# XingqunQi-lab/EmotionGestures

Hardware: AMD Instinct MI355X
Metric: gesture clips/sec (34 frames, 43 joints) (higher is better)
Workload: dtype bf16x3; 1 GPU; TED clips: 4 s 16 kHz audio -> mel(128x124) -> CVAE sample -> generator -> 34x126 pose; global_batch=64, variant=Models_spatial_memory, parallelism=clip-sharded x1, no data-path collective, launch=hipGraph replay, 4 step(s) in flight, branch_streams=False, fold_affine=False

## Files before the change

emotiongestures_amd/_lib.py:

```python
from __future__ import annotations

import ctypes as C
import os

_HERE = os.path.dirname(os.path.abspath(__file__))
LIB_PATH = os.path.join(_HERE, "libemogest_hip.so")

EG_PREC_F32, EG_PREC_BF16X3, EG_PREC_BF16 = 0, 1, 2
PRECISIONS = {"f32": EG_PREC_F32, "fp32": EG_PREC_F32, "bf16x3": EG_PREC_BF16X3, "bf16": EG_PREC_BF16}

(PACK_RAW, PACK_LINEAR, PACK_VEC_PAD, PACK_CONV3X3, PACK_BN_SCALE, PACK_BN_SHIFT, PACK_CONV1X1, PACK_STEM,
 PACK_WN_TAP, PACK_CONV1D, PACK_POS_TABLE, PACK_LINEAR_T, PACK_LINEAR_FOLD, PACK_BIAS_FOLD) = range(14)


class EgError(RuntimeError):
    pass


class EgWeightEntry(C.Structure):
    _fields_ = [("key", C.c_char * 192), ("kind", C.c_int32), ("dims", C.c_int32 * 4),
                ("offset", C.c_int64), ("numel", C.c_int64)]


class EgGeneratorConfig(C.Structure):
    _fields_ = [(n, C.c_int32) for n in (
        "frames", "pose_dim", "prior_frames", "chunk", "d_model", "d_inner", "n_layers", "n_head", "d_k",
        "n_mels", "spec_len", "text_len", "n_words", "embed_dim", "tcn_hidden", "tcn_layers", "variant",
        "precision", "n_position")] + [("reserved", C.c_int32 * 5)]


class EgCvaeConfig(C.Structure):
    _fields_ = [("frames", C.c_int32), ("d_model", C.c_int32), ("latent", C.c_int32), ("n_classes", C.c_int32),
                ("reserved", C.c_int32 * 4)]


_P = C.c_void_p
_I = C.c_int32
_L = C.c_int64


class EgLinearArgs(C.Structure):
    _fields_ = [(n, _P) for n in ("x", "w", "bias", "res1", "res2", "y", "gate_src", "drop_epoch", "partial", "x_images", "y_images")] + \
               [("drop_offset", C.c_uint64)] + \
               [(n, _I) for n in ("lda", "ldw", "ldr", "ldc", "ldg", "m", "n", "k", "relu", "precision", "splits", "k_x", "y_k")] + \
               [("drop_seed", C.c_uint32), ("drop_p", C.c_float)]


SIGNATURES = {
    "eg_last_error": (C.c_char_p, []),
    "eg_launch_count": (_L, []),
    "eg_launch_histogram": (_L, [C.c_char_p, _L, C.c_int32]),
    "eg_version": (C.c_char_p, []),
    "eg_set_default_precision": (C.c_int, [C.c_int]),
    "eg_get_default_precision": (C.c_int, []),
    "eg_generator_default_config": (C.c_int, [C.POINTER(EgGeneratorConfig)]),
    "eg_generator_create": (C.c_int, [C.POINTER(EgGeneratorConfig), C.POINTER(_P)]),
    "eg_generator_destroy": (None, [_P]),
    "eg_generator_arena_floats": (_L, [_P]),
    "eg_generator_num_weights": (_I, [_P]),
    "eg_generator_weight_entry": (C.c_int, [_P, _I, C.POINTER(EgWeightEntry)]),
    "eg_generator_workspace_bytes": (_L, [_P, _I]),
    "eg_generator_forward": (C.c_int, [_P, _P, _I, _P, _P, _P, _P, _P, _P, _P, _P, _P, _P, _L, _P]),
    "eg_generator_forward_draws": (C.c_int, [_P, _P, _I, _I, _P, _P, _P, _P, _P, _L, _P]),
    "eg_generator_draws_workspace_bytes": (_L, [_P, _I, _I]),
    "eg_generator_forward_rollout": (C.c_int, [_P, _P, _I, _I, _P, _P, _P, _P, _P, _P, _P, _P, _P, _P, _P, _P, _L, _P]),
    "eg_generator_rollout_workspace_bytes": (_L, [_P, _I, _I]),
    "eg_generator_forward_rollout_draws": (C.c_int, [_P, _P, _I, _I, _I, _P, _P, _P, _P, _P, _P, _P, _P, _P, _P, _P, _P, _L, _P]),
    "eg_generator_rollout_draws_workspace_bytes": (_L, [_P, _I, _I, _I]),
    "eg_rows_by_table": (C.c_int, [_P, _P, _P, _I, _L, _I, _P]),
    "eg_rollout_ragged_plan_ints": (_L, [_I, _L]),
    "eg_rollout_ragged_plan": (C.c_int, [_P, _I, _P, _P, _P, _P]),
    "eg_generator_forward_rollout_ragged": (C.c_int, [_P, _P, _I, _P, _P, _P, _P, _P, _P, _P, _P, _P, _P, _P, _P, _P, _P, _L, _P]),
    "eg_generator_rollout_ragged_workspace_bytes": (_L, [_P, _I, _L]),
    "eg_stream_state_bytes": (_L, [_P, _I, _I, _I]),
    "eg_stream_reset": (C.c_int, [_P, _P, _I, _I, _I, _P, _P, _P]),
    "eg_stream_push": (C.c_int, [_P, _P, _I, _I, _I, _P, _P, _P, _P]),
    "eg_generator_stream_step": (C.c_int, [_P, _P, _P, _I, _I, _I, _P, _P, _P, _P, _P, _P, _P, _P, _P, _L, _P]),
    "eg_stream_tail": (C.c_int, [_P, _P, _I, _I, _I, _P, _P]),
    "eg_generator_tap": (C.c_int, [_P, _I, _P, C.c_char_p, C.POINTER(_P), C.POINTER(_L)]),
    "eg_cvae_default_config": (C.c_int, [C.POINTER(EgCvaeConfig)]),
    "eg_cvae_create": (C.c_int, [C.POINTER(EgCvaeConfig), C.POINTER(_P)]),
    "eg_cvae_destroy": (None, [_P]),
    "eg_cvae_arena_floats": (_L, [_P]),
    "eg_cvae_num_weights": (_I, [_P]),
    "eg_cvae_weight_entry": (C.c_int, [_P, _I, C.POINTER(EgWeightEntry)]),
    "eg_cvae_workspace_bytes": (_L, [_P, _I]),
    "eg_cvae_sample": (C.c_int, [_P, _P, _I, _P, _P, _P, _P, _L, _P]),
    "eg_cvae_forward": (C.c_int, [_P, _P, _I, _P, _P, _P, _P, _P, _P, _P, _L, _P]),
    "eg_mel_tables": (C.c_int, [_P, _P, _P, _P]),
    "eg_mel_workspace_bytes": (_L, [_I, _I]),
    "eg_melspectrogram": (C.c_int, [_P, _I, _I, _P, _P, _P, _P, _P, _I, _P, _L, _P]),
    "eg_window_gather": (C.c_int, [_P, _I, _L, _I, _L, _I, _P, _P]),
    "eg_window_gather_ragged": (C.c_int, [_P, _I, _L, _P, _P, _L, _I, _P, _P]),
    "eg_beat_tables": (C.c_int, [_P, _P, _P, _P]),
    "eg_beat_workspace_bytes": (_L, [_I, _I]),
    "eg_beat_align": (C.c_int, [_P, _I, _I, _P, _I, _I, _I, _I, _I, C.c_double, _I, _P, _P, _P, _P, _P, _L, _P, _P, _P, _P, _P, _P, _P]),
    "eg_beat_tracks_meta_ints": (_L, [_I]),
    "eg_beat_tracks_meta": (C.c_int, [_P, _P, _P, _I, _I, _P]),
    "eg_beat_tracks_workspace_bytes": (_L, [_P, _P, _I, _I, _I]),
    "eg_beat_align_tracks": (C.c_int, [_P, _I, _L, _P, _P, _P, _I, _I, _I, _P, _I, _I, _P, C.c_double, _I, _P, _P, _P, _P, _P, _L, _P, _P, _P,
                                       _P, _P, _P, _P]),
    "eg_beat_tracks_scan": (C.c_int, [_P, _P, _I, _P, _P, _L, _P, _P, _P]),
    "eg_take_meta_ints": (_L, [_I]),
    "eg_take_meta": (C.c_int, [_P, _I, _P]),
    "eg_track_rows_pack": (C.c_int, [_P, _I, _I, _I, _I, _P, _P, _P, _P]),
    "eg_take_distance_workspace_bytes": (_L, [_P, _I, _I]),
    "eg_take_distance": (C.c_int, [_P, _I, _I, _I, _P, _P, _I, _P, _L, _P, _P, _P]),
    "eg_conv3x3": (C.c_int, [_P, _P, _P, _P, _P, _P, _P, _I, _I, _I, _I, _I, _I, _I, _I, _I, _P]),
    "eg_conv3x3_se": (C.c_int, [_P, _P, _P, _P, _P, _P, _P, _P, _P, _I, _I, _I, _I, _I, _I, _I, _I, _I, _P]),
    "eg_se_gate_pre": (C.c_int, [_P, _P, _I, _P, _P, _P, _P, _P, _P, _P, _P, _I, _I, _I, _I, _P]),
    "eg_conv3x3_gap_tiles": (_I, [_I, _I, _I, _I, _I]),
    "eg_conv3x3_channel_split": (_I, [_I, _I, _I, _I, _I, _I, _I]),
    "eg_stem_conv": (C.c_int, [_P, _P, _P, _P, _P, _P, _I, _I, _I, _I, _P]),
    "eg_se_gate": (C.c_int, [_P, _I, _P, _P, _P, _P, _P, _I, _I, _I, _P]),
    "eg_se_residual_relu": (C.c_int, [_P, _P, _P, _P, _P, _P, _P, _I, _I, _I, _I, _I, _I, _I, _I, _P]),
    "eg_linear": (C.c_int, [_P, _I, _P, _I, _P, _P, _P, _I, _P, _I, _I, _I, _I, _I, _I, _I, _I, _P]),
    "eg_split_tiles": (C.c_int, [_P, _I, _I, _I, _P, _P]),
    "eg_linear_presplit": (C.c_int, [_P, _I, _P, _I, _P, _P, _P, _I, _P, _I, _I, _I, _I, _I, _I, _P]),
    "eg_linear_splitk": (C.c_int, [_P, _I, _P, _I, _P, _P, _I, _I, _I, _I, _I, _I, _P, _I, _P]),
    "eg_layernorm": (C.c_int, [_P, _P, _P, _P, _I, _I, C.c_float, _P]),
    "eg_attention": (C.c_int, [_P, _I, _P, _I, _P, _I, _P, _I, _P, _I, _I, _I, _I, _I, _I, _P]),
    "eg_attention_masked": (C.c_int, [_P, _I, _P, _I, _P, _I, _P, _L, _I, _P, _I, _P, _I, _I, _I, _I, _I, _I, _P]),
    "eg_mha_workspace_bytes": (_L, [_I, _I, _I, _I, _I]),
    "eg_multi_head_attention": (C.c_int, [_P, _P, _P, _P, _P, _P, _P, _P, _P, _P, _I, _I, _I, _I, _I, _I, _P, _L, _P]),
    "eg_ffn_workspace_bytes": (_L, [_I, _I, _I]),
    "eg_positionwise_ffn": (C.c_int, [_P, _P, _P, _P, _P, _P, _P, _P, _I, _I, _I, _I, _P, _L, _P]),
    "eg_tcn_forward": (C.c_int, [_P, _P, _P, _I, _I, _I, _I, _I, _P, _L, _P]),
    "eg_add_rows": (C.c_int, [_P, _P, _P, _L, _I, _I, _P]),
    "eg_conv3x3_packed_floats": (_L, [_I, _I]),
    "eg_profile_enable": (C.c_int, [_I]),
    "eg_profile_disable": (C.c_int, []),
    "eg_profile_read": (_I, [_P, _P, _P, _I]),
    "eg_profile_read_workgroups": (_I, [_P, _I]),
    "eg_reparameterize": (C.c_int, [_P, _P, _P, _P, _L, _P]),
    "eg_conv1d": (C.c_int, [_P, _P, _P, _P, _P, _P, _I, _I, _I, _I, _I, _I, _I, _I, _P]),
    "eg_contrastive_workspace_bytes": (C.c_int64, [_I]),
    "eg_contrastive_loss": (C.c_int, [_P, _P, _I, _I, _P, _P, _P, _P, _L, _P]),
    "eg_contrastive_backward_workspace_bytes": (_L, [_I]),
    "eg_contrastive_loss_backward": (C.c_int, [_P, _P, _I, _I, _P, _P, _P, _L, _P]),
    "eg_transpose": (C.c_int, [_P, _I, _I, _I, _P, _I, _P]),
    "eg_gemm_tn_workspace_floats": (_L, [_I, _I, _L]),
    "eg_gemm_tn": (C.c_int, [_P, _I, _P, _I, _P, _I, _I, _I, _L, _P, _L, _I, _P]),
    "eg_conv3x3_wgrad": (C.c_int, [_P, _P, _P, _I, _I, _I, _I, _I, _I, _P, _L, _P]),
    "eg_im2col3x3": (C.c_int, [_P, _P, _I, _I, _I, _I, _I, _I, _P]),
    "eg_subsample": (C.c_int, [_P, _P, _I, _I, _I, _I, _I, _I, _P]),
    "eg_im2col1d": (C.c_int, [_P, _P, _I, _I, _I, _I, _I, _I, _I, _I, _I, _P]),
    "eg_conv1d_cl_forward": (C.c_int, [_P, _P, _P, _P] + [_I] * 9 + [_P]),
    "eg_conv1d_cl_backward_input": (C.c_int, [_P, _P, _P, _P] + [_I] * 9 + [_P]),
    "eg_conv1d_cl_backward_weight_workspace_floats": (_L, [_I] * 7),
    "eg_conv1d_cl_backward_weight": (C.c_int, [_P, _P, _P, _P, _P] + [_I] * 9 + [_P, _L, _P]),
    "eg_pad_cols": (C.c_int, [_P, _P, _L, _I, _I, _P]),
    "eg_colreduce_workspace_floats": (_L, [_I]),
    "eg_bn_train_forward": (C.c_int, [_P, _P, _P, _P, _P, _P, _P, _P, _L, _I, C.c_float, C.c_float, _P, _P]),
    "eg_bn_train_backward": (C.c_int, [_P, _P, _P, _P, _P, _P, _P, _P, _L, _I, _I, _P, _P]),
    "eg_bn_train_forward_gap": (C.c_int, [_P, _P, _I, _I, _P, _P, _P, _P, _P, _P, _P, _P, _L, _I, C.c_float, C.c_float, _P, _P]),
    "eg_bn_train_forward_sq": (C.c_int, [_P, _P, _P, _I, _I, _P, _P, _P, _P, _P, _P, _P, _P, _L, _I, C.c_float, C.c_float, _P, _P]),
    "eg_conv3x3_sq": (C.c_int, [_P, _P, _P, _P, _P, _P] + [_I] * 8 + [_P]),
    "eg_se_gate_train_forward": (C.c_int, [_P] * 12 + [_I, _I, _I, _P]),
    "eg_se_tail_forward": (C.c_int, [_P] * 9 + [_I, _I, _I, _P]),
    "eg_se_tail_backward_reduce": (C.c_int, [_P] * 7 + [_I, _I, _I, _P, _P]),
    "eg_se_gate_train_backward": (C.c_int, [_P] * 16 + [_I, _I, _I, _P]),
    "eg_se_tail_backward_finish": (C.c_int, [_P] * 14 + [_I, _I, _I, _P]),
    "eg_se_tail_backward_apply": (C.c_int, [_P] * 13 + [_I, _I, _I, _P]),
# ... 82 lines not shown
```

emotiongestures_amd/csrc/common.h:

```cpp
#pragma once
#include <hip/hip_runtime.h>
#include <stdint.h>
#include <stdio.h>
#include <stdarg.h>
#include <atomic>
#include "emogest.h"


typedef float f4 __attribute__((ext_vector_type(4)));
typedef short bf8 __attribute__((ext_vector_type(8)));

#define EG_WAVE 64

void eg_set_error(const char* fmt, ...);

#define EG_REQUIRE(cond, code, ...)                      \
    do {                                                 \
        if (!(cond)) {                                   \
            eg_set_error(__VA_ARGS__);                   \
            return (code);                               \
        }                                                \
    } while (0)

extern std::atomic<long long> g_eg_launches;
extern bool g_eg_launch_hist;
void egi_count_launch(const char* what);
static inline int eg_check_launch(const char* what) {
    g_eg_launches.fetch_add(1, std::memory_order_relaxed);
    if (g_eg_launch_hist) egi_count_launch(what);
    hipError_t e = hipGetLastError();
    if (e != hipSuccess) {
        eg_set_error("%s: %s", what, hipGetErrorString(e));
        return EG_ERR_HIP;
    }
    return EG_OK;
}

int eg_ensure_dynamic_lds(const void* kernel, size_t bytes, const char* who);
#define EG_HIP_TRY(expr, what)                                                         \
    do {                                                                               \
        hipError_t _e = (expr);                                                        \
        if (_e != hipSuccess) {                                                        \
            eg_set_error("%s: %s", (what), hipGetErrorString(_e));                     \
            return EG_ERR_HIP;                                                         \
        }                                                                              \
    } while (0)

static inline bool eg_aligned16(const void* p) { return (reinterpret_cast<uintptr_t>(p) & 15u) == 0; }
static inline int64_t eg_round_up(int64_t x, int64_t m) { return (x + m - 1) / m * m; }
static inline int eg_cdiv(int a, int b) { return (a + b - 1) / b; }

__device__ __forceinline__ float handoff_blend(const float* __restrict__ alpha, int j, int P, float old, float fresh) {
#pragma clang fp contract(off)
    const float a = alpha ? alpha[j] : (float)(j + 1) / (float)(P + 1);
    const float keep = (1.f - a) * old, take = a * fresh;
    return keep + take;
}

__device__ __forceinline__ float wave_sum(float v) {
#pragma unroll
    for (int o = 32; o > 0; o >>= 1) v += __shfl_xor(v, o, 64);
    return v;
}
__device__ __forceinline__ float wave_max(float v) {
#pragma unroll
    for (int o = 32; o > 0; o >>= 1) v = fmaxf(v, __shfl_xor(v, o, 64));
    return v;
}

__device__ __forceinline__ unsigned short f32_to_bf16_rne(float x) {
    unsigned int u = __float_as_uint(x);
    u += 0x7FFFu + ((u >> 16) & 1u);
    return (unsigned short)(u >> 16);
}
__device__ __forceinline__ float bf16_to_f32(unsigned short h) { return __uint_as_float(((unsigned int)h) << 16); }

typedef __bf16 bf16x2_t __attribute__((ext_vector_type(2)));
typedef float f32x2_t __attribute__((ext_vector_type(2)));
typedef unsigned int u32x4_t __attribute__((ext_vector_type(4)));
template <bool WANT_LO>
__device__ __forceinline__ void split_octet(const f4& v0, const f4& v1, bf8& hi, bf8& lo) {
    u32x4_t h, l;
#pragma unroll
    for (int p = 0; p < 4; ++p) {
        const f32x2_t x = {p < 2 ? v0[2 * p] : v1[2 * p - 4], p < 2 ? v0[2 * p + 1] : v1[2 * p - 3]};
        const unsigned hu = __builtin_bit_cast(unsigned, __builtin_convertvector(x, bf16x2_t));
        h[p] = hu;
        if (WANT_LO) {
            const f32x2_t r = {x[0] - __uint_as_float(hu << 16), x[1] - __uint_as_float(hu & 0xffff0000u)};
            l[p] = __builtin_bit_cast(unsigned, __builtin_convertvector(r, bf16x2_t));
        }
    }
    hi = __builtin_bit_cast(bf8, h);
    if (WANT_LO) lo = __builtin_bit_cast(bf8, l);
}

__device__ __forceinline__ unsigned int mix32(unsigned int h) {
    h ^= h >> 16; h *= 0x85EBCA6Bu; h ^= h >> 13; h *= 0xC2B2AE35u; h ^= h >> 16;
    return h;
}
__device__ __forceinline__ unsigned int dropout_seed(unsigned int seed, const int* __restrict__ epoch) {
    return epoch ? seed ^ mix32((unsigned int)*epoch * 0x9E3779B9u + 0x7F4A7C15u) : seed;
}
__device__ __forceinline__ bool dropout_keep(unsigned int seed, unsigned long long ctr, unsigned int thr) {
    return mix32(mix32((unsigned int)ctr ^ seed) + (unsigned int)(ctr >> 32) * 0x9E3779B9u + 0x6A09E667u) >= thr;
}
struct EgDropout {
    unsigned int thr = 0, seed = 0;
    float inv_keep = 1.f;
    unsigned long long offset = 0;
    const int* epoch = nullptr;
};

__device__ __forceinline__ void xcd_tile(int& bx, int& by) {
    const int gx = gridDim.x, gy = gridDim.y, total = gx * gy;
// ... 38 lines not shown
```

emotiongestures_amd/csrc/conv.hip:

```cpp
#include <type_traits>
#include "common.h"


namespace {

struct ConvArgs {
    const float* x; const float* w; const float* bias; const float* scale; const float* shift;
    float* y; float* gap;
    float* gap2 = nullptr;
    int H, W, Ho, Wo, cout, relu, nchw, tiles_x, tiles;
    const float* gate = nullptr; const float* res = nullptr; int relu2 = 0;
    const float* in_scale = nullptr; const float* in_shift = nullptr;
    int wrow = 0;
    const unsigned* res_bits = nullptr;
    const float* res_q = nullptr;
    unsigned int* dbg = nullptr;
};
__device__ __forceinline__ f4 residual_quad(const float* __restrict__ res, const unsigned* __restrict__ bits, size_t e) {
    f4 r = *reinterpret_cast<const f4*>(res + e);
    if (bits) {
        const unsigned nb = bits[e >> 5] >> (unsigned)(e & 28);
        r[0] = (nb & 1u) ? r[0] : 0.f;
        r[1] = (nb & 2u) ? r[1] : 0.f;
        r[2] = (nb & 4u) ? r[2] : 0.f;
        r[3] = (nb & 8u) ? r[3] : 0.f;
    }
    return r;
}

template <int S, int TH> struct ConvGeom {
    static constexpr int IH = (TH - 1) * S + 3;
    static constexpr int IW = 31 * S + 3;
    static constexpr int NPIX = IH * IW;
    static constexpr int PL = (S == 1) ? ((NPIX + 15) / 16 * 16) : (NPIX | 1);
    static constexpr int MT = TH * 2 / 4;
};

template <int TH> struct ConvGeomDG2 {
    static constexpr int IH = TH + 1;
    static constexpr int IW = 33;
    static constexpr int NPIX = IH * IW;
    static constexpr int PL = (NPIX + 15) / 16 * 16;
};

template <int CIN, int NT, int S, int TH>
__global__ __launch_bounds__(256) void conv3x3_f32_kernel(ConvArgs a) {
    using G = ConvGeom<S, TH>;
    constexpr int COUTP = NT * 16, IW = G::IW, NPIX = G::NPIX, PL = G::PL, MT = G::MT;
    __shared__ f4 tile[8 * PL];

    const int tid = threadIdx.x, wave = tid >> 6, lane = tid & 63, li = lane & 15, kq = lane >> 4;
    int tile_id = blockIdx.x, b = blockIdx.y;
    {
        const int total = gridDim.x * gridDim.y;
        if ((total & 7) == 0) {
            const int lin = blockIdx.y * gridDim.x + blockIdx.x;
            const int log = (lin & 7) * (total >> 3) + (lin >> 3);
            b = log / (int)gridDim.x;
            tile_id = log - b * (int)gridDim.x;
        }
    }
    const int ty = tile_id / a.tiles_x, tx = tile_id - ty * a.tiles_x;
    const int oy0 = ty * TH, ox0 = tx * 32;
    const int iy0 = oy0 * S - 1, ix0 = ox0 * S - 1;

    int pbase[MT];
#pragma unroll
    for (int t = 0; t < MT; ++t) {
        const int id = wave * MT + t;
// ... 46 lines not shown
            }
        }
    }

    f4 gsum[NT];
#pragma unroll
    for (int n = 0; n < NT; ++n) gsum[n] = (f4){0.f, 0.f, 0.f, 0.f};
#pragma unroll
    for (int n = 0; n < NT; ++n) {
        const int co = n * 16 + kq * 4;
        const f4 bi = a.bias ? *reinterpret_cast<const f4*>(a.bias + co) : (f4){0.f, 0.f, 0.f, 0.f};
        const f4 sc = a.scale ? *reinterpret_cast<const f4*>(a.scale + co) : (f4){1.f, 1.f, 1.f, 1.f};
        const f4 sh = a.shift ? *reinterpret_cast<const f4*>(a.shift + co) : (f4){0.f, 0.f, 0.f, 0.f};
        const f4 gt = (a.gate && co < a.cout) ? *reinterpret_cast<const f4*>(a.gate + (size_t)b * a.cout + co) : (f4){1.f, 1.f, 1.f, 1.f};
#pragma unroll
        for (int t = 0; t < MT; ++t) {
            const int id = wave * MT + t;
            const int oy = oy0 + (id >> 1), ox = ox0 + (id & 1) * 16 + li;
            const bool valid = (oy < a.Ho) && (ox < a.Wo);
            f4 v = acc[t][n] + bi;
            if (a.relu) {
#pragma unroll
                for (int r = 0; r < 4; ++r) v[r] = fmaxf(v[r], 0.f);
            }
            v = v * sc + sh;
            if (a.gate) v = v * gt;
            if (a.res && valid && co < a.cout) v += residual_quad(a.res, a.res_bits, (((size_t)b * a.Ho + oy) * a.Wo + ox) * a.cout + co);
            if (a.relu2) {
#pragma unroll
                for (int r = 0; r < 4; ++r) v[r] = fmaxf(v[r], 0.f);
            }
            if (valid) {
                if (!a.nchw) {
                    if (co < a.cout)
                        *reinterpret_cast<f4*>(a.y + (((size_t)b * a.Ho + oy) * a.Wo + ox) * a.cout + co) = v;
                } else {
#pragma unroll
                    for (int r = 0; r < 4; ++r)
                        if (co + r < a.cout)
                            a.y[((size_t)b * a.cout + co + r) * a.Ho * a.Wo + (size_t)oy * a.Wo + ox] = v[r];
                }
                gsum[n] += v;
            }
        }
    }
    if (a.gap) {
        float* sred = reinterpret_cast<float*>(tile);
        __syncthreads();
#pragma unroll
        for (int n = 0; n < NT; ++n) {
#pragma unroll
            for (int r = 0; r < 4; ++r) {
                float s = gsum[n][r];
                s += __shfl_xor(s, 1, 64); s += __shfl_xor(s, 2, 64);
                s += __shfl_xor(s, 4, 64); s += __shfl_xor(s, 8, 64);
                if (li == 0) sred[wave * COUTP + n * 16 + kq * 4 + r] = s;
            }
        }
        __syncthreads();
        if (tid < a.cout) {
            const float s = (sred[tid] + sred[COUTP + tid]) + (sred[2 * COUTP + tid] + sred[3 * COUTP + tid]);
            a.gap[((size_t)b * a.tiles + tile_id) * a.cout + tid] = s;
        }
    }
}


template <int CIN, int NTT, int S, int TH, int WM, int WN, int TERMS, int RING, bool SPLIT = false, bool DG2 = false>
__global__ __launch_bounds__(256, 2) void conv3x3_bf16_kernel(ConvArgs a, const bf8* __restrict__ whi,
                                                           const bf8* __restrict__ wlo) {
    static_assert(!DG2 || (S == 1 && !SPLIT), "DG2 tiles the dy grid with unit stride");
    using G = typename std::conditional<DG2, ConvGeomDG2<TH>, ConvGeom<S, TH>>::type;
    constexpr int PH = DG2 ? 4 : 1;
    constexpr int COUTP = NTT * 16, IW = G::IW, NPIX = G::NPIX, PL = G::PL;
    constexpr int MT = TH * 2 / WM, NT = NTT / WN;
    constexpr int NIMG = (TERMS == 3) ? 2 : 1;
    constexpr int TILE = NIMG * 4 * PL;
    constexpr int WIMG = 4 * COUTP;
    constexpr int WBUF = NIMG * WIMG;
    constexpr int NSTEP = (CIN / 32) * 9;
    static_assert(WM * WN == 4 && MT * WM == TH * 2 && NT * WN == NTT, "wave tiling");
    extern __shared__ __attribute__((aligned(16))) bf8 lds[];
    bf8* tile = lds;
    bf8* wring = lds + TILE;

    const int tid = threadIdx.x, wave = tid >> 6, lane = tid & 63, li = lane & 15, kq = lane >> 4;
    const int wm = wave / WN, wn = wave % WN;
    int tile_id = blockIdx.x, b = blockIdx.y;
    const int c0 = SPLIT ? (int)blockIdx.z * COUTP : 0;
    if (!SPLIT) {
        const int total = gridDim.x * gridDim.y;
        if ((total & 7) == 0) {
            const int lin = blockIdx.y * gridDim.x + blockIdx.x;
            const int log = (lin & 7) * (total >> 3) + (lin >> 3);
            b = log / (int)gridDim.x;
            tile_id = log - b * (int)gridDim.x;
        }
    }
    const int ty = tile_id / a.tiles_x, tx = tile_id - ty * a.tiles_x;
    const int oy0 = ty * TH, ox0 = tx * 32;
    const int iy0 = DG2 ? oy0 : oy0 * S - 1, ix0 = DG2 ? ox0 : ox0 * S - 1;

    int pbase[MT];
#pragma unroll
    for (int t = 0; t < MT; ++t) {
        const int id = wm * MT + t;
        pbase[t] = ((id >> 1) * S) * IW + ((id & 1) * 16 + li) * S;
    }
    f4 acc[PH][MT][NT];
#pragma unroll
    for (int ph = 0; ph < PH; ++ph)
#pragma unroll
        for (int t = 0; t < MT; ++t)
#pragma unroll
            for (int n = 0; n < NT; ++n) acc[ph][t][n] = (f4){0.f, 0.f, 0.f, 0.f};
    const float* __restrict__ xb = a.x + (size_t)b * a.H * a.W * CIN;

    const int wave_u = __builtin_amdgcn_readfirstlane(wave);
    constexpr int PIECES = WIMG / 64;
    constexpr int GTOT = NIMG * PIECES;
    constexpr bool COUNTED = (GTOT % 4 == 0);
    constexpr int GW = GTOT / 4;
    auto issue_weights = [&](int step, int buf) {
        const int chunk = step / 9, tap = step - chunk * 9;
        if constexpr (SPLIT) {
            static_assert(COUNTED, "split instantiations deal whole pieces to the four waves");
            const size_t rbase = ((size_t)tap * (CIN / 8) + chunk * 4) * a.wrow + c0;
#pragma unroll
            for (int p = 0; p < GW; ++p) {
                const int flat = p * 4 + wave_u;
                const int img = flat / PIECES, piece = flat - img * PIECES;
                const int slot = piece * 64 + lane, oct = slot / COUTP, co = slot - oct * COUTP;
                const bf8* src = (img ? wlo : whi) + rbase + (size_t)oct * a.wrow + co;
                __builtin_amdgcn_global_load_lds((const __attribute__((address_space(1))) void*)src,
                                                 (__attribute__((address_space(3))) void*)(wring + buf * WBUF + img * WIMG + piece * 64), 16, 0, 0);
            }
            return;
        }
        const size_t gbase = ((size_t)tap * (CIN / 8) + chunk * 4) * COUTP;
        if constexpr (PIECES % 4 == 0) {
#pragma unroll
            for (int img = 0; img < NIMG; ++img) {
                const bf8* src = (img ? wlo : whi) + gbase;
#pragma unroll
                for (int p = 0; p < PIECES / 4; ++p) {
                    const int piece = p * 4 + wave_u;
                    __builtin_amdgcn_global_load_lds((const __attribute__((address_space(1))) void*)(src + piece * 64 + lane),
                                                     (__attribute__((address_space(3))) void*)(wring + buf * WBUF + img * WIMG + piece * 64),
                                                     16, 0, 0);
                }
            }
        } else {
#pragma unroll
            for (int p = 0; p < (GTOT + 3) / 4; ++p) {
                const int flat = p * 4 + wave_u;
                if (COUNTED || flat < GTOT) {
                    const int img = flat / PIECES, piece = flat - img * PIECES;
                    const bf8* src = (img ? wlo : whi) + gbase;
                    __builtin_amdgcn_global_load_lds((const __attribute__((address_space(1))) void*)(src + piece * 64 + lane),
                                                     (__attribute__((address_space(3))) void*)(wring + buf * WBUF + img * WIMG + piece * 64),
                                                     16, 0, 0);
                }
            }
        }
    };
    constexpr int NIT = (((NPIX + 7) / 8) * 32 + 255) / 256;
    f4 pv[NIT][2];
    int goff[NIT], lslot[NIT];
#pragma unroll
    for (int it = 0; it < NIT; ++it) {
        const int idx = tid + it * 256;
        const int p = (idx >> 5) * 8 + (idx & 7), oc = (idx >> 3) & 3;
        const int iy = p / IW, ix = p - iy * IW;
        const int gy = iy0 + iy, gx = ix0 + ix;
        const bool inside = p < NPIX && gy >= 0 && gy < a.H && gx >= 0 && gx < a.W;
        goff[it] = inside ? (gy * a.W + gx) * CIN + oc * 8 : -1;
        lslot[it] = p < NPIX ? oc * PL + p : -1;
    }
    auto load_tile = [&](int chunk) {
#pragma unroll
        for (int it = 0; it < NIT; ++it) {
            pv[it][0] = pv[it][1] = (f4){0.f, 0.f, 0.f, 0.f};
            if (goff[it] >= 0) {
                const float* src = xb + goff[it] + chunk * 32;
                pv[it][0] = *reinterpret_cast<const f4*>(src);
                pv[it][1] = *reinterpret_cast<const f4*>(src + 4);
            }
        }
    };
    const int oc8s = ((tid >> 3) & 3) * 8;
    auto store_tile = [&](int chunk) {
        f4 s0 = (f4){1.f, 1.f, 1.f, 1.f}, s1 = s0, h0 = (f4){0.f, 0.f, 0.f, 0.f}, h1 = h0;
        if (a.in_scale) {
            s0 = *reinterpret_cast<const f4*>(a.in_scale + chunk * 32 + oc8s); s1 = *reinterpret_cast<const f4*>(a.in_scale + chunk * 32 + oc8s + 4);
            h0 = *reinterpret_cast<const f4*>(a.in_shift + chunk * 32 + oc8s); h1 = *reinterpret_cast<const f4*>(a.in_shift + chunk * 32 + oc8s + 4);
        }
#pragma unroll
        for (int it = 0; it < NIT; ++it) {
            if (lslot[it] >= 0) {
                if (a.in_scale && goff[it] >= 0) {
                    pv[it][0] = pv[it][0] * s0 + h0;
                    pv[it][1] = pv[it][1] * s1 + h1;
                }
                bf8 hi, lo;
                split_octet<TERMS == 3>(pv[it][0], pv[it][1], hi, lo);
                tile[lslot[it]] = hi;
                if (TERMS == 3) tile[4 * PL + lslot[it]] = lo;
            }
        }
    };

    struct Frags { bf8 wh[NT], wl[NT], xh[MT], xl[MT]; };
    auto read_w = [&](Frags& f, int tap) {
        const bf8* Wh = wring + (tap % 3) * WBUF + kq * COUTP + wn * NT * 16 + li;
#pragma unroll
        for (int n = 0; n < NT; ++n) {
            f.wh[n] = Wh[n * 16];
            if (TERMS == 3) f.wl[n] = Wh[WIMG + n * 16];
        }
    };
    auto read_x = [&](Frags& f, int tap) {
        const int kh = tap / 3, kw = tap - kh * 3;
        const int toff = DG2 ? (kh == 2 ? IW : 0) + (kw == 2 ? 1 : 0) : kh * IW + kw;
#pragma unroll
        for (int t = 0; t < MT; ++t) {
            f.xh[t] = tile[kq * PL + pbase[t] + toff];
            if (TERMS == 3) f.xl[t] = tile[(4 + kq) * PL + pbase[t] + toff];
        }
    };
    static_assert(MT % 2 == 0, "a step's MFMAs are issued as two halves (pixel tiles)");
    auto mfma_half = [&](const Frags& f, int half, int tap) {
        const int ph = DG2 ? (tap / 3 != 1 ? 2 : 0) + (tap % 3 != 1 ? 1 : 0) : 0;
#pragma unroll
        for (int t = half * (MT / 2); t < (half + 1) * (MT / 2); ++t)
#pragma unroll
            for (int n = 0; n < NT; ++n) {
                if (TERMS == 3) {
                    acc[ph][t][n] = __builtin_amdgcn_mfma_f32_16x16x32_bf16(f.wl[n], f.xh[t], acc[ph][t][n], 0, 0, 0);
                    acc[ph][t][n] = __builtin_amdgcn_mfma_f32_16x16x32_bf16(f.wh[n], f.xl[t], acc[ph][t][n], 0, 0, 0);
                }
                acc[ph][t][n] = __builtin_amdgcn_mfma_f32_16x16x32_bf16(f.wh[n], f.xh[t], acc[ph][t][n], 0, 0, 0);
            }
    };
    static_assert(RING == 3, "schedule below assumes a 3-slot ring");
    auto mid_sync = [&](bool copy_in_flight) {
        if constexpr (COUNTED) {
            __builtin_amdgcn_sched_barrier(0);
            if (copy_in_flight) wait_vmcnt_imm<GW>(); else wait_vmcnt_imm<0>();
            wait_lgkmcnt0();
            wg_barrier();
        } else {
            __syncthreads();
        }
    };
    issue_weights(0, 0);
    if (NSTEP > 1) issue_weights(1, 1);
    load_tile(0);
    Frags fr[2];
#pragma unroll 1
    for (int chunk = 0; chunk < CIN / 32; ++chunk) {
        store_tile(chunk);
        if (COUNTED && chunk > 0) {
            wait_vmcnt_imm<GW>();
            wait_lgkmcnt0();
            wg_barrier();
        } else {
            __syncthreads();
        }
        if (chunk + 1 < CIN / 32) load_tile(chunk + 1);
        read_w(fr[0], 0);
        read_x(fr[0], 0);
#pragma unroll
        for (int tap = 0; tap < 9; ++tap) {
            const int step = chunk * 9 + tap;
            if (step + 2 < NSTEP) issue_weights(step + 2, (tap + 2) % 3);
            mfma_half(fr[tap & 1], 0, tap);
            mid_sync(step + 2 < NSTEP);
            if (tap < 8) { read_w(fr[(tap + 1) & 1], tap + 1); read_x(fr[(tap + 1) & 1], tap + 1); }
            mfma_half(fr[tap & 1], 1, tap);
        }
    }

    if constexpr (DG2) {
        const size_t ohw = (size_t)a.Ho * a.Wo;
        float* __restrict__ yb = a.y + (size_t)b * ohw * a.cout;
        const float* __restrict__ rq = a.res_q ? a.res_q + (size_t)b * a.H * a.W * a.cout : nullptr;
#pragma unroll
        for (int ph = 0; ph < 4; ++ph) {
            const int py = ph >> 1, px = ph & 1;
#pragma unroll
            for (int t = 0; t < MT; ++t) {
                const int id = wm * MT + t;
                const int by = oy0 + (id >> 1), bx = ox0 + (id & 1) * 16 + li;
                const int oy = 2 * by + py, ox = 2 * bx + px;
                if (by < a.H && bx < a.W && oy < a.Ho && ox < a.Wo) {
#pragma unroll
                    for (int n = 0; n < NT; ++n) {
                        const int co = (wn * NT + n) * 16 + kq * 4;
                        if (co < a.cout) {
                            f4 v = acc[ph][t][n];
                            if (ph == 0 && rq) v += *reinterpret_cast<const f4*>(rq + ((size_t)by * a.W + bx) * a.cout + co);
                            *reinterpret_cast<f4*>(yb + ((size_t)oy * a.Wo + ox) * a.cout + co) = v;
                        }
                    }
                }
            }
        }
        return;
    }

    f4 gsum[NT], gsq[NT];
    int pixo[MT];
#pragma unroll
    for (int t = 0; t < MT; ++t) {
        const int id = wm * MT + t;
        const int oy = oy0 + (id >> 1), ox = ox0 + (id & 1) * 16 + li;
        pixo[t] = (oy < a.Ho && ox < a.Wo) ? oy * a.Wo + ox : -1;
    }
    const int hw = a.Ho * a.Wo;
    float* __restrict__ yb = a.y + (size_t)b * hw * a.cout;
#pragma unroll
    for (int n = 0; n < NT; ++n) {
        gsum[n] = (f4){0.f, 0.f, 0.f, 0.f};
        gsq[n] = gsum[n];
        const int co = c0 + (wn * NT + n) * 16 + kq * 4;
        const f4 bi = a.bias ? *reinterpret_cast<const f4*>(a.bias + co) : (f4){0.f, 0.f, 0.f, 0.f};
        const f4 sc = a.scale ? *reinterpret_cast<const f4*>(a.scale + co) : (f4){1.f, 1.f, 1.f, 1.f};
        const f4 sh = a.shift ? *reinterpret_cast<const f4*>(a.shift + co) : (f4){0.f, 0.f, 0.f, 0.f};
        const f4 gt = (a.gate && co < a.cout) ? *reinterpret_cast<const f4*>(a.gate + (size_t)b * a.cout + co) : (f4){1.f, 1.f, 1.f, 1.f};
        const bool rb = a.res != nullptr;
        const size_t rbase = (size_t)b * hw * a.cout;
#pragma unroll
        for (int t = 0; t < MT; ++t) {
            f4 v = acc[0][t][n] + bi;
            if (a.relu) {
#pragma unroll
                for (int r = 0; r < 4; ++r) v[r] = fmaxf(v[r], 0.f);
            }
            v = v * sc + sh;
            if (a.gate) v = v * gt;
            if (rb && pixo[t] >= 0 && co < a.cout) v += residual_quad(a.res, a.res_bits, rbase + (size_t)pixo[t] * a.cout + co);
            if (a.relu2) {
#pragma unroll
                for (int r = 0; r < 4; ++r) v[r] = fmaxf(v[r], 0.f);
            }
            if (pixo[t] >= 0) {
                if (!a.nchw) {
                    if (co < a.cout) *reinterpret_cast<f4*>(yb + pixo[t] * a.cout + co) = v;
                } else {
#pragma unroll
                    for (int r = 0; r < 4; ++r)
                        if (co + r < a.cout) yb[(co + r) * hw + pixo[t]] = v[r];
                }
                gsum[n] += v;
                if (a.gap2) gsq[n] += v * v;
            }
        }
    }
    if (a.gap) {
        float* sred = reinterpret_cast<float*>(lds);
#pragma unroll
        for (int n = 0; n < NT; ++n) {
#pragma unroll
            for (int r = 0; r < 4; ++r) {
                float s = gsum[n][r];
                s += __shfl_xor(s, 1, 64); s += __shfl_xor(s, 2, 64);
                s += __shfl_xor(s, 4, 64); s += __shfl_xor(s, 8, 64);
                if (li == 0) sred[wm * COUTP + (wn * NT + n) * 16 + kq * 4 + r] = s;
                if (a.gap2) {
                    float q = gsq[n][r];
                    q += __shfl_xor(q, 1, 64); q += __shfl_xor(q, 2, 64);
                    q += __shfl_xor(q, 4, 64); q += __shfl_xor(q, 8, 64);
                    if (li == 0) sred[(WM + wm) * COUTP + (wn * NT + n) * 16 + kq * 4 + r] = q;
                }
            }
        }
        __syncthreads();
        if (tid < (SPLIT ? COUTP : a.cout)) {
            float s = 0.f;
#pragma unroll
            for (int m = 0; m < WM; ++m) s += sred[m * COUTP + tid];
            a.gap[((size_t)b * a.tiles + tile_id) * a.cout + c0 + tid] = s;
            if (a.gap2) {
                float q = 0.f;
#pragma unroll
                for (int m = 0; m < WM; ++m) q += sred[(WM + m) * COUTP + tid];
                a.gap2[((size_t)b * a.tiles + tile_id) * a.cout + c0 + tid] = q;
            }
        }
    }
}

template <int TERMS, int TH = 4, bool STAMP = false>
__global__ __launch_bounds__(256, 2) void conv3x3_c32_persistent_kernel(ConvArgs a, const bf8* __restrict__ whi, const bf8* __restrict__ wlo,
                                                                     int total_tiles, int tiles_per_wg) {
    using G = ConvGeom<1, TH>;
    constexpr int CIN = 32, IW = G::IW, NPIX = G::NPIX, PL = G::PL, MT = TH / 2, NT = 2;
    constexpr int NIMG = (TERMS == 3) ? 2 : 1;
    constexpr int TILE = NIMG * 4 * PL, WTAP = 4 * 32, WIMG = 9 * WTAP;
    static_assert(PL - NPIX >= 8 || TH == 4, "the gap scratch of the 8-row variant lives in the planes' padding slots");
    extern __shared__ __attribute__((aligned(16))) bf8 lds[];
    bf8* tile = lds;
    bf8* wl = lds + TILE;
    float* sred_base = reinterpret_cast<float*>(lds + TILE + NIMG * WIMG);
    const int sred_pitch = (TH == 4) ? 32 : PL * 4;
    float* sred = (TH == 4) ? sred_base : reinterpret_cast<float*>(tile + NPIX);

    const int tid = threadIdx.x, wave = tid >> 6, lane = tid & 63, li = lane & 15, kq = lane >> 4;
    const int wave_u = __builtin_amdgcn_readfirstlane(wave);
    int wg = blockIdx.x;
    if ((gridDim.x & 7) == 0) wg = (blockIdx.x & 7) * (gridDim.x >> 3) + (blockIdx.x >> 3);
    const int NWG = gridDim.x;
    const int t_begin = wg, t_end = total_tiles;
    (void)tiles_per_wg;
    if (t_begin >= t_end) return;

#pragma unroll
    for (int img = 0; img < NIMG; ++img) {
        const bf8* src = img ? wlo : whi;
#pragma unroll
        for (int p = 0; p < 5; ++p) {
            const int piece = p * 4 + wave_u;
            if (piece < WIMG / 64)
                __builtin_amdgcn_global_load_lds((const __attribute__((address_space(1))) void*)(src + piece * 64 + lane),
                                                 (__attribute__((address_space(3))) void*)(wl + img * WIMG + piece * 64), 16, 0, 0);
        }
    }

    constexpr int NIT = (((NPIX + 7) / 8) * 32 + 255) / 256;
    int piy[NIT], pix[NIT], lslot[NIT];
#pragma unroll
    for (int it = 0; it < NIT; ++it) {
        const int idx = tid + it * 256;
        const int p = (idx >> 5) * 8 + (idx & 7), oc = (idx >> 3) & 3;
        piy[it] = p / IW;
        pix[it] = p - piy[it] * IW;
        lslot[it] = p < NPIX ? oc * PL + p : -1;
    }
    const int oc8 = ((tid >> 3) & 3) * 8;
    f4 isc[2] = {(f4){1.f, 1.f, 1.f, 1.f}, (f4){1.f, 1.f, 1.f, 1.f}}, ish[2] = {(f4){0.f, 0.f, 0.f, 0.f}, (f4){0.f, 0.f, 0.f, 0.f}};
    if (a.in_scale) {
        isc[0] = *reinterpret_cast<const f4*>(a.in_scale + oc8); isc[1] = *reinterpret_cast<const f4*>(a.in_scale + oc8 + 4);
// ... 142 lines not shown
            for (int t = 0; t < MT; ++t)
#pragma unroll
                for (int n = 0; n < NT; ++n) {
                    if (TERMS == 3) {
                        acc[t][n] = __builtin_amdgcn_mfma_f32_16x16x32_bf16(f.wlf[n], f.xh[t], acc[t][n], 0, 0, 0);
                        acc[t][n] = __builtin_amdgcn_mfma_f32_16x16x32_bf16(f.wh[n], f.xl[t], acc[t][n], 0, 0, 0);
                    }
                    acc[t][n] = __builtin_amdgcn_mfma_f32_16x16x32_bf16(f.wh[n], f.xh[t], acc[t][n], 0, 0, 0);
                }
        }

        if constexpr (STAMP) {
#pragma unroll
            for (int t = 0; t < MT; ++t)
#pragma unroll
                for (int n = 0; n < NT; ++n) asm volatile("" : "+v"(acc[t][n]));
        }
        stamp(3);
        float* __restrict__ yb = a.y + (size_t)b * hw * 32;
        f4 gsum[NT], gsq[NT];
#pragma unroll
        for (int n = 0; n < NT; ++n) {
            gsum[n] = (f4){0.f, 0.f, 0.f, 0.f};
            gsq[n] = gsum[n];
            const int co = n * 16 + kq * 4;
            const f4 gt = a.gate ? *reinterpret_cast<const f4*>(a.gate + (size_t)b * 32 + co) : (f4){1.f, 1.f, 1.f, 1.f};
#pragma unroll
            for (int t = 0; t < MT; ++t) {
                f4 v = acc[t][n] + bi[n];
                if (a.relu) {
#pragma unroll
                    for (int r = 0; r < 4; ++r) v[r] = fmaxf(v[r], 0.f);
                }
                v = v * sc[n] + sh[n];
                if (a.gate) v = v * gt;
                if (has_res && pixo[t] >= 0) v += rs[t][n];
                if (a.relu2) {
#pragma unroll
                    for (int r = 0; r < 4; ++r) v[r] = fmaxf(v[r], 0.f);
                }
                if (pixo[t] >= 0) {
                    *reinterpret_cast<f4*>(yb + pixo[t] * 32 + co) = v;
                    gsum[n] += v;
                    if (a.gap2) gsq[n] += v * v;
                }
            }
        }
        if (a.gap) {
#pragma unroll
            for (int n = 0; n < NT; ++n)
#pragma unroll
                for (int r = 0; r < 4; ++r) {
                    float sm = gsum[n][r];
                    sm += __shfl_xor(sm, 1, 64); sm += __shfl_xor(sm, 2, 64);
                    sm += __shfl_xor(sm, 4, 64); sm += __shfl_xor(sm, 8, 64);
                    if (li == 0) sred[wave * sred_pitch + n * 16 + kq * 4 + r] = sm;
                    if (a.gap2) {
                        float q = gsq[n][r];
                        q += __shfl_xor(q, 1, 64); q += __shfl_xor(q, 2, 64);
                        q += __shfl_xor(q, 4, 64); q += __shfl_xor(q, 8, 64);
                        if (li == 0) sred[128 + wave * 32 + n * 16 + kq * 4 + r] = q;
                    }
                }
        }
        stamp(4);
        __syncthreads();
        stamp(5);
        if (a.gap && tid < 32) {
            float sm = 0.f;
#pragma unroll
            for (int m = 0; m < 4; ++m) sm += sred[m * sred_pitch + tid];
            a.gap[((size_t)b * a.tiles + tile_id) * 32 + tid] = sm;
            if (a.gap2) a.gap2[((size_t)b * a.tiles + tile_id) * 32 + tid] = (sred[128 + tid] + sred[160 + tid]) + (sred[192 + tid] + sred[224 + tid]);
        }
    }
    if constexpr (STAMP) {
        if (lane == 0 && a.dbg)
#pragma unroll
            for (int i = 0; i < 6; ++i) a.dbg[((size_t)blockIdx.x * 4 + wave) * 8 + i] = ph[i];
    }
}

__global__ __launch_bounds__(256) void stem_conv_kernel(const float* __restrict__ x, const float* __restrict__ w,
                                                        const float* __restrict__ bias, const float* __restrict__ scale,
                                                        const float* __restrict__ shift, float* __restrict__ y,
                                                        int B, int H, int W, int C) {
    extern __shared__ float rows[];
    const int cq_n = C >> 2, tid = threadIdx.x;
    const int b = blockIdx.x / H, oy = blockIdx.x - b * H, WP = W + 2;
    const float* xb = x + (size_t)b * H * W;
    for (int i = tid; i < 3 * WP; i += 256) {
        const int r = i / WP, c = i - r * WP, gy = oy + r - 1, gx = c - 1;
        rows[i] = (gy >= 0 && gy < H && gx >= 0 && gx < W) ? xb[gy * W + gx] : 0.f;
    }
    const int cq = tid % cq_n, px0 = tid / cq_n, pstep = 256 / cq_n;
    f4 wv[9];
#pragma unroll
    for (int t = 0; t < 9; ++t) wv[t] = *reinterpret_cast<const f4*>(w + t * C + cq * 4);
    const f4 bi = *reinterpret_cast<const f4*>(bias + cq * 4);
    const f4 sc = *reinterpret_cast<const f4*>(scale + cq * 4), sh = *reinterpret_cast<const f4*>(shift + cq * 4);
    __syncthreads();
    float* yrow = y + ((size_t)b * H + oy) * W * C + cq * 4;
    for (int ox = px0; ox < W; ox += pstep) {
        f4 acc = bi;
#pragma unroll
        for (int kh = 0; kh < 3; ++kh)
#pragma unroll
            for (int kw = 0; kw < 3; ++kw) acc += wv[kh * 3 + kw] * rows[kh * WP + ox + kw];
#pragma unroll
        for (int r = 0; r < 4; ++r) acc[r] = fmaxf(acc[r], 0.f);
        *reinterpret_cast<f4*>(yrow + (size_t)ox * C) = acc * sc + sh;
    }
}

__global__ __launch_bounds__(256) void se_gate_kernel(const float* __restrict__ gap, int tiles, const float* __restrict__ w1,
                                                      const float* __restrict__ b1, const float* __restrict__ w2,
                                                      const float* __restrict__ b2, float* __restrict__ gate, int C, float inv_hw) {
    __shared__ float m[256];
    __shared__ float h[32];
    const int b = blockIdx.x, t = threadIdx.x, R = C >> 3;
    {
        const int c = t % C, g = t / C, G = blockDim.x / C;
        float s = 0.f;
        for (int i = g; i < tiles; i += G) s += gap[((size_t)b * tiles + i) * C + c];
        m[t] = s;
        __syncthreads();
        float tot = 0.f;
        if (t < C)
            for (int j = 0; j < G; ++j) tot += m[j * C + t];
        __syncthreads();
        if (t < C) m[t] = tot * inv_hw;
    }
    __syncthreads();
    if (t < R) {
        float s = b1[t];
        for (int c = 0; c < C; ++c) s += w1[t * C + c] * m[c];
        h[t] = fmaxf(s, 0.f);
    }
    __syncthreads();
    if (t < C) {
        float s = b2[t];
        for (int j = 0; j < R; ++j) s += w2[t * R + j] * h[j];
        gate[(size_t)b * C + t] = 1.f / (1.f + expf(-s));
    }
}

constexpr int GP_T = 1024;
__global__ __launch_bounds__(GP_T) void se_gate_pre_kernel(const float* __restrict__ t1, const float* __restrict__ gap, int tiles,
                                                           const float* __restrict__ w2img, const float* __restrict__ scale2,
                                                           const float* __restrict__ shift2, const float* __restrict__ w1, const float* __restrict__ b1,
                                                           const float* __restrict__ wf2, const float* __restrict__ bf2, float* __restrict__ gate,
                                                           int H, int W, int C) {
    extern __shared__ __attribute__((aligned(16))) float sm[];
    const int b = blockIdx.x, t = threadIdx.x, G = GP_T / C, c = t % C, g = t / C, R = C >> 3;
    float* part = sm;
    float* S = sm + 5 * GP_T;
    float* zp = S + 9 * C;
    float* m = zp + GP_T;
    float* hbuf = m + C;
    const float* tb = t1 + (size_t)b * H * W * C;
    float s0 = 0.f, s1 = 0.f, s2 = 0.f, s3 = 0.f, s4 = 0.f;
#pragma unroll 4
    for (int i = g; i < tiles; i += G) s0 += gap[((size_t)b * tiles + i) * C + c];
#pragma unroll 4
    for (int x = g; x < W; x += G) {
        s1 += tb[(size_t)x * C + c];
        s2 += tb[((size_t)(H - 1) * W + x) * C + c];
    }
#pragma unroll 4
    for (int y = g; y < H; y += G) {
        s3 += tb[((size_t)y * W) * C + c];
        s4 += tb[((size_t)y * W + W - 1) * C + c];
    }
    part[t] = s0; part[GP_T + t] = s1; part[2 * GP_T + t] = s2; part[3 * GP_T + t] = s3; part[4 * GP_T + t] = s4;
    __syncthreads();
    if (t < C) {
        float T = 0.f, R0 = 0.f, RL = 0.f, C0 = 0.f, CL = 0.f;
        for (int j = 0; j < G; ++j) {
            T += part[j * C + t]; R0 += part[GP_T + j * C + t]; RL += part[2 * GP_T + j * C + t]; C0 += part[3 * GP_T + j * C + t];
            CL += part[4 * GP_T + j * C + t];
        }
        const float c00 = tb[t], c0L = tb[(size_t)(W - 1) * C + t], cL0 = tb[((size_t)(H - 1) * W) * C + t], cLL = tb[((size_t)(H - 1) * W + W - 1) * C + t];
#pragma unroll
        for (int kh = 0; kh < 3; ++kh)
#pragma unroll
            for (int kw = 0; kw < 3; ++kw) {
                const float rex = kh == 0 ? RL : (kh == 2 ? R0 : 0.f);
                const float cex = kw == 0 ? CL : (kw == 2 ? C0 : 0.f);
                float corner = 0.f;
                if (kh == 0 && kw == 0) corner = cLL;
                if (kh == 0 && kw == 2) corner = cL0;
                if (kh == 2 && kw == 0) corner = c0L;
                if (kh == 2 && kw == 2) corner = c00;
                S[(kh * 3 + kw) * C + t] = T - rex - cex + corner;
            }
    }
    __syncthreads();
    {
        const f4* w4 = reinterpret_cast<const f4*>(w2img);
        const int nq = 9 * (C >> 2);
        float z = 0.f;
#pragma unroll 4
        for (int q = g; q < nq; q += G) {
            const int tap = q / (C >> 2), cq = q - tap * (C >> 2);
            const f4 wv = w4[(size_t)q * C + c];
            const float* sp = S + tap * C + cq * 4;
            z += (wv[0] * sp[0] + wv[1] * sp[1]) + (wv[2] * sp[2] + wv[3] * sp[3]);
        }
        zp[g * C + c] = z;
    }
    __syncthreads();
    if (t < C) {
        float z = 0.f;
        for (int j = 0; j < G; ++j) z += zp[j * C + t];
        m[t] = z / (float)(H * W) * scale2[t] + shift2[t];
    }
    __syncthreads();
    {
        const int wv = t >> 6, lane = t & 63;
        for (int j = wv; j < R; j += GP_T / 64) {
            float s = 0.f;
            for (int cc = lane; cc < C; cc += 64) s += w1[j * C + cc] * m[cc];
#pragma unroll
            for (int o = 32; o > 0; o >>= 1) s += __shfl_xor(s, o, 64);
            if (lane == 0) hbuf[j] = fmaxf(s + b1[j], 0.f);
        }
    }
    __syncthreads();
    if (t < C) {
        float s = bf2[t];
        for (int j = 0; j < R; ++j) s += wf2[t * R + j] * hbuf[j];
        gate[(size_t)b * C + t] = 1.f / (1.f + expf(-s));
    }
}

__global__ __launch_bounds__(256) void se_tail_identity_kernel(const f4* __restrict__ y, const float* __restrict__ gate,
                                                               const f4* __restrict__ res, f4* __restrict__ out,
                                                               size_t n4, int hw_cq, int cq_n) {
    for (size_t i = (size_t)blockIdx.x * blockDim.x + threadIdx.x; i < n4; i += (size_t)gridDim.x * blockDim.x) {
        const int cq = (int)(i % cq_n);
        const size_t b = i / hw_cq;
        const f4 g = *reinterpret_cast<const f4*>(gate + b * cq_n * 4 + cq * 4);
        f4 v = y[i] * g + res[i];
#pragma unroll
        for (int r = 0; r < 4; ++r) v[r] = fmaxf(v[r], 0.f);
        out[i] = v;
    }
}

template <int CIN, int COUT>
__global__ __launch_bounds__(256) void se_tail_downsample_kernel(const float* __restrict__ y, const float* __restrict__ gate,
                                                                 const float* __restrict__ xin, const float* __restrict__ dsw,
                                                                 const float* __restrict__ dss, const float* __restrict__ dsh,
                                                                 float* __restrict__ out, int B, int Ho, int Wo, int Hin, int Win, int S) {
    extern __shared__ __attribute__((aligned(16))) f4 wl[];
    for (int i = threadIdx.x; i < CIN * COUT / 4; i += 256) wl[i] = reinterpret_cast<const f4*>(dsw)[i];
    __syncthreads();
    constexpr int CQ = COUT / 4;
    for (int row = blockIdx.x; row < B * Ho; row += gridDim.x) {
      const int b = row / Ho, oy = row - b * Ho;
      for (int t = threadIdx.x; t < Wo * CQ; t += 256) {
        const int cq = t % CQ, ox = t / CQ;
        const size_t p = (size_t)row * Wo + ox;
        const float* xp = xin + (((size_t)b * Hin + (size_t)oy * S) * Win + (size_t)ox * S) * CIN;
        f4 acc = (f4){0.f, 0.f, 0.f, 0.f};
#pragma unroll 8
        for (int ci = 0; ci < CIN; ci += 4) {
            const f4 xv = *reinterpret_cast<const f4*>(xp + ci);
#pragma unroll
            for (int j = 0; j < 4; ++j) acc += wl[(ci + j) * CQ + cq] * xv[j];
        }
        const f4 res = acc * *reinterpret_cast<const f4*>(dss + cq * 4) + *reinterpret_cast<const f4*>(dsh + cq * 4);
        const f4 g = *reinterpret_cast<const f4*>(gate + (size_t)b * COUT + cq * 4);
        f4 v = *reinterpret_cast<const f4*>(y + p * COUT + cq * 4) * g + res;
#pragma unroll
        for (int r = 0; r < 4; ++r) v[r] = fmaxf(v[r], 0.f);
        *reinterpret_cast<f4*>(out + p * COUT + cq * 4) = v;
      }
    }
}

template <int CIN, int NT, int S, int TH, int WM, int WN, int TERMS>
int launch_conv_bf16(const ConvArgs& a, const bf8* whi, const bf8* wlo, dim3 grid, hipStream_t st) {
    constexpr int RING = 3;
    using G = ConvGeom<S, TH>;
    constexpr int NIMG = (TERMS == 3) ? 2 : 1;
    constexpr size_t LDS_BYTES = sizeof(bf8) * (size_t)(NIMG * 4 * G::PL + RING * NIMG * 4 * NT * 16);
    auto kern = conv3x3_bf16_kernel<CIN, NT, S, TH, WM, WN, TERMS, RING>;
    if (int rc = eg_ensure_dynamic_lds(reinterpret_cast<const void*>(kern), LDS_BYTES, "conv3x3")) return rc;
    hipLaunchKernelGGL(kern, grid, dim3(256), LDS_BYTES, st, a, whi, wlo);
    return eg_check_launch("conv3x3");
}

template <int CIN, int NTS, int TH, int WM, int WN, int TERMS>
int launch_conv_split_t(ConvArgs a, int batch, const bf8* whi, const bf8* wlo, hipStream_t st) {
    constexpr int RING = 3;
    using G = ConvGeom<1, TH>;
    constexpr int NIMG = (TERMS == 3) ? 2 : 1;
    constexpr size_t LDS_BYTES = sizeof(bf8) * (size_t)(NIMG * 4 * G::PL + RING * NIMG * 4 * NTS * 16);
    auto kern = conv3x3_bf16_kernel<CIN, NTS, 1, TH, WM, WN, TERMS, RING, true>;
    if (int rc = eg_ensure_dynamic_lds(reinterpret_cast<const void*>(kern), LDS_BYTES, "conv3x3 (channel split)")) return rc;
    a.wrow = a.cout;
    hipLaunchKernelGGL(kern, dim3(a.tiles, batch, a.cout / (NTS * 16)), dim3(256), LDS_BYTES, st, a, whi, wlo);
    return eg_check_launch("conv3x3 (channel split)");
}
template <int KCH, int NTN, int TH, int WM, int WN>
int launch_dgrad_s2_t(const ConvArgs& a, int batch, const bf8* whi, const bf8* wlo, hipStream_t st) {
    constexpr int RING = 3;
    using G = ConvGeomDG2<TH>;
    constexpr size_t LDS_BYTES = sizeof(bf8) * (size_t)(2 * 4 * G::PL + RING * 2 * 4 * NTN * 16);
    auto kern = conv3x3_bf16_kernel<KCH, NTN, 1, TH, WM, WN, 3, RING, false, true>;
    if (int rc = eg_ensure_dynamic_lds(reinterpret_cast<const void*>(kern), LDS_BYTES, "conv3x3 (stride-2 input gradient)")) return rc;
    dim3 grid(eg_cdiv(a.W, 32) * eg_cdiv(a.H, TH), batch);
    hipLaunchKernelGGL(kern, grid, dim3(256), LDS_BYTES, st, a, whi, wlo);
    return eg_check_launch("conv3x3 (stride-2 input gradient)");
}
int conv_channel_split(int wgs, int max_split) {
    const char* e = getenv("EG_CONV_SPLIT");
    const int forced = (e && e[0]) ? atoi(e) : -1;
    if (forced >= 0) return (forced == 2 || forced == 4) && forced <= max_split ? forced : 1;
    int split = 1;
    while (split < max_split && wgs * split * 2 <= 512) split *= 2;
    return split;
}

int body_channel_split(int batch, int tiles, int cin, int cout, int stride, int precision, int nchw_out) {
    if (!((cin == 64 || cin == 128) && cout == cin && stride == 1 && precision == EG_PREC_BF16X3 && !nchw_out)) return 1;
    return conv_channel_split(tiles * batch, cin == 128 ? 4 : 2);
}

template <int CIN, int NT, int S, int TH, int WM, int WN>
int launch_conv(const ConvArgs& a, int batch, int precision, hipStream_t st) {
    dim3 grid(a.tiles, batch), block(256);
    if (precision == EG_PREC_F32) {
        hipLaunchKernelGGL((conv3x3_f32_kernel<CIN, NT, S, TH>), grid, block, 0, st, a);
        return eg_check_launch("conv3x3");
    }
    const size_t f32_floats = (size_t)9 * CIN * NT * 16;
    const bf8* whi = reinterpret_cast<const bf8*>(a.w + f32_floats);
    const bf8* wlo = whi + (size_t)9 * (CIN / 8) * NT * 16;
    if (precision == EG_PREC_BF16X3) return launch_conv_bf16<CIN, NT, S, TH, WM, WN, 3>(a, whi, wlo, grid, st);
    return launch_conv_bf16<CIN, NT, S, TH, WM, WN, 1>(a, whi, wlo, grid, st);
}

bool conv32_persistent_enabled() {
    static const bool on = [] { const char* e = getenv("EG_CONV32_PERSISTENT"); return !(e && e[0] == '0'); }();
    return on;
}

template <int TERMS, int TH>
int launch_conv32_persistent_t(const ConvArgs& a, int batch, const bf8* whi, const bf8* wlo, hipStream_t st) {
    using G = ConvGeom<1, TH>;
    constexpr int NIMG = (TERMS == 3) ? 2 : 1;
    constexpr size_t LDS_BYTES = sizeof(bf8) * (size_t)(NIMG * 4 * G::PL + NIMG * 9 * 128) + (TH == 4 ? 2 * 4 * 32 * sizeof(float) : 0);
    auto kern = conv3x3_c32_persistent_kernel<TERMS, TH>;
    if (int rc = eg_ensure_dynamic_lds(reinterpret_cast<const void*>(kern), LDS_BYTES, "conv3x3 (32 -> 32, persistent)")) return rc;
    const int total = a.tiles * batch;
    const int cap = 512;
    int grid = total < cap ? total : cap;
    int tpw = eg_cdiv(total, grid);
    grid = eg_cdiv(total, tpw);
    if (grid >= 8) grid = (int)eg_round_up(grid, 8);
    hipLaunchKernelGGL(kern, dim3(grid), dim3(256), LDS_BYTES, st, a, whi, wlo, total, tpw);
    return eg_check_launch("conv3x3 (32 -> 32, persistent)");
}
int launch_conv32_persistent(const ConvArgs& a, int batch, int precision, int th, hipStream_t st) {
    const size_t f32_floats = (size_t)9 * 32 * 32;
    const bf8* whi = reinterpret_cast<const bf8*>(a.w + f32_floats);
    const bf8* wlo = whi + (size_t)9 * 4 * 32;
    static const bool stamp = [] { const char* e = getenv("EG_CONV32_STAMP"); return e && e[0] == '1'; }();
    if (stamp && precision == EG_PREC_BF16X3 && th == 4) {
        static unsigned int* dbg = nullptr;
        const int nwords = 512 * 4 * 8;
        if (!dbg && hipMalloc(&dbg, nwords * sizeof(unsigned int)) != hipSuccess) return EG_ERR_HIP;
        (void)hipMemsetAsync(dbg, 0, nwords * sizeof(unsigned int), st);
        ConvArgs b = a;
        b.dbg = dbg;
        constexpr size_t LDS_BYTES = sizeof(bf8) * (size_t)(2 * 4 * ConvGeom<1, 4>::PL + 2 * 9 * 128) + 2 * 4 * 32 * sizeof(float);
        auto kern = conv3x3_c32_persistent_kernel<3, 4, true>;
        if (int rc = eg_ensure_dynamic_lds(reinterpret_cast<const void*>(kern), LDS_BYTES, "conv3x3 (stamps)")) return rc;
        const int total = a.tiles * batch;
        int grid = total < 512 ? total : 512;
        grid = eg_cdiv(total, eg_cdiv(total, grid));
        if (grid >= 8) grid = (int)eg_round_up(grid, 8);
        hipLaunchKernelGGL(kern, dim3(grid), dim3(256), LDS_BYTES, st, b, whi, wlo, total, 0);
        static unsigned int host[512 * 4 * 8];
        if (hipMemcpyAsync(host, dbg, sizeof(host), hipMemcpyDeviceToHost, st) != hipSuccess || hipStreamSynchronize(st) != hipSuccess) return EG_ERR_HIP;
        double sum[6] = {0, 0, 0, 0, 0, 0};
        int nw = 0;
        for (int w = 0; w < grid * 4; ++w) {
            if (host[w * 8 + 3] == 0) continue;
            ++nw;
            for (int i = 0; i < 6; ++i) sum[i] += host[w * 8 + i];
        }
        const double tiles_per_wave = (double)total / grid;
        fprintf(stderr, "conv32 stamps (cycles per tile and wave, %d waves, %s residual): store_tile %.0f  barrier1 %.0f  issue_loads %.0f  taps %.0f  epilogue %.0f  barrier2 %.0f\n",
                nw, a.res ? "with" : "no", sum[0] / nw / tiles_per_wave, sum[1] / nw / tiles_per_wave, sum[2] / nw / tiles_per_wave, sum[3] / nw / tiles_per_wave,
                sum[4] / nw / tiles_per_wave, sum[5] / nw / tiles_per_wave);
        return eg_check_launch("conv3x3 (32 -> 32, stamps)");
    }
    if (th == 8) {
        if (precision == EG_PREC_BF16X3) return launch_conv32_persistent_t<3, 8>(a, batch, whi, wlo, st);
        return launch_conv32_persistent_t<1, 8>(a, batch, whi, wlo, st);
    }
    if (precision == EG_PREC_BF16X3) return launch_conv32_persistent_t<3, 4>(a, batch, whi, wlo, st);
    return launch_conv32_persistent_t<1, 4>(a, batch, whi, wlo, st);
}

int conv_tile_rows(int cin, int cout, int stride) {
    if (stride == 2 || cout >= 256) return 2;
    if (cin == 32 && cout == 32) {
        static const int th = [] { const char* e = getenv("EG_CONV32_TH"); return (e && atoi(e) == 8) ? 8 : 4; }();
        return th;
    }
    return (cout >= 128 || cin >= 128) ? 4 : 8;
}

}

extern "C" int32_t eg_conv3x3_gap_tiles(int32_t h, int32_t wdt, int32_t cin, int32_t cout, int32_t stride) {
    const int ho = (h + 2 - 3) / stride + 1, wo = (wdt + 2 - 3) / stride + 1;
    const int th = conv_tile_rows(cin, cout, stride);
    return eg_cdiv(ho, th) * eg_cdiv(wo, 32);
}

extern "C" int32_t eg_conv3x3_channel_split(int32_t batch, int32_t h, int32_t wdt, int32_t cin, int32_t cout, int32_t stride, int32_t precision) {
    return body_channel_split(batch, eg_conv3x3_gap_tiles(h, wdt, cin, cout, stride), cin, cout, stride, precision, 0);
}

extern "C" int64_t eg_conv3x3_packed_floats(int32_t cin, int32_t cout_pad) {
    return (int64_t)9 * cin * cout_pad * 2;
}

extern "C" int eg_conv3x3(const float* x, const float* w, const float* bias, const float* scale, const float* shift,
                          float* y, float* gap_partial, int32_t batch, int32_t h, int32_t wdt, int32_t cin, int32_t cout,
                          int32_t stride, int32_t relu, int32_t nchw_out, int32_t precision, void* stream) {
    return eg_conv3x3_se(x, w, bias, scale, shift, nullptr, nullptr, y, gap_partial, batch, h, wdt, cin, cout, stride, relu, nchw_out, precision, stream);
}

namespace {
int conv3x3_dispatch(const float* x, const float* w, const float* bias, const float* scale, const float* shift, const float* gate, const float* residual,
                     float* y, float* gap_partial, float* gap_sq, int32_t batch, int32_t h, int32_t wdt, int32_t cin, int32_t cout, int32_t stride,
                     int32_t relu, int32_t nchw_out, int32_t precision, void* stream, const float* in_scale = nullptr, const float* in_shift = nullptr,
                     const uint32_t* res_bits = nullptr);
}
extern "C" int eg_conv3x3_se(const float* x, const float* w, const float* bias, const float* scale, const float* shift, const float* gate,
                             const float* residual, float* y, float* gap_partial, int32_t batch, int32_t h, int32_t wdt, int32_t cin,
                             int32_t cout, int32_t stride, int32_t relu, int32_t nchw_out, int32_t precision, void* stream) {
    return conv3x3_dispatch(x, w, bias, scale, shift, gate, residual, y, gap_partial, nullptr, batch, h, wdt, cin, cout, stride, relu, nchw_out, precision, stream);
}
extern "C" int eg_conv3x3_res_masked(const float* x, const float* w, const float* residual, const uint32_t* res_bits, float* y, int32_t batch, int32_t h,
                                     int32_t wdt, int32_t cin, int32_t cout, int32_t precision, void* stream) {
    EG_REQUIRE(residual && res_bits, EG_ERR_BAD_ARG, "eg_conv3x3_res_masked: the residual and its bit mask are required");
    return conv3x3_dispatch(x, w, nullptr, nullptr, nullptr, nullptr, residual, y, nullptr, nullptr, batch, h, wdt, cin, cout, 1, 0, 0, precision, stream, nullptr,
                            nullptr, res_bits);
}
extern "C" int eg_conv3x3_sq(const float* x, const float* w, const float* bias, float* y, float* gap_partial, float* gap_sq_partial, int32_t batch, int32_t h,
                             int32_t wdt, int32_t cin, int32_t cout, int32_t stride, int32_t relu, int32_t precision, void* stream) {
    EG_REQUIRE(gap_partial && gap_sq_partial, EG_ERR_BAD_ARG, "eg_conv3x3_sq: both partial buffers are required");
    EG_REQUIRE(precision != EG_PREC_F32, EG_ERR_UNSUPPORTED, "eg_conv3x3_sq: split-bf16 modes only (the fp32 kernel emits sums only)");
    EG_REQUIRE(!(cin == 32 && cout == 32 && stride == 1) || conv_tile_rows(cin, cout, stride) == 4, EG_ERR_UNSUPPORTED,
               "eg_conv3x3_sq: the 8-row experiment tiles of the 32 -> 32 kernel have no room for the squares scratch");
    return conv3x3_dispatch(x, w, bias, nullptr, nullptr, nullptr, nullptr, y, gap_partial, gap_sq_partial, batch, h, wdt, cin, cout, stride, relu, 0, precision,
                            stream);
}
extern "C" int eg_conv3x3_sq_in_affine(const float* x, const float* in_scale, const float* in_shift, const float* w, const float* bias, float* y,
                                       float* gap_partial, float* gap_sq_partial, int32_t batch, int32_t h, int32_t wdt, int32_t cin, int32_t cout,
                                       int32_t stride, int32_t relu, int32_t precision, void* stream) {
    EG_REQUIRE(in_scale && in_shift, EG_ERR_BAD_ARG, "eg_conv3x3_sq_in_affine: both affine vectors are required");
    EG_REQUIRE(!gap_partial == !gap_sq_partial, EG_ERR_BAD_ARG, "eg_conv3x3_sq_in_affine: both partial buffers or none");
    return conv3x3_dispatch(x, w, bias, nullptr, nullptr, nullptr, nullptr, y, gap_partial, gap_sq_partial, batch, h, wdt, cin, cout, stride, relu, 0, precision,
                            stream, in_scale, in_shift);
}
namespace {
int conv3x3_dispatch(const float* x, const float* w, const float* bias, const float* scale, const float* shift, const float* gate, const float* residual,
                     float* y, float* gap_partial, float* gap_sq, int32_t batch, int32_t h, int32_t wdt, int32_t cin, int32_t cout, int32_t stride,
                     int32_t relu, int32_t nchw_out, int32_t precision, void* stream, const float* in_scale, const float* in_shift, const uint32_t* res_bits) {
    EG_REQUIRE(x && w && y && batch > 0 && h > 0 && wdt > 0, EG_ERR_BAD_ARG, "eg_conv3x3: null pointer or empty shape");
    EG_REQUIRE(!res_bits || (residual && !gate && ((size_t)batch * h * wdt * cout) % 32 == 0), EG_ERR_BAD_ARG,
               "eg_conv3x3_res_masked: the bit mask needs a residual, no gate and a map of a multiple of 32 elements");
    EG_REQUIRE((in_scale == nullptr) == (in_shift == nullptr) && (!in_scale || (precision != EG_PREC_F32 && cin % 32 == 0 && eg_aligned16(in_scale) &&
               eg_aligned16(in_shift))), EG_ERR_BAD_ARG, "eg_conv3x3: the input affine needs both vectors, a split-bf16 mode and cin %% 32 == 0");
    EG_REQUIRE(!gate || residual, EG_ERR_BAD_ARG, "eg_conv3x3_se: a gate needs a residual");
    EG_REQUIRE(!residual || (!nchw_out && stride == 1 && cout % 4 == 0 && (!gate || eg_aligned16(gate)) && eg_aligned16(residual) && residual != y),
               EG_ERR_BAD_ARG, "eg_conv3x3_se: the fused residual needs NHWC output, stride 1, cout %% 4 == 0 and a residual buffer distinct from y");
    EG_REQUIRE(eg_aligned16(x) && eg_aligned16(w) && eg_aligned16(y), EG_ERR_ALIGN, "eg_conv3x3: pointers must be 16-byte aligned");
    EG_REQUIRE(stride == 1 || stride == 2, EG_ERR_UNSUPPORTED, "eg_conv3x3: stride %d", stride);
    EG_REQUIRE(precision >= 0 && precision <= 2, EG_ERR_BAD_ARG, "eg_conv3x3: precision %d", precision);
    EG_REQUIRE(nchw_out || (cout % 4 == 0), EG_ERR_UNSUPPORTED, "eg_conv3x3: NHWC output needs cout %% 4 == 0");
    ConvArgs a;
    a.x = x; a.w = w; a.bias = bias; a.scale = scale; a.shift = shift; a.y = y; a.gap = gap_partial; a.gap2 = gap_sq;
    a.gate = gate; a.res = residual; a.relu2 = gate ? 1 : 0;
    a.res_bits = res_bits;
    a.in_scale = in_scale; a.in_shift = in_shift;
    a.H = h; a.W = wdt; a.Ho = (h + 2 - 3) / stride + 1; a.Wo = (wdt + 2 - 3) / stride + 1;
    a.cout = cout; a.relu = relu; a.nchw = nchw_out;
    const int th = conv_tile_rows(cin, cout, stride);
    a.tiles_x = eg_cdiv(a.Wo, 32);
    a.tiles = a.tiles_x * eg_cdiv(a.Ho, th);
    hipStream_t st = (hipStream_t)stream;
    const int coutp = (int)eg_round_up(cout, 16);
    EgProfScope prof((int64_t)cin * 1000000 + (int64_t)cout * 1000 + stride * 100 + 1,
                     2.0 * 9 * cin * cout * (double)a.Ho * a.Wo * batch, st);
    if (cin == 32 && coutp == 32 && cout == 32 && stride == 1 && precision != EG_PREC_F32 && !nchw_out && conv32_persistent_enabled())
        return launch_conv32_persistent(a, batch, precision, th, st);
    if (cin == 32 && coutp == 32 && stride == 1 && th == 4) return launch_conv<32, 2, 1, 4, 4, 1>(a, batch, precision, st);
    if (cin == 32 && coutp == 32 && stride == 1) return launch_conv<32, 2, 1, 8, 4, 1>(a, batch, precision, st);
    if (cin == 32 && coutp == 64 && stride == 2) return launch_conv<32, 4, 2, 2, 2, 2>(a, batch, precision, st);
    if (const int split = body_channel_split(batch, a.tiles, cin, cout, stride, precision, nchw_out); split > 1) {
        const size_t f32_floats = (size_t)9 * cin * cout;
        const bf8* whi = reinterpret_cast<const bf8*>(a.w + f32_floats);
        const bf8* wlo = whi + (size_t)9 * (cin / 8) * cout;
        if (cin == 64 && split == 2) return launch_conv_split_t<64, 2, 8, 4, 1, 3>(a, batch, whi, wlo, st);
        if (cin == 128 && split == 2) return launch_conv_split_t<128, 4, 4, 2, 2, 3>(a, batch, whi, wlo, st);
        if (cin == 128 && split == 4) return launch_conv_split_t<128, 2, 4, 2, 2, 3>(a, batch, whi, wlo, st);
    }
    if (cin == 64 && coutp == 64 && stride == 1) return launch_conv<64, 4, 1, 8, 4, 1>(a, batch, precision, st);
    if (cin == 64 && coutp == 128 && stride == 2) return launch_conv<64, 8, 2, 2, 2, 2>(a, batch, precision, st);
    if (cin == 64 && coutp == 128 && stride == 1) return launch_conv<64, 8, 1, 4, 2, 2>(a, batch, precision, st);
    if (cin == 128 && coutp == 128 && stride == 1) return launch_conv<128, 8, 1, 4, 2, 2>(a, batch, precision, st);
    if (cin == 128 && coutp == 256 && stride == 2) return launch_conv<128, 16, 2, 2, 1, 4>(a, batch, precision, st);
    if (cin == 256 && coutp == 256 && stride == 1) return launch_conv<256, 16, 1, 2, 1, 4>(a, batch, precision, st);
    if (cin == 128 && coutp <= 64 && stride == 1) {
        if (coutp <= 48) return launch_conv<128, 3, 1, 4, 4, 1>(a, batch, precision, st);
        return launch_conv<128, 4, 1, 4, 4, 1>(a, batch, precision, st);
    }
    if (cin == 128 && coutp <= 128 && stride == 1) return launch_conv<128, 8, 1, 4, 2, 2>(a, batch, precision, st);
    eg_set_error("eg_conv3x3: unsupported channels cin=%d cout=%d stride=%d", cin, cout, stride);
    return EG_ERR_UNSUPPORTED;
}
}

extern "C" int eg_conv3x3_dgrad_s2(const float* dy, const float* w_flip, const float* res_q, float* dx, int32_t batch, int32_t h, int32_t wdt, int32_t cin,
                                   int32_t cout, int32_t precision, void* stream) {
    EG_REQUIRE(dy && w_flip && dx && batch > 0 && h > 0 && wdt > 0, EG_ERR_BAD_ARG, "eg_conv3x3_dgrad_s2: null pointer or empty shape");
    EG_REQUIRE(precision == EG_PREC_BF16X3, EG_ERR_UNSUPPORTED, "eg_conv3x3_dgrad_s2: split-bf16 arithmetic only (precision %d)", precision);
    EG_REQUIRE(eg_aligned16(dy) && eg_aligned16(w_flip) && eg_aligned16(dx) && (!res_q || eg_aligned16(res_q)), EG_ERR_ALIGN,
               "eg_conv3x3_dgrad_s2: pointers must be 16-byte aligned");
    ConvArgs a;
    a.x = dy; a.w = w_flip; a.bias = nullptr; a.scale = nullptr; a.shift = nullptr; a.y = dx; a.gap = nullptr;
    a.H = (h - 1) / 2 + 1; a.W = (wdt - 1) / 2 + 1; a.Ho = h; a.Wo = wdt;
    a.cout = cin; a.relu = 0; a.nchw = 0; a.tiles_x = eg_cdiv(a.W, 32); a.tiles = 0;
    a.res_q = res_q;
    hipStream_t st = (hipStream_t)stream;
    const size_t f32_floats = (size_t)9 * cout * cin;
    const bf8* whi = reinterpret_cast<const bf8*>(w_flip + f32_floats);
    const bf8* wlo = whi + (size_t)9 * (cout / 8) * cin;
    EgProfScope prof((int64_t)cin * 1000000 + (int64_t)cout * 1000 + 200 + 8, 2.0 * 9 * cin * cout * (double)a.H * a.W * batch, st);
    if (cin == 32 && cout == 64) return launch_dgrad_s2_t<64, 2, 4, 4, 1>(a, batch, whi, wlo, st);
    if (cin == 64 && cout == 128) return launch_dgrad_s2_t<128, 4, 2, 2, 2>(a, batch, whi, wlo, st);
    if (cin == 128 && cout == 256) return launch_dgrad_s2_t<256, 8, 1, 1, 4>(a, batch, whi, wlo, st);
    eg_set_error("eg_conv3x3_dgrad_s2: unsupported channels %d -> %d", cin, cout);
    return EG_ERR_UNSUPPORTED;
}

extern "C" int eg_stem_conv(const float* x, const float* w9xc, const float* bias, const float* scale, const float* shift,
                            float* y, int32_t batch, int32_t h, int32_t wdt, int32_t c, void* stream) {
    EG_REQUIRE(x && w9xc && bias && scale && shift && y && batch > 0, EG_ERR_BAD_ARG, "eg_stem_conv: null pointer");
    EG_REQUIRE(c % 4 == 0 && c <= 128 && 256 % (c / 4) == 0, EG_ERR_UNSUPPORTED, "eg_stem_conv: C=%d", c);
    hipLaunchKernelGGL(stem_conv_kernel, dim3(batch * h), dim3(256), 3 * (wdt + 2) * sizeof(float), (hipStream_t)stream, x, w9xc, bias, scale, shift, y,
                       batch, h, wdt, c);
    return eg_check_launch("stem_conv");
}

extern "C" int eg_se_gate(const float* gap_partial, int32_t tiles, const float* w1, const float* b1, const float* w2,
                          const float* b2, float* gate, int32_t batch, int32_t c, int32_t hw, void* stream) {
    EG_REQUIRE(gap_partial && w1 && b1 && w2 && b2 && gate && batch > 0, EG_ERR_BAD_ARG, "eg_se_gate: null pointer");
    EG_REQUIRE(c % 8 == 0 && c <= 256 && (c <= 128 ? 128 % c : 256 % c) == 0, EG_ERR_UNSUPPORTED, "eg_se_gate: C=%d", c);
    hipLaunchKernelGGL(se_gate_kernel, dim3(batch), dim3(c <= 128 ? 128 : 256), 0, (hipStream_t)stream, gap_partial, tiles, w1, b1, w2, b2,
                       gate, c, 1.0f / (float)hw);
    return eg_check_launch("se_gate");
}

extern "C" int eg_se_gate_pre(const float* t1, const float* gap_partial, int32_t tiles, const float* conv2_w, const float* scale2,
                              const float* shift2, const float* w1, const float* b1, const float* w2, const float* b2, float* gate,
                              int32_t batch, int32_t h, int32_t wdt, int32_t c, void* stream) {
    EG_REQUIRE(t1 && gap_partial && conv2_w && scale2 && shift2 && w1 && b1 && w2 && b2 && gate && batch > 0 && h > 1 && wdt > 1, EG_ERR_BAD_ARG,
               "eg_se_gate_pre: null pointer or empty shape");
    EG_REQUIRE(c % 8 == 0 && c <= 256 && 256 % c == 0 && eg_aligned16(conv2_w), EG_ERR_UNSUPPORTED, "eg_se_gate_pre: C=%d", c);
    const size_t smem = sizeof(float) * (5 * GP_T + 9 * (size_t)c + GP_T + c + (c >> 3) + 4);
    hipLaunchKernelGGL(se_gate_pre_kernel, dim3(batch), dim3(GP_T), smem, (hipStream_t)stream, t1, gap_partial, tiles, conv2_w, scale2, shift2, w1,
                       b1, w2, b2, gate, h, wdt, c);
    return eg_check_launch("se_gate_pre");
}

extern "C" int eg_se_residual_relu(const float* y, const float* gate, const float* x_in, const float* ds_w,
                                   const float* ds_scale, const float* ds_shift, float* out, int32_t batch, int32_t ho,
                                   int32_t wo, int32_t c, int32_t h_in, int32_t w_in, int32_t cin, int32_t stride, void* stream) {
    EG_REQUIRE(y && gate && x_in && out && batch > 0, EG_ERR_BAD_ARG, "eg_se_residual_relu: null pointer");
    hipStream_t st = (hipStream_t)stream;
    if (!ds_w) {
        EG_REQUIRE(cin == c && h_in == ho && w_in == wo, EG_ERR_BAD_ARG, "eg_se_residual_relu: identity shortcut shape mismatch");
        const size_t n4 = (size_t)batch * ho * wo * c / 4;
        const int blocks = (int)((n4 + 255) / 256 < 8192 ? (n4 + 255) / 256 : 8192);
        hipLaunchKernelGGL(se_tail_identity_kernel, dim3(blocks), dim3(256), 0, st, reinterpret_cast<const f4*>(y), gate,
                           reinterpret_cast<const f4*>(x_in), reinterpret_cast<f4*>(out), n4, ho * wo * (c / 4), c / 4);
        return eg_check_launch("se_tail");
    }
    EG_REQUIRE(ds_scale && ds_shift, EG_ERR_BAD_ARG, "eg_se_residual_relu: downsample BN missing");
    const size_t total = (size_t)batch * ho * wo * (c / 4);
    const int blocks = (int)((total + 255) / 256 < 4096 ? (total + 255) / 256 : 4096);
    if (cin == 32 && c == 64)
        hipLaunchKernelGGL((se_tail_downsample_kernel<32, 64>), dim3(blocks), dim3(256), 32 * 64 * 4, st, y, gate, x_in, ds_w, ds_scale,
                           ds_shift, out, batch, ho, wo, h_in, w_in, stride);
    else if (cin == 64 && c == 128)
        hipLaunchKernelGGL((se_tail_downsample_kernel<64, 128>), dim3(blocks), dim3(256), 64 * 128 * 4, st, y, gate, x_in, ds_w, ds_scale,
                           ds_shift, out, batch, ho, wo, h_in, w_in, stride);
    else if (cin == 128 && c == 256) {
        if (int rc = eg_ensure_dynamic_lds(reinterpret_cast<const void*>(se_tail_downsample_kernel<128, 256>), 128 * 256 * 4, "eg_se_residual_relu")) return rc;
        hipLaunchKernelGGL((se_tail_downsample_kernel<128, 256>), dim3(blocks < 1024 ? blocks : 1024), dim3(256), 128 * 256 * 4, st, y, gate,
                           x_in, ds_w, ds_scale, ds_shift, out, batch, ho, wo, h_in, w_in, stride);
    } else {
        eg_set_error("eg_se_residual_relu: unsupported downsample %d->%d", cin, c);
        return EG_ERR_UNSUPPORTED;
    }
    return eg_check_launch("se_tail_downsample");
}
```

emotiongestures_amd/csrc/generator.hip:

```cpp
#include "common.h"
#include <string>
#include <vector>
#include <algorithm>
#include <string.h>
#include <map>
#include <mutex>

static thread_local char g_err[512] = "";
void eg_set_error(const char* fmt, ...) {
    va_list ap;
    va_start(ap, fmt);
    vsnprintf(g_err, sizeof(g_err), fmt, ap);
    va_end(ap);
}
extern "C" const char* eg_last_error(void) { return g_err; }
std::atomic<long long> g_eg_launches{0};
extern "C" int64_t eg_launch_count(void) { return (int64_t)g_eg_launches.load(std::memory_order_relaxed); }
bool g_eg_launch_hist = [] { const char* e = getenv("EG_LAUNCH_HIST"); return e && e[0] == '1'; }();
namespace {
std::mutex g_hist_mu;
std::map<std::string, long long> g_hist;
}
void egi_count_launch(const char* what) {
    std::lock_guard<std::mutex> lk(g_hist_mu);
// ... 103 lines not shown
int egi_linear(const EgiLinear& p, hipStream_t st);
int egi_layernorm(const float* x, const float* gamma, const float* beta, float* y, void* img, int rows, int d, float eps, hipStream_t st);
int egi_attention(const float* q, int ldq, const float* k, int ldk, const float* v, int ldv, float* out, int ldo, float* attn,
                  void* oimg, int batch, int heads, int lq, int lk, int dk, int precision, hipStream_t st);
int egi_add_bcast(const float* a, const float* b, float* out, size_t rows, int row_len, int period, int rep, hipStream_t st);
int egi_prior_encoder(const float* prior, const EgiPriorW& w, float* cat, float* tm_mem, float* tm_pe, float* tm_gram, int batch,
                      int P, int F, int D, int Dpad, int chunk, int variant, hipStream_t st);
int egi_conv1d(const float* x, const float* w, const float* bias, const float* scale, const float* shift, float* y, int n, int cin,
               int cout, int lin, int k, int stride, int pad, int act, hipStream_t st);
int egi_convt1d(const float* x, const float* w, const float* bias, const float* scale, const float* shift, float* y, int n, int cin,
                int cout, int lin, hipStream_t st);
int egi_swap01(const void* in, void* out, int A, int B, size_t inner_words, hipStream_t st);
int egi_rows_by_table(const void* in, void* out, const int32_t* table, int rows, size_t inner_words, bool scatter, hipStream_t st);
int egi_rollout_handoff_ragged(const float* pose, const float* prior_in, const float* alpha, float* track, float* windows, float* prior_out,
                               const int32_t* table, int N, int U, int active, int Wmax, int s, int F, int P, int D, hipStream_t st);
int egi_rollout_handoff(const float* pose, const float* prior_in, const float* alpha, float* track, float* windows, float* prior_out, int U,
                        int W, int w, int F, int P, int D, hipStream_t st);
int egi_small_linear(const float* x, int ldx, const float* w, const float* bias, float* y, int ldy, int n, int in, int out,
                     hipStream_t st);

#define EG_TRY(expr)              \
    do {                          \
        int _rc = (expr);         \
        if (_rc) return _rc;      \
    } while (0)

namespace {

struct Layout {
    std::vector<EgWeightEntry> entries;
    int64_t total = 0;
    int64_t add(const std::string& key, int kind, int d0, int d1, int d2, int d3, int64_t numel) {
        total = eg_round_up(total, 16);
        EgWeightEntry e;
        memset(&e, 0, sizeof(e));
        snprintf(e.key, sizeof(e.key), "%s", key.c_str());
        e.kind = kind; e.dims[0] = d0; e.dims[1] = d1; e.dims[2] = d2; e.dims[3] = d3;
        e.offset = total; e.numel = numel;
        entries.push_back(e);
        total += numel;
        return e.offset;
    }
    int64_t raw(const std::string& key, int64_t numel) { return add(key, EG_PACK_RAW, (int)numel, 0, 0, 0, numel); }
    int64_t vec(const std::string& key, int n, int npad) { return add(key, EG_PACK_VEC_PAD, n, npad, 0, 0, npad); }
};

struct LinW { int64_t w = -1, b = -1; int n = 0, k = 0, npad = 0, kpad = 0; };
struct ConvW { int64_t w = -1, bias = -1, scale = -1, shift = -1; int cin = 0, cout = 0, coutp = 0, stride = 1; };
struct BlockW {
    ConvW c1, c2;
    int64_t se_w1, se_b1, se_w2, se_b2;
    bool ds = false;
    int64_t ds_w = -1, ds_scale = -1, ds_shift = -1;
    int cin, cout, stride;
};
struct MhaW { LinW q, kv, qkv, o; int64_t ln_g, ln_b; };
struct FfnW { LinW w1, w2; int64_t ln_g, ln_b; };

LinW add_linear(Layout& L, const std::string& prefix, int n, int k, bool bias, int kpad_force = 0, int npad_force = 0) {
    LinW w;
    w.n = n; w.k = k;
    w.npad = npad_force ? npad_force : (int)eg_round_up(n, 64);
    w.kpad = kpad_force ? kpad_force : (int)eg_round_up(k, 64);
    w.w = L.add(prefix + ".weight", EG_PACK_LINEAR, n, k, w.npad, w.kpad, (int64_t)w.npad * w.kpad * 2);
    if (bias) w.b = L.vec(prefix + ".bias", n, w.npad);
    return w;
}
ConvW add_conv3(Layout& L, const std::string& key, int cin, int cout, int stride) {
    ConvW c;
    c.cin = cin; c.cout = cout; c.coutp = (int)eg_round_up(cout, 16); c.stride = stride;
    c.w = L.add(key + ".weight", EG_PACK_CONV3X3, cout, cin, c.coutp, 0, (int64_t)9 * cin * c.coutp * 2);
    return c;
}
void add_bn(Layout& L, const std::string& prefix, int n, int npad, int64_t& scale, int64_t& shift) {
    scale = L.add(prefix, EG_PACK_BN_SCALE, n, npad, 0, 0, npad);
    shift = L.add(prefix, EG_PACK_BN_SHIFT, n, npad, 0, 0, npad);
}
LinW add_linear_cat(Layout& L, const std::vector<std::string>& prefixes, int n_each, int k, bool bias) {
    LinW w;
    const int n = n_each * (int)prefixes.size();
    w.n = n; w.k = k; w.npad = (int)eg_round_up(n, 64); w.kpad = (int)eg_round_up(k, 64);
    std::string wk, bk;
    for (size_t i = 0; i < prefixes.size(); ++i) {
        wk += (i ? "|" : "") + prefixes[i] + ".weight";
        bk += (i ? "|" : "") + prefixes[i] + ".bias";
    }
    w.w = L.add(wk, EG_PACK_LINEAR, n, k, w.npad, w.kpad, (int64_t)w.npad * w.kpad * 2);
    if (bias) w.b = L.vec(bk, n, w.npad);
    return w;
}
LinW add_linear_fold(Layout& L, const std::string& chains, int n, int k, int kpad_force = 0, int npad_force = 0) {
    LinW w;
    w.n = n; w.k = k;
    w.npad = npad_force ? npad_force : (int)eg_round_up(n, 64);
    w.kpad = kpad_force ? kpad_force : (int)eg_round_up(k, 64);
    w.w = L.add(chains, EG_PACK_LINEAR_FOLD, n, k, w.npad, w.kpad, (int64_t)w.npad * w.kpad * 2);
    w.b = L.add(chains, EG_PACK_BIAS_FOLD, n, w.npad, 0, 0, w.npad);
    return w;
}
MhaW add_mha(Layout& L, const std::string& p, int d, bool self_attn) {
    MhaW m;
    if (self_attn) {
        m.qkv = add_linear_cat(L, {p + ".w_qs", p + ".w_ks", p + ".w_vs"}, d, d, false);
    } else {
        m.q = add_linear(L, p + ".w_qs", d, d, false);
        m.kv = add_linear_cat(L, {p + ".w_ks", p + ".w_vs"}, d, d, false);
// ... 23 lines not shown

}

struct EgGenerator {
    EgGeneratorConfig cfg;
    Layout L;
    int H1, W1, H2, W2, H3, W3, HW3, Dpad, stages[3] = {3, 4, 6}, filters[3] = {32, 64, 128};
    int64_t stem_w, stem_b, stem_scale, stem_shift;
    std::vector<BlockW> blocks;
    ConvW final_conv;
    LinW a_fc1, a_fc2, emosem0, emo2, sem2, fus0, fus2, cls[4], post[4], prior_h0, prior_h2, txt_dec;
    bool fuse_se = true;
    bool fold = false;
    bool shared_chip = false;
    LinW f_audio, f_emo, f_sem, f_post, f_prior;
    int64_t pos_table;
    std::vector<MhaW> enc_attn, dec_attn;
    std::vector<FfnW> enc_ffn, dec_ffn;
    int64_t pc_w1, pc_b1, pc_s1, pc_t1, pc_w2, pc_b2, pc_s2, pc_t2;
    int64_t sp_w0, sp_b0, sp_w1, sp_b1, tc_w0, tc_b0, tc_w1, tc_b1, tm_w0, tm_b0, tm_w1, tm_b1;
    int64_t emb;
    struct TcnConv { LinW tap0, tap1; int64_t bias; };
    std::vector<TcnConv> tcn;
    int64_t txt_fc1_w, txt_fc1_b;
    int Cpad;
    bool keep_taps = false;
    bool concurrent = false;
    mutable hipStream_t side[2] = {nullptr, nullptr};
    mutable hipEvent_t ev_fork = nullptr, ev_join[2] = {nullptr, nullptr};
    int ensure_streams() const {
        if (side[0]) return EG_OK;
        for (int i = 0; i < 2; ++i) {
            if (hipStreamCreateWithFlags(&side[i], hipStreamNonBlocking) != hipSuccess ||
                hipEventCreateWithFlags(&ev_join[i], hipEventDisableTiming) != hipSuccess) {
                eg_set_error("cannot create side stream/event");
                return EG_ERR_HIP;
            }
        }
        if (hipEventCreateWithFlags(&ev_fork, hipEventDisableTiming) != hipSuccess) { eg_set_error("cannot create event"); return EG_ERR_HIP; }
        return EG_OK;
    }
    ~EgGenerator() {
        for (int i = 0; i < 2; ++i) {
            if (side[i]) (void)hipStreamDestroy(side[i]);
            if (ev_join[i]) (void)hipEventDestroy(ev_join[i]);
        }
        if (ev_fork) (void)hipEventDestroy(ev_fork);
    }
};

namespace {

struct GenWs {
    int64_t act[3], gap, gate, amap, afc1, afeat, emo_t, emo, sem_t, sem, cls_part, cls_h[3], cls_out;
    int64_t fus_in, fus_h, fusion, xa, xb, q, qkv, ao, proj, ffn_h, im_x[2], im_enc, im_h, im_a[3], im_p[2];
    int64_t prior_cat, prior_h, prior_enc, prior_rep, tm_mem, tm_pe, tm_gram, post_a, post_b, post_c, pose;
    int64_t t_emb, t_a, t_b, t_c, t_out;
    int64_t tap_stem, tap_l[3];
    int64_t total;
};

GenWs carve(const EgGenerator* g, int B, int NB = 0) {
    if (NB <= 0) NB = B;
    const EgGeneratorConfig& c = g->cfg;
    GenWs w;
    Carver cv;
    const int64_t BF = (int64_t)B * c.frames, D = c.d_model, NF = (int64_t)NB * c.frames;
    const int64_t act = (int64_t)B * g->H1 * g->W1 * 32;
    for (int i = 0; i < 3; ++i) w.act[i] = cv.take(act);
    {
        int64_t gap_per_clip = 0;
        int h = g->H1, wd = g->W1;
        for (const BlockW& b : g->blocks) {
            const int ho = (h + 2 - 3) / b.stride + 1, wo = (wd + 2 - 3) / b.stride + 1;
            const int64_t need = (int64_t)eg_conv3x3_gap_tiles(ho, wo, b.cout, b.cout, 1) * b.cout;
            gap_per_clip = need > gap_per_clip ? need : gap_per_clip;
            h = ho; wd = wo;
        }
        w.gap = cv.take((int64_t)B * gap_per_clip);
    }
    w.gate = cv.take((int64_t)B * 128);
    w.amap = cv.take(BF * g->HW3);
    w.afc1 = cv.take(BF * D); w.afeat = cv.take(BF * D);
    w.emo_t = cv.take(BF * D * 2); w.emo = cv.take(BF * D); w.sem_t = cv.take(16); w.sem = cv.take(BF * D);
    w.cls_part = cv.take((int64_t)(c.frames > 64 ? c.frames : 64) * B * D);
    w.cls_h[0] = cv.take((int64_t)B * D); w.cls_h[1] = cv.take((int64_t)B * 256); w.cls_h[2] = cv.take((int64_t)B * 64);
    w.cls_out = cv.take((int64_t)B * 16);
    w.fus_in = cv.take(NF * D); w.fus_h = cv.take(NF * D); w.fusion = cv.take(NF * D);
    w.xa = cv.take(NF * D); w.xb = cv.take(NF * D);
    w.q = cv.take(NF * D); w.qkv = cv.take(NF * D * 3); w.ao = cv.take(NF * D); w.proj = cv.take(NF * D);
    w.ffn_h = cv.take(NF * c.d_inner);
    {
        const int64_t N64 = eg_round_up(NF, 64), B64 = eg_round_up(BF, 64), KX = D > g->Dpad ? D : g->Dpad;
        w.im_x[0] = cv.take(N64 * KX); w.im_x[1] = cv.take(N64 * KX); w.im_enc = cv.take(N64 * D); w.im_h = cv.take(N64 * c.d_inner);
        w.im_a[0] = cv.take(B64 * D); w.im_a[1] = cv.take(B64 * D); w.im_a[2] = cv.take(B64 * D * 2);
        w.im_p[0] = cv.take(B64 * D); w.im_p[1] = cv.take(B64 * D);
    }
    w.prior_cat = cv.take(BF * g->Dpad); w.prior_h = cv.take(BF * D); w.prior_enc = cv.take(BF * D);
    w.prior_rep = cv.take(NB > B ? NF * D : 16);
    w.tm_mem = cv.take((int64_t)B * c.pose_dim); w.tm_pe = cv.take((int64_t)B * c.chunk + 16); w.tm_gram = cv.take((int64_t)c.pose_dim * c.chunk);
    w.post_a = cv.take(NF * D * 4); w.post_b = cv.take(NF * D); w.post_c = cv.take(NF * g->Dpad); w.pose = cv.take(NF * c.pose_dim);
    const int64_t BT = (int64_t)B * c.text_len;
    w.t_emb = cv.take(BT * g->Cpad); w.t_a = cv.take(BT * g->Cpad); w.t_b = cv.take(BT * g->Cpad); w.t_c = cv.take(BT * g->Cpad);
    w.t_out = cv.take(BT * 512);
    w.tap_stem = w.tap_l[0] = w.tap_l[1] = w.tap_l[2] = -1;
    if (g->keep_taps) {
        w.tap_stem = cv.take(act);
        w.tap_l[0] = cv.take(act);
        w.tap_l[1] = cv.take((int64_t)B * g->H2 * g->W2 * 64);
        w.tap_l[2] = cv.take((int64_t)B * g->H3 * g->W3 * 128);
    }
    w.total = cv.off;
    return w;
}

inline float* P(void* ws, int64_t off) { return reinterpret_cast<float*>(reinterpret_cast<char*>(ws) + off); }

int run_linear(const float* arena, const LinW& w, const float* x, int lda, float* y, int ldc, int m, int relu, const float* res1,
               int ldr, int prec, hipStream_t st, int n_override = 0) {
    return eg_linear(x, lda, arena + w.w, w.kpad, w.b >= 0 ? arena + w.b : nullptr, res1, nullptr, ldr, y, ldc, m,
                     n_override ? n_override : w.n, w.kpad <= lda ? w.kpad : w.k, relu, 0, 0, prec, st);
}

int run_conv(const float* arena, const ConvW& c, const float* x, float* y, float* gap, int B, int h, int w, int relu, int nchw,
             int prec, hipStream_t st) {
    return eg_conv3x3(x, arena + c.w, c.bias >= 0 ? arena + c.bias : nullptr, c.scale >= 0 ? arena + c.scale : nullptr,
                      c.shift >= 0 ? arena + c.shift : nullptr, y, gap, B, h, w, c.cin, c.cout, c.stride, relu, nchw, prec, st);
}

struct Act { float* f = nullptr; int ld = 0; void* img = nullptr; int kimg = 0; };
inline Act act(float* f, int ld, void* img = nullptr, int kimg = 0) { Act a; a.f = f; a.ld = ld; a.img = img; a.kimg = kimg; return a; }

int lin(const EgGenerator* g, const float* arena, const LinW& w, const Act& x, int xk0, const Act& y, bool want_f32, int m, int relu,
        const float* res1, int ldr, hipStream_t st, int n_override = 0, int splits = 0, float* partial = nullptr) {
// ... 19 lines not shown
    const int D = g->cfg.d_model;
    float *qkv = P(ws, w.qkv), *ao = P(ws, w.ao), *pr = P(ws, w.proj);
    void* aimg = g->cfg.precision != EG_PREC_F32 ? P(ws, w.im_h) : nullptr;
    if (!xkv.f) {
        EG_TRY(lin(g, arena, m.qkv, xq, 0, act(qkv, 3 * D), true, B * Lq, 0, nullptr, 0, st));
        EG_TRY(egi_attention(qkv, 3 * D, qkv + D, 3 * D, qkv + 2 * D, 3 * D, ao, D, nullptr, aimg, B, g->cfg.n_head, Lq, Lk, g->cfg.d_k, g->cfg.precision, st));
    } else {
        float* q = P(ws, w.q);
        EG_TRY(lin(g, arena, m.q, xq, 0, act(q, D), true, B * Lq, 0, nullptr, 0, st));
        EG_TRY(lin(g, arena, m.kv, xkv, 0, act(qkv, 2 * D), true, B * Lk, 0, nullptr, 0, st));
        EG_TRY(egi_attention(q, D, qkv, 2 * D, qkv + D, 2 * D, ao, D, nullptr, aimg, B, g->cfg.n_head, Lq, Lk, g->cfg.d_k, g->cfg.precision, st));
    }
    EG_TRY(lin(g, arena, m.o, act(ao, D, aimg, D), 0, act(pr, D), true, B * Lq, 0, xq.f, D, st));
    return egi_layernorm(pr, arena + m.ln_g, arena + m.ln_b, out.f, g->cfg.precision != EG_PREC_F32 ? out.img : nullptr, B * Lq, D, 1e-6f, st);
}

int run_mha_kv(const EgGenerator* g, const float* arena, const MhaW& m, const Act& xq, const float* kv, const Act& out, const GenWs& w,
               void* ws, int B, int Lq, int Lk, hipStream_t st) {
    const int D = g->cfg.d_model;
    float *q = P(ws, w.q), *ao = P(ws, w.ao), *pr = P(ws, w.proj);
    void* aimg = g->cfg.precision != EG_PREC_F32 ? P(ws, w.im_h) : nullptr;
    EG_TRY(lin(g, arena, m.q, xq, 0, act(q, D), true, B * Lq, 0, nullptr, 0, st));
    EG_TRY(egi_attention(q, D, kv, 2 * D, kv + D, 2 * D, ao, D, nullptr, aimg, B, g->cfg.n_head, Lq, Lk, g->cfg.d_k, g->cfg.precision, st));
    EG_TRY(lin(g, arena, m.o, act(ao, D, aimg, D), 0, act(pr, D), true, B * Lq, 0, xq.f, D, st));
    return egi_layernorm(pr, arena + m.ln_g, arena + m.ln_b, out.f, g->cfg.precision != EG_PREC_F32 ? out.img : nullptr, B * Lq, D, 1e-6f, st);
}

int run_ffn(const EgGenerator* g, const float* arena, const FfnW& f, const Act& x, const Act& out, const GenWs& w, void* ws, int rows,
            hipStream_t st) {
    const int D = g->cfg.d_model, DI = g->cfg.d_inner;
    float *h = P(ws, w.ffn_h), *pr = P(ws, w.proj);
    const Act hid = act(h, DI, P(ws, w.im_h), DI);
    EG_TRY(lin(g, arena, f.w1, x, 0, hid, false, rows, 1, nullptr, 0, st));
    const int sp = (g->cfg.precision != EG_PREC_F32 && rows <= 64 && DI >= 2048 && 4 * D <= DI) ? 4 : 0;
    EG_TRY(lin(g, arena, f.w2, hid, 0, act(pr, D), true, rows, 0, x.f, D, st, 0, sp, h));
    return egi_layernorm(pr, arena + f.ln_g, arena + f.ln_b, out.f, g->cfg.precision != EG_PREC_F32 ? out.img : nullptr, rows, D, 1e-6f, st);
}


int run_audio_tower(const EgGenerator* g, const float* arena, const float* spec, const GenWs& w, void* ws, int B, hipStream_t st) {
    const int prec = g->cfg.precision, F = g->cfg.frames, D = g->cfg.d_model;
    float* bufs[3] = {P(ws, w.act[0]), P(ws, w.act[1]), P(ws, w.act[2])};
    float *gap = P(ws, w.gap), *gate = P(ws, w.gate);
    int xi = 0, h = g->H1, wd = g->W1, bi = 0;
    EG_TRY(eg_stem_conv(spec, arena + g->stem_w, arena + g->stem_b, arena + g->stem_scale, arena + g->stem_shift, bufs[0], B, g->H1,
                        g->W1, 32, st));
    if (g->keep_taps)
        EG_HIP_TRY(hipMemcpyAsync(P(ws, w.tap_stem), bufs[0], sizeof(float) * (size_t)B * g->H1 * g->W1 * 32, hipMemcpyDeviceToDevice, st), "tap copy");
    for (int s = 0; s < 3; ++s) {
        for (int j = 0; j < g->stages[s]; ++j, ++bi) {
            const BlockW& bw = g->blocks[bi];
            const int t1 = (xi + 1) % 3, t2 = (xi + 2) % 3;
            const int ho = (h + 2 - 3) / bw.stride + 1, wo = (wd + 2 - 3) / bw.stride + 1;
            if (!bw.ds && g->fuse_se) {
                EG_TRY(run_conv(arena, bw.c1, bufs[xi], bufs[t1], gap, B, h, wd, 1, 0, prec, st));
                const int tiles1 = eg_conv3x3_gap_tiles(h, wd, bw.cin, bw.cout, 1);
                EG_TRY(eg_se_gate_pre(bufs[t1], gap, tiles1, arena + bw.c2.w, arena + bw.c2.scale, arena + bw.c2.shift, arena + bw.se_w1,
                                      arena + bw.se_b1, arena + bw.se_w2, arena + bw.se_b2, gate, B, ho, wo, bw.cout, st));
                EG_TRY(eg_conv3x3_se(bufs[t1], arena + bw.c2.w, nullptr, arena + bw.c2.scale, arena + bw.c2.shift, gate, bufs[xi], bufs[t2], nullptr, B,
                                     ho, wo, bw.cout, bw.cout, 1, 0, 0, prec, st));
                xi = t2; h = ho; wd = wo;
                continue;
            }
            EG_TRY(run_conv(arena, bw.c1, bufs[xi], bufs[t1], nullptr, B, h, wd, 1, 0, prec, st));
            EG_TRY(run_conv(arena, bw.c2, bufs[t1], bufs[t2], gap, B, ho, wo, 0, 0, prec, st));
            const int tiles = eg_conv3x3_gap_tiles(ho, wo, bw.cout, bw.cout, 1);
            EG_TRY(eg_se_gate(gap, tiles, arena + bw.se_w1, arena + bw.se_b1, arena + bw.se_w2, arena + bw.se_b2, gate, B, bw.cout,
                              ho * wo, st));
            EG_TRY(eg_se_residual_relu(bufs[t2], gate, bufs[xi], bw.ds ? arena + bw.ds_w : nullptr, bw.ds ? arena + bw.ds_scale : nullptr,
                                       bw.ds ? arena + bw.ds_shift : nullptr, bufs[t1], B, ho, wo, bw.cout, h, wd, bw.cin, bw.stride, st));
            xi = t1; h = ho; wd = wo;
        }
        if (g->keep_taps)
            EG_HIP_TRY(hipMemcpyAsync(P(ws, w.tap_l[s]), bufs[xi], sizeof(float) * (size_t)B * h * wd * g->filters[s], hipMemcpyDeviceToDevice, st), "tap copy");
    }
    float* amap = P(ws, w.amap);
    EG_TRY(run_conv(arena, g->final_conv, bufs[xi], amap, nullptr, B, h, wd, 0, 1, prec, st));
    if (g->fold) return lin(g, arena, g->f_audio, act(amap, g->HW3), 0, act(P(ws, w.afeat), D, P(ws, w.im_a[1]), D), true, B * F, 0, nullptr, 0, st);
    const Act h1 = act(P(ws, w.afc1), D, P(ws, w.im_a[0]), D);
    EG_TRY(lin(g, arena, g->a_fc1, act(amap, g->HW3), 0, h1, false, B * F, 0, nullptr, 0, st));
    return lin(g, arena, g->a_fc2, h1, 0, act(P(ws, w.afeat), D, P(ws, w.im_a[1]), D), true, B * F, 0, nullptr, 0, st);
}

int run_text(const EgGenerator* g, const float* arena, const int64_t* text, float* out, const GenWs& w, void* ws, int B, hipStream_t st) {
    const EgGeneratorConfig& c = g->cfg;
    const int L = c.text_len, C = c.tcn_hidden, ld = g->Cpad, rows = B * L, prec = c.precision;
    float *x = P(ws, w.t_emb), *h1 = P(ws, w.t_a), *h2 = P(ws, w.t_b), *y = P(ws, w.t_c);
    EG_TRY(egi_embedding(text, arena + g->emb, x, rows, c.embed_dim, ld, c.n_words, st));
    for (int i = 0; i < c.tcn_layers; ++i) {
        const int d = 1 << i;
        const EgGenerator::TcnConv& c1 = g->tcn[2 * i];
        const EgGenerator::TcnConv& c2 = g->tcn[2 * i + 1];
        EG_TRY(eg_linear(x, ld, arena + c1.tap0.w, c1.tap0.kpad, arena + c1.bias, nullptr, nullptr, 0, h1, ld, rows, C, C, 0, d, L, prec, st));
        EG_TRY(eg_linear(x, ld, arena + c1.tap1.w, c1.tap1.kpad, nullptr, h1, nullptr, ld, h1, ld, rows, C, C, 1, 0, 0, prec, st));
        EG_TRY(eg_linear(h1, ld, arena + c2.tap0.w, c2.tap0.kpad, arena + c2.bias, nullptr, nullptr, 0, h2, ld, rows, C, C, 0, d, L, prec, st));
        EG_TRY(eg_linear(h1, ld, arena + c2.tap1.w, c2.tap1.kpad, nullptr, h2, x, ld, y, ld, rows, C, C, 1, 0, 0, prec, st));
        float* t = x; x = y; y = t;
    }
    EG_TRY(egi_time_linear(x, arena + g->txt_fc1_w, arena + g->txt_fc1_b, h1, B, L, C, ld, st));
    return eg_linear(h1, ld, arena + g->txt_dec.w, g->txt_dec.kpad, arena + g->txt_dec.b, nullptr, nullptr, 0, out, 512, rows, 512, C, 0,
                     0, 0, prec, st);
}

int run_prior(const EgGenerator* g, const float* arena, const float* prior, const GenWs& w, void* ws, int B, hipStream_t st) {
    const EgGeneratorConfig& c = g->cfg;
    EgiPriorW pw;
    memset(&pw, 0, sizeof(pw));
    pw.w1 = arena + g->pc_w1; pw.b1 = arena + g->pc_b1; pw.s1 = arena + g->pc_s1; pw.t1 = arena + g->pc_t1;
    pw.w2 = arena + g->pc_w2; pw.b2 = arena + g->pc_b2; pw.s2 = arena + g->pc_s2; pw.t2 = arena + g->pc_t2;
    if (c.variant == 1) {
        pw.sp_w0 = arena + g->sp_w0; pw.sp_b0 = arena + g->sp_b0; pw.sp_w1 = arena + g->sp_w1; pw.sp_b1 = arena + g->sp_b1;
        pw.tc_w0 = arena + g->tc_w0; pw.tc_b0 = arena + g->tc_b0; pw.tc_w1 = arena + g->tc_w1; pw.tc_b1 = arena + g->tc_b1;
        pw.tm_w0 = arena + g->tm_w0; pw.tm_b0 = arena + g->tm_b0; pw.tm_w1 = arena + g->tm_w1; pw.tm_b1 = arena + g->tm_b1;
// ... 106 lines not shown

extern "C" int eg_generator_default_config(EgGeneratorConfig* c) {
    EG_REQUIRE(c, EG_ERR_BAD_ARG, "null config");
    memset(c, 0, sizeof(*c));
    c->frames = 34; c->pose_dim = 126; c->prior_frames = 4; c->chunk = 4; c->d_model = 512; c->d_inner = 2048; c->n_layers = 3;
    c->n_head = 8; c->d_k = 64; c->n_mels = 128; c->spec_len = 124; c->text_len = 60; c->n_words = 200; c->embed_dim = 300;
    c->tcn_hidden = 300; c->tcn_layers = 3; c->variant = 0; c->precision = g_default_precision; c->n_position = 60;
    return EG_OK;
}

extern "C" int eg_generator_create(const EgGeneratorConfig* cfg, EgGenerator** out) {
    EG_REQUIRE(cfg && out, EG_ERR_BAD_ARG, "eg_generator_create: null pointer");
    EG_TRY(validate_cfg(*cfg));
    EgGenerator* g = new EgGenerator();
    g->cfg = *cfg;
    g->keep_taps = cfg->reserved[0] != 0;
    g->concurrent = cfg->reserved[1] != 0;
    g->fold = cfg->reserved[2] != 0;
    g->fuse_se = cfg->reserved[3] == 0;
    g->shared_chip = cfg->reserved[4] != 0;
    const EgGeneratorConfig& c = g->cfg;
    g->H1 = c.n_mels; g->W1 = c.spec_len;
    g->H2 = (g->H1 - 1) / 2 + 1; g->W2 = (g->W1 - 1) / 2 + 1;
    g->H3 = (g->H2 - 1) / 2 + 1; g->W3 = (g->W2 - 1) / 2 + 1;
    g->HW3 = g->H3 * g->W3;
    if (g->HW3 % 8 != 0) { delete g; eg_set_error("config: final map %dx%d not a multiple of 8", g->H3, g->W3); return EG_ERR_UNSUPPORTED; }
    g->Dpad = (int)eg_round_up(c.pose_dim, 64);
    g->Cpad = (int)eg_round_up(c.tcn_hidden, 64);
    Layout& L = g->L;
    const int D = c.d_model, F = c.frames, P_ = c.prior_frames, PL = F - P_, PD = c.pose_dim;
    const std::string fe = "audio_encoder.feat_extractor";
    g->stem_w = L.add(fe + ".conv1.weight", EG_PACK_STEM, 32, 0, 0, 0, 9 * 32);
    g->stem_b = L.raw(fe + ".conv1.bias", 32);
    add_bn(L, fe + ".bn1", 32, 32, g->stem_scale, g->stem_shift);
    int inpl = 32;
    for (int s = 0; s < 3; ++s) {
        const int planes = g->filters[s];
        for (int j = 0; j < g->stages[s]; ++j) {
            BlockW b;
            const std::string p = fe + ".layer" + std::to_string(s + 1) + "." + std::to_string(j);
            b.stride = (s > 0 && j == 0) ? 2 : 1;
            b.cin = inpl; b.cout = planes;
            b.c1 = add_conv3(L, p + ".conv1", inpl, planes, b.stride);
            add_bn(L, p + ".bn1", planes, planes, b.c1.scale, b.c1.shift);
            b.c2 = add_conv3(L, p + ".conv2", planes, planes, 1);
            add_bn(L, p + ".bn2", planes, planes, b.c2.scale, b.c2.shift);
            b.se_w1 = L.raw(p + ".se.fc.0.weight", planes / 8 * planes);
            b.se_b1 = L.raw(p + ".se.fc.0.bias", planes / 8);
            b.se_w2 = L.raw(p + ".se.fc.2.weight", planes * (planes / 8));
            b.se_b2 = L.raw(p + ".se.fc.2.bias", planes);
            b.ds = (b.stride != 1 || inpl != planes);
            if (b.ds) {
                b.ds_w = L.add(p + ".downsample.0.weight", EG_PACK_CONV1X1, planes, inpl, 0, 0, (int64_t)inpl * planes);
                add_bn(L, p + ".downsample.1", planes, planes, b.ds_scale, b.ds_shift);
            }
            g->blocks.push_back(b);
            inpl = planes;
        }
    }
    g->final_conv = add_conv3(L, "audio_encoder.final_conv1", 128, F, 1);
    if (g->final_conv.coutp > 64) {
        g->final_conv.coutp = 128;
        L.entries.back().dims[2] = 128;
        L.total -= L.entries.back().numel;
        L.entries.back().numel = (int64_t)9 * 128 * 128 * 2;
        L.total += L.entries.back().numel;
    }
    g->final_conv.bias = L.vec("audio_encoder.final_conv1.bias", F, g->final_conv.coutp);
    add_bn(L, "audio_encoder.bn1", F, g->final_conv.coutp, g->final_conv.scale, g->final_conv.shift);
    if (g->fold) {
        g->f_audio = add_linear_fold(L, "audio_encoder.fc2@audio_encoder.fc1", D, g->HW3);
        g->f_emo = add_linear_fold(L, "emotion_proj.2@emotion_proj.0", D, D);
        g->f_sem = add_linear_fold(L, "semantic_proj.2@semantic_proj.0", D, D);
    } else {
        g->a_fc1 = add_linear(L, "audio_encoder.fc1", D, g->HW3, true);
        g->a_fc2 = add_linear(L, "audio_encoder.fc2", D, D, true);
        g->emosem0 = add_linear_cat(L, {"emotion_proj.0", "semantic_proj.0"}, D, D, true);
        g->emo2 = add_linear(L, "emotion_proj.2", D, D, true);
        g->sem2 = add_linear(L, "semantic_proj.2", D, D, true);
    }
    g->fus0 = add_linear(L, "fusion_proj.0", D, D, true); g->fus2 = add_linear(L, "fusion_proj.2", D, D, true);
    g->cls[0] = add_linear(L, "emotion_classifer_header.0", D, F * D, true);
    g->cls[1] = add_linear(L, "emotion_classifer_header.2", 256, D, true);
    g->cls[2] = add_linear(L, "emotion_classifer_header.4", 64, 256, true);
    g->cls[3] = add_linear(L, "emotion_classifer_header.6", 8, 64, true);
    const std::string pp = "prior_seq_encoder";
    if (g->fold) {
        g->f_post = add_linear_fold(L, "post_projector.6@post_projector.4@post_projector.2@post_projector.0", PD, D);
        g->f_prior = add_linear_fold(L, pp + ".post_header.2@" + pp + ".post_header.0", D, PD, g->Dpad, 0);
    } else {
        g->post[0] = add_linear(L, "post_projector.0", D * 4, D, true);
        g->post[1] = add_linear(L, "post_projector.2", D, D * 4, true);
        g->post[2] = add_linear(L, "post_projector.4", PD, D, true, 0, g->Dpad);
        g->post[3] = add_linear(L, "post_projector.6", PD, PD, true, g->Dpad, 0);
        g->prior_h0 = add_linear(L, pp + ".post_header.0", D, PD, true, g->Dpad, 0);
        g->prior_h2 = add_linear(L, pp + ".post_header.2", D, D, true);
    }
    g->pc_w1 = L.raw(pp + ".pred_conv.0.weight", (int64_t)PL * P_ * 3); g->pc_b1 = L.raw(pp + ".pred_conv.0.bias", PL);
    add_bn(L, pp + ".pred_conv.2", PL, PL, g->pc_s1, g->pc_t1);
    g->pc_w2 = L.raw(pp + ".pred_conv.3.weight", (int64_t)PL * PL * 3); g->pc_b2 = L.raw(pp + ".pred_conv.3.bias", PL);
    add_bn(L, pp + ".pred_conv.5", PL, PL, g->pc_s2, g->pc_t2);
    if (c.variant == 1) {
        const int CD = c.chunk * PD;
        const std::string sp = pp + ".spatial_memory.spatial_chunk_encoder", tm = pp + ".temporal_memory";
        g->sp_w0 = L.raw(sp + ".0.weight", (int64_t)PD * CD); g->sp_b0 = L.raw(sp + ".0.bias", PD);
        g->sp_w1 = L.raw(sp + ".2.weight", (int64_t)PD * PD); g->sp_b1 = L.raw(sp + ".2.bias", PD);
// ... 664 lines not shown
```

emotiongestures_amd/csrc/misc.hip:

```cpp
#include "common.h"

namespace {

struct LnSum { int nparts = 0; const float* bias2 = nullptr; const float* resid = nullptr; int ldr = 0; };
template <int NV, bool SUMP = false>
__global__ __launch_bounds__(256) void layernorm_kernel(const float* __restrict__ x, const float* __restrict__ g,
                                                        const float* __restrict__ b, float* __restrict__ y, int rows, int D,
                                                        float eps, unsigned short* __restrict__ img, LnSum ps = LnSum()) {
    const int row = blockIdx.x * 4 + (threadIdx.x >> 6), lane = threadIdx.x & 63;
    if (row >= rows) return;
    const f4* xr = reinterpret_cast<const f4*>(x + (size_t)row * D);
    const int nq = D >> 2;
    f4 v[NV];
    float s = 0.f;
#pragma unroll
    for (int i = 0; i < NV; ++i) {
        const int q = lane + i * 64;
        v[i] = q < nq ? xr[q] : (f4){0.f, 0.f, 0.f, 0.f};
        if (SUMP && q < nq) {
            for (int p = 1; p < ps.nparts; ++p) v[i] += reinterpret_cast<const f4*>(x + ((size_t)p * rows + row) * D)[q];
            v[i] = v[i] + reinterpret_cast<const f4*>(ps.bias2)[q] + reinterpret_cast<const f4*>(ps.resid + (size_t)row * ps.ldr)[q];
        }
        s += (v[i][0] + v[i][1]) + (v[i][2] + v[i][3]);
    }
    const float mean = wave_sum(s) / (float)D;
    float ss = 0.f;
#pragma unroll
    for (int i = 0; i < NV; ++i) {
        const int q = lane + i * 64;
        if (q < nq) {
            const f4 d = v[i] - mean;
            ss += (d[0] * d[0] + d[1] * d[1]) + (d[2] * d[2] + d[3] * d[3]);
        }
    }
    const float rstd = 1.0f / sqrtf(wave_sum(ss) / (float)D + eps);
    f4* yr = reinterpret_cast<f4*>(y + (size_t)row * D);
#pragma unroll
    for (int i = 0; i < NV; ++i) {
        const int q = lane + i * 64;
        if (q < nq) {
            const f4 o = (v[i] - mean) * rstd * reinterpret_cast<const f4*>(g)[q] + reinterpret_cast<const f4*>(b)[q];
            yr[q] = o;
            if (img) {
                const f4 z = (f4){0.f, 0.f, 0.f, 0.f};
                bf8 h8, l8;
                split_octet<true>(o, z, h8, l8);
                const int KO = D >> 3;
                const size_t slot = (((size_t)(row >> 6) * KO + (q >> 1)) * 64 + (row & 63)) * 8 + (q & 1) * 4;
                const size_t lo_off = (size_t)((rows + 63) >> 6) * KO * 512;
                typedef unsigned int u32x2 __attribute__((ext_vector_type(2)));
                const u32x4_t hh = __builtin_bit_cast(u32x4_t, h8), ll = __builtin_bit_cast(u32x4_t, l8);
                *reinterpret_cast<u32x2*>(img + slot) = (u32x2){hh[0], hh[1]};
                *reinterpret_cast<u32x2*>(img + lo_off + slot) = (u32x2){ll[0], ll[1]};
            }
        }
    }
}

__global__ __launch_bounds__(256) void layernorm_any_kernel(const float* __restrict__ x, const float* __restrict__ g, const float* __restrict__ b,
                                                            float* __restrict__ y, int rows, int D, float eps) {
    const int row = blockIdx.x * 4 + (threadIdx.x >> 6), lane = threadIdx.x & 63;
    if (row >= rows) return;
    const float* xr = x + (size_t)row * D;
    float s = 0.f;
    for (int i = lane; i < D; i += 64) s += xr[i];
    const float mean = wave_sum(s) / (float)D;
    float ss = 0.f;
    for (int i = lane; i < D; i += 64) { const float d = xr[i] - mean; ss += d * d; }
    const float rstd = 1.0f / sqrtf(wave_sum(ss) / (float)D + eps);
    for (int i = lane; i < D; i += 64) y[(size_t)row * D + i] = (xr[i] - mean) * rstd * g[i] + b[i];
}

__global__ __launch_bounds__(256) void add_rows_any_kernel(const float* __restrict__ a, const float* __restrict__ table, float* __restrict__ out,
                                                           size_t n, int d, int period) {
    for (size_t i = (size_t)blockIdx.x * 256 + threadIdx.x; i < n; i += (size_t)gridDim.x * 256) {
// ... 763 lines not shown
```

emotiongestures_amd/modules.py:

```python
from __future__ import annotations

import copy
import functools
import math
import threading
from typing import Optional

import numpy as np
import torch
import torch.nn as nn

from . import _lib as L
from . import ops
from .engine import CvaeEngine, GeneratorEngine

__all__ = [
    "Linear", "Conv1d", "Conv2d", "ConvTranspose1d", "BatchNorm", "LayerNormParams", "WeightNormConv1d",
    "SELayer", "SEBasicBlock", "ResNetSE", "ScaledDotProductAttention", "MultiHeadAttention",
    "PositionwiseFeedForward", "EncoderLayer", "DecoderLayer", "TemporalBlock", "TemporalConvNet",
    "PositionalEncoding", "Audio_ResNetEncoder", "TextEncoderTCN", "SP_Memory_Net_v1", "SP_Memory_Net_v2",
    "TM_Memory_Net", "Prior_MemoryEncoder", "Encoder", "Decoder", "Transformer", "MLP_Reconstruct_v3",
]

_DEFAULT_PRECISION = "f32"
# ... 187 lines not shown
    def forward(self, x):
        raise RuntimeError("placeholder slot; computed by the fused HIP path of the parent module")


def _seq(*mods):
    return nn.Sequential(*[m if m is not None else _Placeholder() for m in mods])


class SELayer(nn.Module):

    def __init__(self, channel, reduction=8):
        super().__init__()
        self.fc = _seq(Linear(channel, channel // reduction), None, Linear(channel // reduction, channel), None)


class SEBasicBlock(nn.Module):
    expansion = 1

    def __init__(self, inplanes, planes, stride=1, downsample=None, reduction=8):
        super().__init__()
        self.conv1 = Conv2d(inplanes, planes, 3, stride, 1, bias=False)
        self.bn1 = BatchNorm(planes)
        self.conv2 = Conv2d(planes, planes, 3, 1, 1, bias=False)
        self.bn2 = BatchNorm(planes)
        self.se = SELayer(planes, reduction)
        self.downsample = downsample
        self.stride = stride if isinstance(stride, int) else stride[0]
        self.precision = _DEFAULT_PRECISION

    def _packed(self, device):
        ver = (str(device),) + tuple(t._version for t in list(self.parameters()) + list(self.buffers()))
        if getattr(self, "_pack", None) is None or self._pack[0] != ver:
            s1, t1 = self.bn1.affine()
            s2, t2 = self.bn2.affine()
            c1 = ops.conv3x3_pack(self.conv1.weight, None, s1, t1, device)
            c2 = ops.conv3x3_pack(self.conv2.weight, None, s2, t2, device)
            ds = None
            if self.downsample is not None:
                a, b = self.downsample[1].affine()
                ds = (a.detach().to(device).contiguous(), b.detach().to(device).contiguous())
            self._pack = (ver, c1, c2, ds)
        return self._pack[1:]

    def forward_nhwc(self, x):
        _eval_only(self)
        c1, c2, ds = self._packed(x.device)
        h = ops.conv3x3(x, self.conv1.weight, stride=self.stride, relu=True, precision=self.precision, packed=c1)
        y, gap = ops.conv3x3(h, self.conv2.weight, want_gap=True, precision=self.precision, packed=c2)
        gate = ops.se_gate(gap, self.se.fc[0].weight, self.se.fc[0].bias, self.se.fc[2].weight, self.se.fc[2].bias,
                           y.shape[1] * y.shape[2])
        if self.downsample is not None:
            return ops.se_residual_relu(y, gate, x, self.downsample[0].weight, ds[0], ds[1], stride=self.stride)
        return ops.se_residual_relu(y, gate, x)

    def forward(self, x):
        return self.forward_nhwc(x.permute(0, 2, 3, 1).contiguous()).permute(0, 3, 1, 2).contiguous()


class ResNetSE(nn.Module):

    def __init__(self, block, layers, num_filters):
        super().__init__()
        self.inplanes = num_filters[0]
        self.conv1 = Conv2d(1, num_filters[0], 3, 1, 1)
        self.bn1 = BatchNorm(num_filters[0])
        self.layer1 = self._make_layer(block, num_filters[0], layers[0])
        self.layer2 = self._make_layer(block, num_filters[1], layers[1], stride=(2, 2))
        self.layer3 = self._make_layer(block, num_filters[2], layers[2], stride=(2, 2))
        if len(num_filters) > 3:
            self.layer4 = self._make_layer(block, num_filters[3], layers[3], stride=(2, 2))
        for m in self.modules():
            if isinstance(m, Conv2d):
                nn.init.kaiming_normal_(m.weight, mode="fan_out", nonlinearity="relu")

    def _make_layer(self, block, planes, blocks, stride=1):
        downsample = None
        s = stride if isinstance(stride, int) else stride[0]
        if s != 1 or self.inplanes != planes * block.expansion:
            downsample = _seq(Conv2d(self.inplanes, planes * block.expansion, 1, s, 0, bias=False),
                              BatchNorm(planes * block.expansion))
        layers = [block(self.inplanes, planes, s, downsample)]
        self.inplanes = planes * block.expansion
        layers += [block(self.inplanes, planes) for _ in range(1, blocks)]
        return nn.Sequential(*layers)

    def forward_nhwc(self, spec):
        _eval_only(self)
        s, t = self.bn1.affine()
        x = ops.stem_conv(spec, self.conv1.weight, self.conv1.bias, s, t)
        for layer in (self.layer1, self.layer2, self.layer3, getattr(self, "layer4", ())):
            for blk in layer:
                x = blk.forward_nhwc(x)
        return x

    def forward(self, x):
        return self.forward_nhwc(x[:, 0]).permute(0, 3, 1, 2).contiguous()


class ScaledDotProductAttention(nn.Module):

    def __init__(self, temperature, attn_dropout=0.1):
        super().__init__()
        self.temperature = temperature
        self.dropout_p = float(attn_dropout)

    def forward(self, q, k, v, mask=None):
# ... 438 lines not shown
```

emotiongestures_amd/ops.py:

```python
from __future__ import annotations

import ctypes as C
from typing import Optional

import numpy as np
import torch

from . import _lib as L
from . import packing
from .engine import _need_cuda, _ptr, _stream


def _dev(t):
    return t.device


def pack_linear_weight(w: torch.Tensor, device) -> torch.Tensor:
    n, k = w.shape
    npad, kpad = (n + 63) // 64 * 64, (k + 63) // 64 * 64
    if w.is_cuda and w.device == torch.device(device) and w.dtype == torch.float32:
        lib = L.load()
        wd = w.detach().contiguous()
        img = torch.empty(int(lib.eg_linear_packed_floats(n, k)), dtype=torch.float32, device=wd.device)
        L.check(lib.eg_pack_linear_device(_ptr(wd), k, n, k, 0, _ptr(img), _stream(wd.device)), "eg_pack_linear_device")
# ... 37 lines not shown
    tiles = lib.eg_conv3x3_gap_tiles(H, W, Cin, Cout, stride)
    if want_gap:
        gap = torch.empty(B, tiles, Cout, device=dev)
    L.check(lib.eg_conv3x3(_ptr(x), _ptr(wp), _ptr(bias_p), _ptr(scale_p), _ptr(shift_p), _ptr(y), _ptr(gap), B, H, W, Cin, Cout,
                           stride, int(relu), int(nchw_out), L.precision_code(precision), _stream(dev)), "eg_conv3x3")
    return (y, gap) if want_gap else y


def conv3x3_pack(weight_oihw, bias, scale, shift, device):
    wp, opad = pack_conv3x3_weight(weight_oihw, device)
    return wp, _padvec(bias, opad, device), _padvec(scale, opad, device), _padvec(shift, opad, device)


def stem_conv(x, weight, bias, scale, shift):
    lib = L.load()
    x = _need_cuda(x, "x")
    dev = x.device
    B, H, W = x.shape
    Cc = weight.shape[0]
    w9 = weight.detach().reshape(Cc, 9).t().contiguous().to(dev, torch.float32)
    y = torch.empty(B, H, W, Cc, device=dev)
    L.check(lib.eg_stem_conv(_ptr(x), _ptr(w9), _ptr(_need_cuda(bias, "bias")), _ptr(_need_cuda(scale, "scale")),
                             _ptr(_need_cuda(shift, "shift")), _ptr(y), B, H, W, Cc, _stream(dev)), "eg_stem_conv")
    return y


def se_gate(gap_partial, w1, b1, w2, b2, hw: int):
    lib = L.load()
    g = _need_cuda(gap_partial, "gap")
    dev = g.device
    B, tiles, Cc = g.shape
    gate = torch.empty(B, Cc, device=dev)
    L.check(lib.eg_se_gate(_ptr(g), tiles, _ptr(_need_cuda(w1, "w1")), _ptr(_need_cuda(b1, "b1")), _ptr(_need_cuda(w2, "w2")),
                           _ptr(_need_cuda(b2, "b2")), _ptr(gate), B, Cc, hw, _stream(dev)), "eg_se_gate")
    return gate


def se_residual_relu(y, gate, x_in, ds_weight=None, ds_scale=None, ds_shift=None, stride=1):
    lib = L.load()
    y, gate, x_in = _need_cuda(y, "y"), _need_cuda(gate, "gate"), _need_cuda(x_in, "x_in")
    dev = y.device
    B, Ho, Wo, Cc = y.shape
    _, Hi, Wi, Cin = x_in.shape
    dsw = None
    if ds_weight is not None:
        dsw = ds_weight.detach().reshape(Cc, Cin).t().contiguous().to(dev, torch.float32)
        ds_scale, ds_shift = _need_cuda(ds_scale, "ds_scale"), _need_cuda(ds_shift, "ds_shift")
    out = torch.empty_like(y)
    L.check(lib.eg_se_residual_relu(_ptr(y), _ptr(gate), _ptr(x_in), _ptr(dsw), _ptr(ds_scale), _ptr(ds_shift), _ptr(out), B, Ho, Wo,
                                    Cc, Hi, Wi, Cin, stride, _stream(dev)), "eg_se_residual_relu")
    return out


def linear(x, weight, bias=None, res1=None, res2=None, relu=False, a_shift=0, a_seq=0, precision="f32", packed=None):
    lib = L.load()
    x = _need_cuda(x, "x")
    dev = x.device
    M, K = x.shape
    N = weight.shape[0]
    wp, npad, kpad = packed if packed is not None else pack_linear_weight(weight, dev)
    bias_p = _padvec(bias, npad, dev)
    y = torch.empty(M, N, device=dev)
    r1 = _need_cuda(res1, "res1") if res1 is not None else None
    r2 = _need_cuda(res2, "res2") if res2 is not None else None
    L.check(lib.eg_linear(_ptr(x), K, _ptr(wp), kpad, _ptr(bias_p), _ptr(r1), _ptr(r2), N, _ptr(y), N, M, N, K, int(relu), a_shift,
                          a_seq, L.precision_code(precision), _stream(dev)), "eg_linear")
    return y


def linear_splitk(x, weight, bias=None, relu=False, splits=8, precision="f32", packed=None):
    lib = L.load()
    x = _need_cuda(x, "x")
    dev = x.device
    M, K = x.shape
    N = weight.shape[0]
    wp, npad, kpad = packed if packed is not None else pack_linear_weight(weight, dev)
    bias_p = _padvec(bias, npad, dev)
    y = torch.empty(M, N, device=dev)
    part = torch.empty(splits + 1, M, N, device=dev)
    L.check(lib.eg_linear_splitk(_ptr(x), K, _ptr(wp), kpad, _ptr(bias_p), _ptr(y), N, M, N, K, int(relu), splits, _ptr(part),
                                 L.precision_code(precision), _stream(dev)), "eg_linear_splitk")
    return y


def layernorm(x, gamma, beta, eps=1e-6):
    lib = L.load()
    x = _need_cuda(x, "x")
    dev = x.device
    rows, d = x.reshape(-1, x.shape[-1]).shape
    y = torch.empty_like(x)
    L.check(lib.eg_layernorm(_ptr(x), _ptr(_need_cuda(gamma, "gamma")), _ptr(_need_cuda(beta, "beta")), _ptr(y), rows, d, eps,
                             _stream(dev)), "eg_layernorm")
    return y


def _attention_mask_bytes(mask, B, Lq, Lk, dev):
    m = mask
    if m.dim() == 4:
        if m.shape[1] != 1:
            raise NotImplementedError("attention mask: per-head masks are not used by the reference (the head axis is broadcast)")
        m = m[:, 0]
    if m.dim() == 2:
        m = m[:, None, :]
    rows = Lq if m.shape[1] != 1 else 1
    m = (m != 0).expand(B, rows, Lk).to(device=dev, dtype=torch.uint8).contiguous()
    return m, rows * Lk, (Lk if rows > 1 else 0)
# ... 126 lines not shown
```

emotiongestures_amd/packing.py:

```python
from __future__ import annotations

import ctypes as C
from typing import Mapping

import numpy as np
import torch

from . import _lib as L

BN_EPS = 1e-5


def _t(sd: Mapping[str, torch.Tensor], key: str) -> torch.Tensor:
    if "|" in key:
        return torch.cat([_t(sd, k) for k in key.split("|")], 0)
    if key not in sd:
        raise KeyError(f"state_dict is missing '{key}' required by the HIP weight manifest")
    return sd[key].detach().to("cpu", torch.float32)


def _bf16_split_bits(w: torch.Tensor):
    hi = w.to(torch.bfloat16)
    lo = (w - hi.to(torch.float32)).to(torch.bfloat16)
    return hi.view(torch.int16).numpy(), lo.view(torch.int16).numpy()


def _with_bf16_images(f32_img: np.ndarray, hi_bits: np.ndarray, lo_bits: np.ndarray) -> np.ndarray:
    out = np.concatenate([f32_img.reshape(-1).view(np.int16), hi_bits.reshape(-1), lo_bits.reshape(-1)])
    return out.view(np.float32)


def _pack_linear(w: torch.Tensor, npad: int, kpad: int) -> np.ndarray:
    n, k = w.shape
    assert npad % 64 == 0 and kpad % 64 == 0
    p = torch.zeros(npad, kpad, dtype=torch.float32)
    p[:n, :k] = w
    t = p.reshape(npad // 64, 64, kpad // 8, 8).permute(0, 2, 1, 3).contiguous()
    hi, lo = _bf16_split_bits(t)
    return _with_bf16_images(p.numpy(), hi, lo)


def _pack_conv3x3(w: torch.Tensor, opad: int) -> np.ndarray:
    o, i = w.shape[:2]
    p = torch.zeros(opad, i, 3, 3, dtype=torch.float32)
    p[:o] = w
    t = p.permute(2, 3, 1, 0).reshape(9, i, opad)
    f32 = t.reshape(9, i // 4, 4, opad).permute(0, 1, 3, 2).contiguous()
    oct_ = t.reshape(9, i // 8, 8, opad).permute(0, 1, 3, 2).contiguous()
    hi, lo = _bf16_split_bits(oct_)
    return _with_bf16_images(f32.numpy(), hi, lo)


def _bn_affine(sd, prefix: str):
    scale = _t(sd, prefix + ".weight") / torch.sqrt(_t(sd, prefix + ".running_var") + BN_EPS)
    shift = _t(sd, prefix + ".bias") - _t(sd, prefix + ".running_mean") * scale
    return scale, shift


def _pad1(v: torch.Tensor, npad: int) -> np.ndarray:
    out = np.zeros(npad, dtype=np.float32)
    out[: v.numel()] = v.reshape(-1).numpy()
    return out


def _fold_chain(sd, chain: str):
    names = chain.split("@")[::-1]
    w = _t(sd, names[0] + ".weight").double()
    b = _t(sd, names[0] + ".bias").double()
    for nme in names[1:]:
        wi, bi = _t(sd, nme + ".weight").double(), _t(sd, nme + ".bias").double()
        w, b = wi @ w, wi @ b + bi
    return w, b


def _fold(sd, key: str):
    parts = [_fold_chain(sd, c) for c in key.split("|")]
    return torch.cat([p[0] for p in parts], 0).float(), torch.cat([p[1] for p in parts], 0).float()


def pack_entry(sd: Mapping[str, torch.Tensor], e: L.EgWeightEntry) -> np.ndarray:
    key, kind, d = e.key.decode(), e.kind, list(e.dims)
    if kind in (L.PACK_RAW, L.PACK_CONV1D):
        out = _t(sd, key).reshape(-1).numpy()
    elif kind == L.PACK_LINEAR:
        out = _pack_linear(_t(sd, key), d[2], d[3])
    elif kind == L.PACK_VEC_PAD:
        out = _pad1(_t(sd, key), d[1])
    elif kind == L.PACK_CONV3X3:
        out = _pack_conv3x3(_t(sd, key), d[2])
    elif kind == L.PACK_BN_SCALE:
        out = _pad1(_bn_affine(sd, key)[0], d[1])
    elif kind == L.PACK_BN_SHIFT:
        out = _pad1(_bn_affine(sd, key)[1], d[1])
    elif kind == L.PACK_CONV1X1:
        w = _t(sd, key)
        out = w.reshape(w.shape[0], w.shape[1]).t().contiguous().reshape(-1).numpy()
    elif kind == L.PACK_STEM:
        w = _t(sd, key)
        out = w.reshape(w.shape[0], 9).t().contiguous().reshape(-1).numpy()
    elif kind == L.PACK_WN_TAP:
        g, v = _t(sd, key + ".weight_g"), _t(sd, key + ".weight_v")
        w = v * (g / v.flatten(1).norm(dim=1).view(-1, 1, 1))
        npad = (d[0] + 63) // 64 * 64
        out = _pack_linear(w[:, :, d[2]].contiguous(), npad, d[3])
    elif kind == L.PACK_POS_TABLE:
        out = _t(sd, key)[0, : d[0], :].contiguous().reshape(-1).numpy()
    elif kind == L.PACK_LINEAR_T:
        out = _t(sd, key).t().contiguous().reshape(-1).numpy()
    elif kind == L.PACK_LINEAR_FOLD:
        out = _pack_linear(_fold(sd, key)[0], d[2], d[3])
    elif kind == L.PACK_BIAS_FOLD:
        out = _pad1(_fold(sd, key)[1], d[1])
    else:
        raise L.EgError(f"unknown pack kind {kind} for '{key}'")
    out = np.ascontiguousarray(out, dtype=np.float32)
    if out.size != e.numel:
        raise L.EgError(f"packing '{key}' (kind {kind}) produced {out.size} floats, manifest says {e.numel}")
    return out


def manifest(handle, num_fn, entry_fn):
    lib = L.load()
    n = getattr(lib, num_fn)(handle)
    out = []
    for i in range(n):
        e = L.EgWeightEntry()
        L.check(getattr(lib, entry_fn)(handle, i, C.byref(e)), entry_fn)
        out.append(e)
    return out


def build_arena(sd: Mapping[str, torch.Tensor], entries, total_floats: int) -> torch.Tensor:
    arena = np.zeros(int(total_floats), dtype=np.float32)
    for e in entries:
        arena[e.offset: e.offset + e.numel] = pack_entry(sd, e)
    return torch.from_numpy(arena)


def strip_module_prefix(sd: Mapping[str, torch.Tensor]):
    return {(k[7:] if k.startswith("module.") else k): v for k, v in sd.items()}
```

include/emogest.h:

```cpp
#ifndef EMOGEST_H
#define EMOGEST_H

#include <stddef.h>
#include <stdint.h>

#ifdef __cplusplus
extern "C" {
#endif

typedef enum EgStatus {
    EG_OK = 0,
    EG_ERR_BAD_ARG = -1,
    EG_ERR_UNSUPPORTED = -2,
    EG_ERR_WORKSPACE = -3,
    EG_ERR_HIP = -4,
    EG_ERR_ALIGN = -5
} EgStatus;

typedef enum EgPrecision {
    EG_PREC_F32 = 0,
    EG_PREC_BF16X3 = 1,
    EG_PREC_BF16 = 2
} EgPrecision;

const char* eg_last_error(void);
const char* eg_version(void);
int eg_set_default_precision(int precision);
int eg_get_default_precision(void);

int64_t eg_launch_count(void);
int64_t eg_launch_histogram(char* buf, int64_t cap, int32_t reset);
int eg_profile_enable(int32_t max_records);
int eg_profile_disable(void);
int32_t eg_profile_read(int64_t* tags, double* flops, float* ms, int32_t capacity);
int32_t eg_profile_read_workgroups(int32_t* workgroups, int32_t capacity);

typedef enum EgPackKind {
    EG_PACK_RAW = 0,
    EG_PACK_LINEAR = 1,
    EG_PACK_VEC_PAD = 2,
    EG_PACK_CONV3X3 = 3,
    EG_PACK_BN_SCALE = 4,
    EG_PACK_BN_SHIFT = 5,
    EG_PACK_CONV1X1 = 6,
    EG_PACK_STEM = 7,
    EG_PACK_WN_TAP = 8,
    EG_PACK_CONV1D = 9,
    EG_PACK_POS_TABLE = 10,
    EG_PACK_LINEAR_T = 11,
    EG_PACK_LINEAR_FOLD = 12,
    EG_PACK_BIAS_FOLD = 13
} EgPackKind;

typedef struct EgWeightEntry {
    char key[192];
    int32_t kind;
    int32_t dims[4];
    int64_t offset;
    int64_t numel;
} EgWeightEntry;

typedef struct EgGeneratorConfig {
    int32_t frames;
    int32_t pose_dim;
    int32_t prior_frames;
    int32_t chunk;
    int32_t d_model;
    int32_t d_inner;
    int32_t n_layers;
    int32_t n_head;
    int32_t d_k;
    int32_t n_mels;
    int32_t spec_len;
    int32_t text_len;
    int32_t n_words;
    int32_t embed_dim;
    int32_t tcn_hidden;
    int32_t tcn_layers;
    int32_t variant;
    int32_t precision;
    int32_t n_position;
    int32_t reserved[5];
} EgGeneratorConfig;

typedef struct EgGenerator EgGenerator;

int eg_generator_default_config(EgGeneratorConfig* cfg);
int eg_generator_create(const EgGeneratorConfig* cfg, EgGenerator** out);
void eg_generator_destroy(EgGenerator* g);
int64_t eg_generator_arena_floats(const EgGenerator* g);
int32_t eg_generator_num_weights(const EgGenerator* g);
int eg_generator_weight_entry(const EgGenerator* g, int32_t index, EgWeightEntry* out);
int64_t eg_generator_workspace_bytes(const EgGenerator* g, int32_t batch);

int eg_generator_forward(const EgGenerator* g, const float* arena, int32_t batch,
                         const float* spec, const int64_t* text, const float* prior, const float* sampled,
                         float* pose, float* emotion_feature, float* semantic_feature,
                         float* emotion_prediction, float* text_embedding,
                         void* workspace, int64_t workspace_bytes, void* stream);

int eg_generator_forward_draws(const EgGenerator* g, const float* arena, int32_t batch, int32_t draws,
                               const float* spec, const float* prior, const float* sampled, float* pose,
                               void* workspace, int64_t workspace_bytes, void* stream);
int64_t eg_generator_draws_workspace_bytes(const EgGenerator* g, int32_t batch, int32_t draws);
// ... 75 lines not shown
#define EG_BEAT_MAX_FRAMES 1024
int eg_beat_tables(float* h_melfb_t , float* h_window , float* h_twiddle ,
                   int32_t* h_band );
int64_t eg_beat_workspace_bytes(int32_t batch, int32_t n_samples);
int eg_beat_align(const float* audio, int32_t batch, int32_t n_samples, const float* pose, int32_t frames, int32_t pose_dim,
                  int32_t pose_fps, int32_t t_start, int32_t t_end, double sigma, int32_t order, const float* d_melfb_t,
                  const float* d_window, const float* d_twiddle, const int32_t* d_band, void* workspace, int64_t workspace_bytes,
                  double* score, int32_t* n_audio_beats, float* oenv, float* rms, uint8_t* audio_beats, uint8_t* pose_beats,
                  void* stream);

int64_t eg_beat_tracks_meta_ints(int32_t recordings);
int eg_beat_tracks_meta(const int32_t* lengths, const int32_t* frames , const int32_t* t_end ,
                        int32_t pose_fps, int32_t recordings, int32_t* meta);
int64_t eg_beat_tracks_workspace_bytes(const int32_t* lengths, const int32_t* frames , int32_t recordings, int32_t draws,
                                       int32_t Tmax);
int eg_beat_align_tracks(const float* audio, int32_t recordings, int64_t stride, const int32_t* lengths, const int32_t* d_meta,
                         const float* pose, int32_t draws, int32_t Tmax, int32_t pose_dim, const int32_t* frames, int32_t pose_fps,
                         int32_t t_start, const int32_t* t_end, double sigma, int32_t order, const float* d_melfb_t, const float* d_window,
                         const float* d_twiddle, const int32_t* d_band, void* workspace, int64_t workspace_bytes, double* score,
                         int32_t* n_audio_beats, float* oenv, float* rms, uint8_t* audio_beats, uint8_t* pose_beats, void* stream);
int eg_beat_tracks_scan(const uint8_t* d_cand, const int32_t* lengths, int32_t recordings, const int32_t* d_meta, void* workspace,
                        int64_t workspace_bytes, int32_t* events, int32_t* counts, void* stream);

#define EG_TAKE_CHUNK_FRAMES 16
#define EG_TAKE_MAX_DRAWS 64
int64_t eg_take_meta_ints(int32_t recordings);
int eg_take_meta(const int32_t* frames, int32_t recordings, int32_t* meta);
int eg_track_rows_pack(const float* track, int32_t recordings, int32_t draws, int32_t Tmax, int32_t pose_dim, const int32_t* frames,
                       const int32_t* d_meta, float* rows, void* stream);
int64_t eg_take_distance_workspace_bytes(const int32_t* frames, int32_t recordings, int32_t draws);
int eg_take_distance(const float* feat, int32_t recordings, int32_t draws, int32_t feat_dim, const int32_t* frames, const int32_t* d_meta,
                     int32_t span , void* workspace, int64_t workspace_bytes, double* distance, double* diversity,
                     void* stream);


int eg_conv3x3(const float* x, const float* w, const float* bias, const float* scale, const float* shift,
               float* y, float* gap_partial, int32_t batch, int32_t h, int32_t wdt, int32_t cin, int32_t cout,
               int32_t stride, int32_t relu, int32_t nchw_out, int32_t precision, void* stream);
int32_t eg_conv3x3_gap_tiles(int32_t h, int32_t wdt, int32_t cin, int32_t cout, int32_t stride);
int32_t eg_conv3x3_channel_split(int32_t batch, int32_t h, int32_t wdt, int32_t cin, int32_t cout, int32_t stride, int32_t precision);
int eg_conv3x3_se(const float* x, const float* w_packed, const float* bias, const float* scale, const float* shift, const float* gate,
                  const float* residual, float* y, float* gap_partial, int32_t batch, int32_t h, int32_t wdt, int32_t cin, int32_t cout,
                  int32_t stride, int32_t relu, int32_t nchw_out, int32_t precision, void* stream);
int eg_conv3x3_res_masked(const float* x, const float* w_packed, const float* residual, const uint32_t* res_bits, float* y, int32_t batch, int32_t h,
                          int32_t wdt, int32_t cin, int32_t cout, int32_t precision, void* stream);
int eg_conv3x3_sq(const float* x, const float* w_packed, const float* bias, float* y, float* gap_partial, float* gap_sq_partial, int32_t batch,
                  int32_t h, int32_t wdt, int32_t cin, int32_t cout, int32_t stride, int32_t relu, int32_t precision, void* stream);
int eg_conv3x3_sq_in_affine(const float* x, const float* in_scale, const float* in_shift, const float* w_packed, const float* bias, float* y,
                            float* gap_partial, float* gap_sq_partial, int32_t batch, int32_t h, int32_t wdt, int32_t cin, int32_t cout, int32_t stride,
                            int32_t relu, int32_t precision, void* stream);
int eg_se_gate_pre(const float* t1, const float* gap_partial, int32_t tiles, const float* conv2_w_packed, const float* scale2,
                   const float* shift2, const float* w1, const float* b1, const float* w2, const float* b2, float* gate,
                   int32_t batch, int32_t h, int32_t wdt, int32_t c, void* stream);
int64_t eg_conv3x3_packed_floats(int32_t cin, int32_t cout_pad);

int eg_stem_conv(const float* x, const float* w9xc, const float* bias, const float* scale, const float* shift,
                 float* y, int32_t batch, int32_t h, int32_t wdt, int32_t c, void* stream);

int eg_se_gate(const float* gap_partial, int32_t tiles, const float* w1, const float* b1, const float* w2,
               const float* b2, float* gate, int32_t batch, int32_t c, int32_t hw, void* stream);

int eg_se_residual_relu(const float* y, const float* gate, const float* x_in, const float* ds_w,
                        const float* ds_scale, const float* ds_shift, float* out, int32_t batch, int32_t ho,
                        int32_t wo, int32_t c, int32_t h_in, int32_t w_in, int32_t cin, int32_t stride, void* stream);

int eg_linear(const float* x, int32_t lda, const float* w, int32_t ldw, const float* bias,
              const float* res1, const float* res2, int32_t ldr, float* y, int32_t ldc,
              int32_t m, int32_t n, int32_t k, int32_t relu, int32_t a_shift, int32_t a_seq,
              int32_t precision, void* stream);
int eg_split_tiles(const float* x, int32_t lda, int32_t m, int32_t k, void* images, void* stream);
int eg_linear_presplit(const void* x_images, int32_t k_x, const float* w, int32_t ldw, const float* bias,
                       const float* res1, const float* res2, int32_t ldr, float* y, int32_t ldc,
                       int32_t m, int32_t n, int32_t k, int32_t relu, int32_t precision, void* stream);

int eg_linear_splitk(const float* x, int32_t lda, const float* w, int32_t ldw, const float* bias, float* y,
                     int32_t ldc, int32_t m, int32_t n, int32_t k, int32_t relu, int32_t splits,
                     float* partial, int32_t precision, void* stream);

typedef struct EgLinearArgs {
    const float* x; const float* w; const float* bias; const float* res1; const float* res2; float* y;
    const float* gate_src;
    const int32_t* drop_epoch;
    float* partial;
    const void* x_images;
    void* y_images;
    uint64_t drop_offset;
    int32_t lda, ldw, ldr, ldc, ldg;
    int32_t m, n, k, relu, precision, splits;
    int32_t k_x, y_k;
    uint32_t drop_seed;
    float drop_p;
} EgLinearArgs;
int eg_linear_ex(const EgLinearArgs* args, void* stream);

int eg_layernorm(const float* x, const float* gamma, const float* beta, float* y, int32_t rows, int32_t d,
                 float eps, void* stream);
int eg_layernorm_img(const float* x, const float* gamma, const float* beta, float* y, void* y_images, int32_t rows, int32_t d, float eps,
                     void* stream);

int eg_attention(const float* q, int32_t ldq, const float* k, int32_t ldk, const float* v, int32_t ldv,
                 float* out, int32_t ldo, float* attn, int32_t batch, int32_t heads, int32_t lq, int32_t lk,
                 int32_t dk, int32_t precision, void* stream);
int eg_attention_masked(const float* q, int32_t ldq, const float* k, int32_t ldk, const float* v, int32_t ldv, const uint8_t* mask,
                        int64_t mask_batch_stride, int32_t mask_query_stride, float* out, int32_t ldo, float* attn, int32_t batch,
                        int32_t heads, int32_t lq, int32_t lk, int32_t dk, int32_t precision, void* stream);

// ... 147 lines not shown
```

Before: 25430 clips/s.

## Fuse SE residual block including downsample shortcut into persistent conv kernels

```diff
diff --git a/emotiongestures_amd/_lib.py b/emotiongestures_amd/_lib.py
--- a/emotiongestures_amd/_lib.py
+++ b/emotiongestures_amd/_lib.py
@@ -10,7 +10,7 @@
 PRECISIONS = {"f32": EG_PREC_F32, "fp32": EG_PREC_F32, "bf16x3": EG_PREC_BF16X3, "bf16": EG_PREC_BF16}
 
 (PACK_RAW, PACK_LINEAR, PACK_VEC_PAD, PACK_CONV3X3, PACK_BN_SCALE, PACK_BN_SHIFT, PACK_CONV1X1, PACK_STEM,
- PACK_WN_TAP, PACK_CONV1D, PACK_POS_TABLE, PACK_LINEAR_T, PACK_LINEAR_FOLD, PACK_BIAS_FOLD) = range(14)
+ PACK_WN_TAP, PACK_CONV1D, PACK_POS_TABLE, PACK_LINEAR_T, PACK_LINEAR_FOLD, PACK_BIAS_FOLD, PACK_CONV1X1_BF16) = range(15)
 
 
 class EgError(RuntimeError):
@@ -109,6 +109,7 @@
     "eg_conv3x3": (C.c_int, [_P, _P, _P, _P, _P, _P, _P, _I, _I, _I, _I, _I, _I, _I, _I, _I, _P]),
     "eg_conv3x3_se": (C.c_int, [_P, _P, _P, _P, _P, _P, _P, _P, _P, _I, _I, _I, _I, _I, _I, _I, _I, _I, _P]),
     "eg_se_gate_pre": (C.c_int, [_P, _P, _I, _P, _P, _P, _P, _P, _P, _P, _P, _I, _I, _I, _I, _P]),
+    "eg_se_block_fused": (C.c_int, [_P] * 19 + [_I] * 7 + [_P]),
     "eg_conv3x3_gap_tiles": (_I, [_I, _I, _I, _I, _I]),
     "eg_conv3x3_channel_split": (_I, [_I, _I, _I, _I, _I, _I, _I]),
     "eg_stem_conv": (C.c_int, [_P, _P, _P, _P, _P, _P, _I, _I, _I, _I, _P]),
diff --git a/emotiongestures_amd/csrc/common.h b/emotiongestures_amd/csrc/common.h
--- a/emotiongestures_amd/csrc/common.h
+++ b/emotiongestures_amd/csrc/common.h
@@ -61,6 +61,16 @@
 #pragma unroll
     for (int o = 32; o > 0; o >>= 1) v += __shfl_xor(v, o, 64);
     return v;
+}
+template <int CTRL> __device__ __forceinline__ float dpp_move(float v) {
+    return __builtin_bit_cast(float, __builtin_amdgcn_update_dpp(0, __builtin_bit_cast(int, v), CTRL, 0xF, 0xF, true));
+}
+__device__ __forceinline__ float row16_sum(float s) {
+    s += dpp_move<0xB1>(s);
+    s += dpp_move<0x4E>(s);
+    s += dpp_move<0x141>(s);
+    s += dpp_move<0x140>(s);
+    return s;
 }
 __device__ __forceinline__ float wave_max(float v) {
 #pragma unroll
diff --git a/emotiongestures_amd/csrc/conv.hip b/emotiongestures_amd/csrc/conv.hip
--- a/emotiongestures_amd/csrc/conv.hip
+++ b/emotiongestures_amd/csrc/conv.hip
@@ -9,12 +9,15 @@
     float* y; float* gap;
     float* gap2 = nullptr;
     int H, W, Ho, Wo, cout, relu, nchw, tiles_x, tiles;
+    int batch = 0;
     const float* gate = nullptr; const float* res = nullptr; int relu2 = 0;
     const float* in_scale = nullptr; const float* in_shift = nullptr;
     int wrow = 0;
     const unsigned* res_bits = nullptr;
     const float* res_q = nullptr;
     unsigned int* dbg = nullptr;
+    const float* sc_x = nullptr; const bf8* sc_whi = nullptr; const bf8* sc_wlo = nullptr; const float* sc_vec = nullptr;
+    int sc_H = 0, sc_W = 0, sc_S = 2, sc_B = 0;
 };
 __device__ __forceinline__ f4 residual_quad(const float* __restrict__ res, const unsigned* __restrict__ bits, size_t e) {
     f4 r = *reinterpret_cast<const f4*>(res + e);
@@ -167,8 +170,7 @@
 #pragma unroll
             for (int r = 0; r < 4; ++r) {
                 float s = gsum[n][r];
-                s += __shfl_xor(s, 1, 64); s += __shfl_xor(s, 2, 64);
-                s += __shfl_xor(s, 4, 64); s += __shfl_xor(s, 8, 64);
+                s = row16_sum(s);
                 if (li == 0) sred[wave * COUTP + n * 16 + kq * 4 + r] = s;
             }
         }
@@ -181,10 +183,12 @@
 }
 
 
-template <int CIN, int NTT, int S, int TH, int WM, int WN, int TERMS, int RING, bool SPLIT = false, bool DG2 = false>
+template <int CIN, int NTT, int S, int TH, int WM, int WN, int TERMS, int RING, bool SPLIT = false, bool DG2 = false, int SCC = 0, bool PERSIST = false>
 __global__ __launch_bounds__(256, 2) void conv3x3_bf16_kernel(ConvArgs a, const bf8* __restrict__ whi,
                                                            const bf8* __restrict__ wlo) {
+    static_assert(!PERSIST || (!SPLIT && !DG2 && SCC <= 1), "the persistent walk serves the unsplit forward kernels");
     static_assert(!DG2 || (S == 1 && !SPLIT), "DG2 tiles the dy grid with unit stride");
+    static_assert(SCC == 0 || (S == 1 && !DG2 && SCC <= 2 && CIN >= 64), "the shortcut pre-phase belongs to a stride-1 conv2 and uses ring slots 2 and 1");
     using G = typename std::conditional<DG2, ConvGeomDG2<TH>, ConvGeom<S, TH>>::type;
     constexpr int PH = DG2 ? 4 : 1;
     constexpr int COUTP = NTT * 16, IW = G::IW, NPIX = G::NPIX, PL = G::PL;
@@ -203,7 +207,13 @@
     const int wm = wave / WN, wn = wave % WN;
     int tile_id = blockIdx.x, b = blockIdx.y;
     const int c0 = SPLIT ? (int)blockIdx.z * COUTP : 0;
-    if (!SPLIT) {
+    const int NWG = PERSIST ? (int)gridDim.x : 1, total_tiles = PERSIST ? a.tiles * a.batch : 1;
+    int L = PERSIST ? (int)((blockIdx.x & 7) * (gridDim.x >> 3) + (blockIdx.x >> 3)) : 0;
+    if constexpr (PERSIST) {
+        if (L >= total_tiles) return;
+        b = L / a.tiles;
+        tile_id = L - b * a.tiles;
+    } else if (!SPLIT) {
         const int total = gridDim.x * gridDim.y;
         if ((total & 7) == 0) {
             const int lin = blockIdx.y * gridDim.x + blockIdx.x;
@@ -212,9 +222,7 @@
             tile_id = log - b * (int)gridDim.x;
         }
     }
-    const int ty = tile_id / a.tiles_x, tx = tile_id - ty * a.tiles_x;
-    const int oy0 = ty * TH, ox0 = tx * 32;
-    const int iy0 = DG2 ? oy0 : oy0 * S - 1, ix0 = DG2 ? ox0 : ox0 * S - 1;
+    int oy0 = (tile_id / a.tiles_x) * TH, ox0 = (tile_id % a.tiles_x) * 32;
 
     int pbase[MT];
 #pragma unroll
@@ -229,34 +237,33 @@
         for (int t = 0; t < MT; ++t)
 #pragma unroll
             for (int n = 0; n < NT; ++n) acc[ph][t][n] = (f4){0.f, 0.f, 0.f, 0.f};
-    const float* __restrict__ xb = a.x + (size_t)b * a.H * a.W * CIN;
+    const float* xb = a.x + (size_t)b * a.H * a.W * CIN;
 
     const int wave_u = __builtin_amdgcn_readfirstlane(wave);
     constexpr int PIECES = WIMG / 64;
     constexpr int GTOT = NIMG * PIECES;
     constexpr bool COUNTED = (GTOT % 4 == 0);
     constexpr int GW = GTOT / 4;
-    auto issue_weights = [&](int step, int buf) {
-        const int chunk = step / 9, tap = step - chunk * 9;
+    auto issue_rows = [&](const bf8* __restrict__ ihi, const bf8* __restrict__ ilo, int row0, int buf) {
         if constexpr (SPLIT) {
             static_assert(COUNTED, "split instantiations deal whole pieces to the four waves");
-            const size_t rbase = ((size_t)tap * (CIN / 8) + chunk * 4) * a.wrow + c0;
+            const size_t rbase = (size_t)row0 * a.wrow + c0;
 #pragma unroll
             for (int p = 0; p < GW; ++p) {
                 const int flat = p * 4 + wave_u;
                 const int img = flat / PIECES, piece = flat - img * PIECES;
                 const int slot = piece * 64 + lane, oct = slot / COUTP, co = slot - oct * COUTP;
-                const bf8* src = (img ? wlo : whi) + rbase + (size_t)oct * a.wrow + co;
+                const bf8* src = (img ? ilo : ihi) + rbase + (size_t)oct * a.wrow + co;
                 __builtin_amdgcn_global_load_lds((const __attribute__((address_space(1))) void*)src,
                                                  (__attribute__((address_space(3))) void*)(wring + buf * WBUF + img * WIMG + piece * 64), 16, 0, 0);
             }
             return;
         }
-        const size_t gbase = ((size_t)tap * (CIN / 8) + chunk * 4) * COUTP;
+        const size_t gbase = (size_t)row0 * COUTP;
         if constexpr (PIECES % 4 == 0) {
 #pragma unroll
             for (int img = 0; img < NIMG; ++img) {
-                const bf8* src = (img ? wlo : whi) + gbase;
+                const bf8* src = (img ? ilo : ihi) + gbase;
 #pragma unroll
                 for (int p = 0; p < PIECES / 4; ++p) {
                     const int piece = p * 4 + wave_u;
@@ -271,27 +278,35 @@
                 const int flat = p * 4 + wave_u;
                 if (COUNTED || flat < GTOT) {
                     const int img = flat / PIECES, piece = flat - img * PIECES;
-                    const bf8* src = (img ? wlo : whi) + gbase;
+                    const bf8* src = (img ? ilo : ihi) + gbase;
                     __builtin_amdgcn_global_load_lds((const __attribute__((address_space(1))) void*)(src + piece * 64 + lane),
                                                      (__attribute__((address_space(3))) void*)(wring + buf * WBUF + img * WIMG + piece * 64),
                                                      16, 0, 0);
                 }
             }
         }
+    };
+    auto issue_weights = [&](int step, int buf) {
+        const int chunk = step / 9, tap = step - chunk * 9;
+        issue_rows(whi, wlo, tap * (CIN / 8) + chunk * 4, buf);
     };
     constexpr int NIT = (((NPIX + 7) / 8) * 32 + 255) / 256;
     f4 pv[NIT][2];
     int goff[NIT], lslot[NIT];
-#pragma unroll
-    for (int it = 0; it < NIT; ++it) {
-        const int idx = tid + it * 256;
-        const int p = (idx >> 5) * 8 + (idx & 7), oc = (idx >> 3) & 3;
-        const int iy = p / IW, ix = p - iy * IW;
-        const int gy = iy0 + iy, gx = ix0 + ix;
-        const bool inside = p < NPIX && gy >= 0 && gy < a.H && gx >= 0 && gx < a.W;
-        goff[it] = inside ? (gy * a.W + gx) * CIN + oc * 8 : -1;
-        lslot[it] = p < NPIX ? oc * PL + p : -1;
-    }
+    auto set_goff = [&](int toy0, int tox0) {
+        const int iy0 = DG2 ? toy0 : toy0 * S - 1, ix0 = DG2 ? tox0 : tox0 * S - 1;
+#pragma unroll
+        for (int it = 0; it < NIT; ++it) {
+            const int idx = tid + it * 256;
+            const int p = (idx >> 5) * 8 + (idx & 7), oc = (idx >> 3) & 3;
+            const int iy = p / IW, ix = p - iy * IW;
+            const int gy = iy0 + iy, gx = ix0 + ix;
+            const bool inside = p < NPIX && gy >= 0 && gy < a.H && gx >= 0 && gx < a.W;
+            goff[it] = inside ? (gy * a.W + gx) * CIN + oc * 8 : -1;
+            lslot[it] = p < NPIX ? oc * PL + p : -1;
+        }
+    };
+    set_goff(oy0, ox0);
     auto load_tile = [&](int chunk) {
 #pragma unroll
         for (int it = 0; it < NIT; ++it) {
@@ -306,14 +321,15 @@
     const int oc8s = ((tid >> 3) & 3) * 8;
     auto store_tile = [&](int chunk) {
         f4 s0 = (f4){1.f, 1.f, 1.f, 1.f}, s1 = s0, h0 = (f4){0.f, 0.f, 0.f, 0.f}, h1 = h0;
-        if (a.in_scale) {
+        const bool in_aff = a.in_scale != nullptr;
+        if (in_aff) {
             s0 = *reinterpret_cast<const f4*>(a.in_scale + chunk * 32 + oc8s); s1 = *reinterpret_cast<const f4*>(a.in_scale + chunk * 32 + oc8s + 4);
             h0 = *reinterpret_cast<const f4*>(a.in_shift + chunk * 32 + oc8s); h1 = *reinterpret_cast<const f4*>(a.in_shift + chunk * 32 + oc8s + 4);
         }
 #pragma unroll
         for (int it = 0; it < NIT; ++it) {
             if (lslot[it] >= 0) {
-                if (a.in_scale && goff[it] >= 0) {
+                if (in_aff && goff[it] >= 0) {
                     pv[it][0] = pv[it][0] * s0 + h0;
                     pv[it][1] = pv[it][1] * s1 + h1;
                 }
@@ -326,8 +342,8 @@
     };
 
     struct Frags { bf8 wh[NT], wl[NT], xh[MT], xl[MT]; };
-    auto read_w = [&](Frags& f, int tap) {
-        const bf8* Wh = wring + (tap % 3) * WBUF + kq * COUTP + wn * NT * 16 + li;
+    auto read_w = [&](Frags& f, int slot) {
+        const bf8* Wh = wring + slot * WBUF + kq * COUTP + wn * NT * 16 + li;
 #pragma unroll
         for (int n = 0; n < NT; ++n) {
             f.wh[n] = Wh[n * 16];
@@ -368,141 +384,230 @@
             __syncthreads();
         }
     };
-    issue_weights(0, 0);
-    if (NSTEP > 1) issue_weights(1, 1);
-    load_tile(0);
     Frags fr[2];
+    for (bool first = true;; first = false) {
+        const bool has_next = PERSIST && L + NWG < total_tiles;
+        int n_b = 0, n_tile = 0, n_oy0 = 0, n_ox0 = 0;
+        if (has_next) {
+            n_b = (L + NWG) / a.tiles;
+            n_tile = L + NWG - n_b * a.tiles;
+            n_oy0 = (n_tile / a.tiles_x) * TH;
+            n_ox0 = (n_tile % a.tiles_x) * 32;
+        }
+        if constexpr (SCC > 0) {
+#pragma unroll
+            for (int c = 0; c < SCC; ++c) issue_rows(a.sc_whi, a.sc_wlo, c * 4, 2 - c);
+            if (first) {
+                issue_weights(0, 0);
+                if (SCC == 1) issue_weights(1, 1);
+            }
+            constexpr int SNIT = TH * 128 / 256;
+            static_assert(SNIT * 256 == TH * 128, "shortcut staging deals whole iterations");
+            int sgoff[SNIT], sslot[SNIT];
+#pragma unroll
+            for (int it = 0; it < SNIT; ++it) {
+                const int idx = tid + it * 256;
+                const int p = (idx >> 5) * 8 + (idx & 7), oc = (idx >> 3) & 3;
+                const int r = p >> 5, col = p & 31, oy = oy0 + r, ox = ox0 + col;
+                sgoff[it] = (oy < a.Ho && ox < a.Wo) ? (oy * a.sc_S * a.sc_W + ox * a.sc_S) * (SCC * 32) + oc * 8 : -1;
+                sslot[it] = oc * PL + (r + 1) * IW + col + 1;
+            }
+            const float* __restrict__ sxb = a.sc_x + (size_t)b * a.sc_H * a.sc_W * (SCC * 32);
+            f4 sv[SNIT][2];
+            auto load_sc = [&](int c) {
+#pragma unroll
+                for (int it = 0; it < SNIT; ++it) {
+                    sv[it][0] = sv[it][1] = (f4){0.f, 0.f, 0.f, 0.f};
+                    if (sgoff[it] >= 0) {
+                        const float* src = sxb + sgoff[it] + c * 32;
+                        sv[it][0] = *reinterpret_cast<const f4*>(src);
+                        sv[it][1] = *reinterpret_cast<const f4*>(src + 4);
+                    }
+                }
+            };
+            load_sc(0);
+            if (first) load_tile(0);
+#pragma unroll
+            for (int c = 0; c < SCC; ++c) {
+#pragma unroll
+                for (int it = 0; it < SNIT; ++it) {
+                    bf8 hi, lo;
+                    split_octet<TERMS == 3>(sv[it][0], sv[it][1], hi, lo);
+                    tile[sslot[it]] = hi;
+                    if (TERMS == 3) tile[4 * PL + sslot[it]] = lo;
+                }
+                if (c + 1 < SCC) load_sc(c + 1);
+                __syncthreads();
+                read_w(fr[0], 2 - c);
+                read_x(fr[0], 4);
+                mfma_half(fr[0], 0, 4);
+                mfma_half(fr[0], 1, 4);
+                __syncthreads();
+            }
+            if (SCC == 2) issue_weights(1, 1);
+            const float* __restrict__ fv = a.sc_vec + (size_t)b * a.cout;
+#pragma unroll
+            for (int n = 0; n < NT; ++n) {
+                const f4 fq = *reinterpret_cast<const f4*>(fv + c0 + (wn * NT + n) * 16 + kq * 4);
+#pragma unroll
+                for (int t = 0; t < MT; ++t) acc[0][t][n] = acc[0][t][n] * fq;
+            }
+        } else if (first) {
+            issue_weights(0, 0);
+            if (NSTEP > 1) issue_weights(1, 1);
+            load_tile(0);
+        }
 #pragma unroll 1
-    for (int chunk = 0; chunk < CIN / 32; ++chunk) {
-        store_tile(chunk);
-        if (COUNTED && chunk > 0) {
-            wait_vmcnt_imm<GW>();
+        for (int chunk = 0; chunk < CIN / 32; ++chunk) {
+            store_tile(chunk);
+            if (COUNTED && chunk > 0) {
+                wait_vmcnt_imm<GW>();
+                wait_lgkmcnt0();
+                wg_barrier();
+            } else {
+                __syncthreads();
+            }
+            if (chunk + 1 < CIN / 32) {
+                load_tile(chunk + 1);
+            } else if (has_next) {
+                set_goff(n_oy0, n_ox0);
+                xb = a.x + (size_t)n_b * a.H * a.W * CIN;
+                load_tile(0);
+            }
+            read_w(fr[0], 0);
+            read_x(fr[0], 0);
+#pragma unroll
+            for (int tap = 0; tap < 9; ++tap) {
+                const int step = chunk * 9 + tap;
+                const bool more = step + 2 < NSTEP || has_next;
+                if (more) issue_weights(step + 2 < NSTEP ? step + 2 : step + 2 - NSTEP, (tap + 2) % 3);
+                mfma_half(fr[tap & 1], 0, tap);
+                mid_sync(more);
+                if (tap < 8) { read_w(fr[(tap + 1) & 1], (tap + 1) % 3); read_x(fr[(tap + 1) & 1], tap + 1); }
+                mfma_half(fr[tap & 1], 1, tap);
+            }
+        }
+
+        if constexpr (DG2) {
+            const size_t ohw = (size_t)a.Ho * a.Wo;
+            float* __restrict__ yb = a.y + (size_t)b * ohw * a.cout;
+            const float* __restrict__ rq = a.res_q ? a.res_q + (size_t)b * a.H * a.W * a.cout : nullptr;
+#pragma unroll
+            for (int ph = 0; ph < 4; ++ph) {
+                const int py = ph >> 1, px = ph & 1;
+#pragma unroll
+                for (int t = 0; t < MT; ++t) {
+                    const int id = wm * MT + t;
+                    const int by = oy0 + (id >> 1), bx = ox0 + (id & 1) * 16 + li;
+                    const int oy = 2 * by + py, ox = 2 * bx + px;
+                    if (by < a.H && bx < a.W && oy < a.Ho && ox < a.Wo) {
+#pragma unroll
+                        for (int n = 0; n < NT; ++n) {
+                            const int co = (wn * NT + n) * 16 + kq * 4;
+                            if (co < a.cout) {
+                                f4 v = acc[ph][t][n];
+                                if (ph == 0 && rq) v += *reinterpret_cast<const f4*>(rq + ((size_t)by * a.W + bx) * a.cout + co);
+                                *reinterpret_cast<f4*>(yb + ((size_t)oy * a.Wo + ox) * a.cout + co) = v;
+                            }
+                        }
+                    }
+                }
+            }
+            return;
+        }
+
+        f4 gsum[NT], gsq[NT];
+        int pixo[MT];
+#pragma unroll
+        for (int t = 0; t < MT; ++t) {
+            const int id = wm * MT + t;
+            const int oy = oy0 + (id >> 1), ox = ox0 + (id & 1) * 16 + li;
+            pixo[t] = (oy < a.Ho && ox < a.Wo) ? oy * a.Wo + ox : -1;
+        }
+        const int hw = a.Ho * a.Wo;
+        float* __restrict__ yb = a.y + (size_t)b * hw * a.cout;
+        int cbase = c0;
+        if constexpr (PERSIST) asm volatile("" : "+s"(cbase));
+#pragma unroll
+        for (int n = 0; n < NT; ++n) {
+            gsum[n] = (f4){0.f, 0.f, 0.f, 0.f};
+            gsq[n] = gsum[n];
+            const int co = cbase + (wn * NT + n) * 16 + kq * 4;
+            const f4 bi = a.bias ? *reinterpret_cast<const f4*>(a.bias + co) : (f4){0.f, 0.f, 0.f, 0.f};
+            f4 sc = a.scale ? *reinterpret_cast<const f4*>(a.scale + co) : (f4){1.f, 1.f, 1.f, 1.f};
+            f4 sh = a.shift ? *reinterpret_cast<const f4*>(a.shift + co) : (f4){0.f, 0.f, 0.f, 0.f};
+            if constexpr (SCC > 0) {
+                const float* __restrict__ qv = a.sc_vec + ((size_t)a.sc_B + b) * a.cout + co;
+                sc = *reinterpret_cast<const f4*>(qv);
+                sh = *reinterpret_cast<const f4*>(qv + (size_t)a.sc_B * a.cout);
+            }
+            const f4 gt = (a.gate && co < a.cout) ? *reinterpret_cast<const f4*>(a.gate + (size_t)b * a.cout + co) : (f4){1.f, 1.f, 1.f, 1.f};
+            const bool rb = a.res != nullptr;
+            const size_t rbase = (size_t)b * hw * a.cout;
+#pragma unroll
+            for (int t = 0; t < MT; ++t) {
+                f4 v = acc[0][t][n] + bi;
+                if (a.relu) {
+#pragma unroll
+                    for (int r = 0; r < 4; ++r) v[r] = fmaxf(v[r], 0.f);
+                }
+                v = v * sc + sh;
+                if (a.gate) v = v * gt;
+                if (rb && pixo[t] >= 0 && co < a.cout) v += residual_quad(a.res, a.res_bits, rbase + (size_t)pixo[t] * a.cout + co);
+                if (a.relu2) {
+#pragma unroll
+                    for (int r = 0; r < 4; ++r) v[r] = fmaxf(v[r], 0.f);
+                }
+                if (pixo[t] >= 0) {
+                    if (!a.nchw) {
+                        if (co < a.cout) *reinterpret_cast<f4*>(yb + pixo[t] * a.cout + co) = v;
+                    } else {
+#pragma unroll
+                        for (int r = 0; r < 4; ++r)
+                            if (co + r < a.cout) yb[(co + r) * hw + pixo[t]] = v[r];
+                    }
+                    gsum[n] += v;
+                    if (a.gap2) gsq[n] += v * v;
+                }
+            }
+        }
+        if (a.gap) {
+            float* sred = reinterpret_cast<float*>(PERSIST ? lds + TILE + RING * WBUF : lds);
+#pragma unroll
+            for (int n = 0; n < NT; ++n) {
+#pragma unroll
+                for (int r = 0; r < 4; ++r) {
+                    float s = gsum[n][r];
+                    s = row16_sum(s);
+                    if (li == 0) sred[wm * COUTP + (wn * NT + n) * 16 + kq * 4 + r] = s;
+                    if (a.gap2) {
+                        float q = gsq[n][r];
+                        q = row16_sum(q);
+                        if (li == 0) sred[(WM + wm) * COUTP + (wn * NT + n) * 16 + kq * 4 + r] = q;
+                    }
+                }
+            }
             wait_lgkmcnt0();
             wg_barrier();
-        } else {
-            __syncthreads();
-        }
-        if (chunk + 1 < CIN / 32) load_tile(chunk + 1);
-        read_w(fr[0], 0);
-        read_x(fr[0], 0);
-#pragma unroll
-        for (int tap = 0; tap < 9; ++tap) {
-            const int step = chunk * 9 + tap;
-            if (step + 2 < NSTEP) issue_weights(step + 2, (tap + 2) % 3);
-            mfma_half(fr[tap & 1], 0, tap);
-            mid_sync(step + 2 < NSTEP);
-            if (tap < 8) { read_w(fr[(tap + 1) & 1], tap + 1); read_x(fr[(tap + 1) & 1], tap + 1); }
-            mfma_half(fr[tap & 1], 1, tap);
-        }
-    }
-
-    if constexpr (DG2) {
-        const size_t ohw = (size_t)a.Ho * a.Wo;
-        float* __restrict__ yb = a.y + (size_t)b * ohw * a.cout;
-        const float* __restrict__ rq = a.res_q ? a.res_q + (size_t)b * a.H * a.W * a.cout : nullptr;
-#pragma unroll
-        for (int ph = 0; ph < 4; ++ph) {
-            const int py = ph >> 1, px = ph & 1;
-#pragma unroll
-            for (int t = 0; t < MT; ++t) {
-                const int id = wm * MT + t;
-                const int by = oy0 + (id >> 1), bx = ox0 + (id & 1) * 16 + li;
-                const int oy = 2 * by + py, ox = 2 * bx + px;
-                if (by < a.H && bx < a.W && oy < a.Ho && ox < a.Wo) {
-#pragma unroll
-                    for (int n = 0; n < NT; ++n) {
-                        const int co = (wn * NT + n) * 16 + kq * 4;
-                        if (co < a.cout) {
-                            f4 v = acc[ph][t][n];
-                            if (ph == 0 && rq) v += *reinterpret_cast<const f4*>(rq + ((size_t)by * a.W + bx) * a.cout + co);
-                            *reinterpret_cast<f4*>(yb + ((size_t)oy * a.Wo + ox) * a.cout + co) = v;
-                        }
-                    }
-                }
-            }
-        }
-        return;
-    }
-
-    f4 gsum[NT], gsq[NT];
-    int pixo[MT];
-#pragma unroll
-    for (int t = 0; t < MT; ++t) {
-        const int id = wm * MT + t;
-        const int oy = oy0 + (id >> 1), ox = ox0 + (id & 1) * 16 + li;
-        pixo[t] = (oy < a.Ho && ox < a.Wo) ? oy * a.Wo + ox : -1;
-    }
-    const int hw = a.Ho * a.Wo;
-    float* __restrict__ yb = a.y + (size_t)b * hw * a.cout;
-#pragma unroll
-    for (int n = 0; n < NT; ++n) {
-        gsum[n] = (f4){0.f, 0.f, 0.f, 0.f};
-        gsq[n] = gsum[n];
-        const int co = c0 + (wn * NT + n) * 16 + kq * 4;
-        const f4 bi = a.bias ? *reinterpret_cast<const f4*>(a.bias + co) : (f4){0.f, 0.f, 0.f, 0.f};
-        const f4 sc = a.scale ? *reinterpret_cast<const f4*>(a.scale + co) : (f4){1.f, 1.f, 1.f, 1.f};
-        const f4 sh = a.shift ? *reinterpret_cast<const f4*>(a.shift + co) : (f4){0.f, 0.f, 0.f, 0.f};
-        const f4 gt = (a.gate && co < a.cout) ? *reinterpret_cast<const f4*>(a.gate + (size_t)b * a.cout + co) : (f4){1.f, 1.f, 1.f, 1.f};
-        const bool rb = a.res != nullptr;
-        const size_t rbase = (size_t)b * hw * a.cout;
-#pragma unroll
-        for (int t = 0; t < MT; ++t) {
-            f4 v = acc[0][t][n] + bi;
-            if (a.relu) {
-#pragma unroll
-                for (int r = 0; r < 4; ++r) v[r] = fmaxf(v[r], 0.f);
-            }
-            v = v * sc + sh;
-            if (a.gate) v = v * gt;
-            if (rb && pixo[t] >= 0 && co < a.cout) v += residual_quad(a.res, a.res_bits, rbase + (size_t)pixo[t] * a.cout + co);
-            if (a.relu2) {
-#pragma unroll
-                for (int r = 0; r < 4; ++r) v[r] = fmaxf(v[r], 0.f);
-            }
-            if (pixo[t] >= 0) {
-                if (!a.nchw) {
-                    if (co < a.cout) *reinterpret_cast<f4*>(yb + pixo[t] * a.cout + co) = v;
-                } else {
-#pragma unroll
-                    for (int r = 0; r < 4; ++r)
-                        if (co + r < a.cout) yb[(co + r) * hw + pixo[t]] = v[r];
-                }
-                gsum[n] += v;
-                if (a.gap2) gsq[n] += v * v;
-            }
-        }
-    }
-    if (a.gap) {
-        float* sred = reinterpret_cast<float*>(lds);
-#pragma unroll
-        for (int n = 0; n < NT; ++n) {
-#pragma unroll
-            for (int r = 0; r < 4; ++r) {
-                float s = gsum[n][r];
-                s += __shfl_xor(s, 1, 64); s += __shfl_xor(s, 2, 64);
-                s += __shfl_xor(s, 4, 64); s += __shfl_xor(s, 8, 64);
-                if (li == 0) sred[wm * COUTP + (wn * NT + n) * 16 + kq * 4 + r] = s;
+            if (tid < (SPLIT ? COUTP : a.cout)) {
+                float s = 0.f;
+#pragma unroll
+                for (int m = 0; m < WM; ++m) s += sred[m * COUTP + tid];
+                a.gap[((size_t)b * a.tiles + tile_id) * a.cout + c0 + tid] = s;
                 if (a.gap2) {
-                    float q = gsq[n][r];
-                    q += __shfl_xor(q, 1, 64); q += __shfl_xor(q, 2, 64);
-                    q += __shfl_xor(q, 4, 64); q += __shfl_xor(q, 8, 64);
-                    if (li == 0) sred[(WM + wm) * COUTP + (wn * NT + n) * 16 + kq * 4 + r] = q;
-                }
-            }
-        }
-        __syncthreads();
-        if (tid < (SPLIT ? COUTP : a.cout)) {
-            float s = 0.f;
-#pragma unroll
-            for (int m = 0; m < WM; ++m) s += sred[m * COUTP + tid];
-            a.gap[((size_t)b * a.tiles + tile_id) * a.cout + c0 + tid] = s;
-            if (a.gap2) {
-                float q = 0.f;
-#pragma unroll
-                for (int m = 0; m < WM; ++m) q += sred[(WM + m) * COUTP + tid];
-                a.gap2[((size_t)b * a.tiles + tile_id) * a.cout + c0 + tid] = q;
-            }
-        }
+                    float q = 0.f;
+#pragma unroll
+                    for (int m = 0; m < WM; ++m) q += sred[(WM + m) * COUTP + tid];
+                    a.gap2[((size_t)b * a.tiles + tile_id) * a.cout + c0 + tid] = q;
+                }
+            }
+        }
+        if (!has_next) break;
+        L += NWG; b = n_b; tile_id = n_tile; oy0 = n_oy0; ox0 = n_ox0;
+#pragma unroll
+        for (int t = 0; t < MT; ++t)
+#pragma unroll
+            for (int n = 0; n < NT; ++n) acc[0][t][n] = (f4){0.f, 0.f, 0.f, 0.f};
     }
 }
 
@@ -751,13 +856,11 @@
 #pragma unroll
                 for (int r = 0; r < 4; ++r) {
                     float sm = gsum[n][r];
-                    sm += __shfl_xor(sm, 1, 64); sm += __shfl_xor(sm, 2, 64);
-                    sm += __shfl_xor(sm, 4, 64); sm += __shfl_xor(sm, 8, 64);
+                    sm = row16_sum(sm);
                     if (li == 0) sred[wave * sred_pitch + n * 16 + kq * 4 + r] = sm;
                     if (a.gap2) {
                         float q = gsq[n][r];
-                        q += __shfl_xor(q, 1, 64); q += __shfl_xor(q, 2, 64);
-                        q += __shfl_xor(q, 4, 64); q += __shfl_xor(q, 8, 64);
+                        q = row16_sum(q);
                         if (li == 0) sred[128 + wave * 32 + n * 16 + kq * 4 + r] = q;
                     }
                 }
@@ -849,7 +952,8 @@
                                                            const float* __restrict__ w2img, const float* __restrict__ scale2,
                                                            const float* __restrict__ shift2, const float* __restrict__ w1, const float* __restrict__ b1,
                                                            const float* __restrict__ wf2, const float* __restrict__ bf2, float* __restrict__ gate,
-                                                           int H, int W, int C) {
+                                                           int H, int W, int C, const float* __restrict__ ds_scale, const float* __restrict__ ds_shift,
+                                                           float* __restrict__ sc_vec) {
     extern __shared__ __attribute__((aligned(16))) float sm[];
     const int b = blockIdx.x, t = threadIdx.x, G = GP_T / C, c = t % C, g = t / C, R = C >> 3;
     float* part = sm;
@@ -929,7 +1033,16 @@
     if (t < C) {
         float s = bf2[t];
         for (int j = 0; j < R; ++j) s += wf2[t * R + j] * hbuf[j];
-        gate[(size_t)b * C + t] = 1.f / (1.f + expf(-s));
+        const float gt = 1.f / (1.f + expf(-s));
+        gate[(size_t)b * C + t] = gt;
+        if (sc_vec) {
+            const size_t BC = (size_t)gridDim.x * C;
+            float q = gt * scale2[t];
+            if (!(fabsf(q) >= 1e-30f)) q = copysignf(1e-30f, q);
+            sc_vec[(size_t)b * C + t] = ds_scale[t] / q;
+            sc_vec[BC + (size_t)b * C + t] = q;
+            sc_vec[2 * BC + (size_t)b * C + t] = shift2[t] * gt + ds_shift[t];
+        }
     }
 }
 
@@ -979,25 +1092,26 @@
     }
 }
 
-template <int CIN, int NT, int S, int TH, int WM, int WN, int TERMS>
+template <int CIN, int NT, int S, int TH, int WM, int WN, int TERMS, int SCC = 0, bool PERSIST = false>
 int launch_conv_bf16(const ConvArgs& a, const bf8* whi, const bf8* wlo, dim3 grid, hipStream_t st) {
     constexpr int RING = 3;
     using G = ConvGeom<S, TH>;
     constexpr int NIMG = (TERMS == 3) ? 2 : 1;
-    constexpr size_t LDS_BYTES = sizeof(bf8) * (size_t)(NIMG * 4 * G::PL + RING * NIMG * 4 * NT * 16);
-    auto kern = conv3x3_bf16_kernel<CIN, NT, S, TH, WM, WN, TERMS, RING>;
+    constexpr size_t LDS_BYTES = sizeof(bf8) * (size_t)(NIMG * 4 * G::PL + RING * NIMG * 4 * NT * 16) +
+                                 (PERSIST ? sizeof(float) * 2 * WM * NT * 16 : 0);
+    auto kern = conv3x3_bf16_kernel<CIN, NT, S, TH, WM, WN, TERMS, RING, false, false, SCC, PERSIST>;
     if (int rc = eg_ensure_dynamic_lds(reinterpret_cast<const void*>(kern), LDS_BYTES, "conv3x3")) return rc;
     hipLaunchKernelGGL(kern, grid, dim3(256), LDS_BYTES, st, a, whi, wlo);
     return eg_check_launch("conv3x3");
 }
 
-template <int CIN, int NTS, int TH, int WM, int WN, int TERMS>
+template <int CIN, int NTS, int TH, int WM, int WN, int TERMS, int SCC = 0>
 int launch_conv_split_t(ConvArgs a, int batch, const bf8* whi, const bf8* wlo, hipStream_t st) {
     constexpr int RING = 3;
     using G = ConvGeom<1, TH>;
     constexpr int NIMG = (TERMS == 3) ? 2 : 1;
     constexpr size_t LDS_BYTES = sizeof(bf8) * (size_t)(NIMG * 4 * G::PL + RING * NIMG * 4 * NTS * 16);
-    auto kern = conv3x3_bf16_kernel<CIN, NTS, 1, TH, WM, WN, TERMS, RING, true>;
+    auto kern = conv3x3_bf16_kernel<CIN, NTS, 1, TH, WM, WN, TERMS, RING, true, false, SCC>;
     if (int rc = eg_ensure_dynamic_lds(reinterpret_cast<const void*>(kern), LDS_BYTES, "conv3x3 (channel split)")) return rc;
     a.wrow = a.cout;
     hipLaunchKernelGGL(kern, dim3(a.tiles, batch, a.cout / (NTS * 16)), dim3(256), LDS_BYTES, st, a, whi, wlo);
@@ -1028,18 +1142,47 @@
     return conv_channel_split(tiles * batch, cin == 128 ? 4 : 2);
 }
 
-template <int CIN, int NT, int S, int TH, int WM, int WN>
+constexpr int CONV_PERSIST_DEFAULT_KINDS = 0;
+int conv_persist_grid(int kind, int total) {
+    const int resident = 512;
+    const char* e = getenv("EG_CONV_GRID");
+    if (e && e[0]) {
+        const int g = atoi(e);
+        if (g <= 0) return 0;
+        const int64_t cap = eg_round_up(total, 8), want = eg_round_up(g, 8);
+        return (int)(total > 0 && cap < want ? cap : want);
+    }
+    if (total <= 0) return 0;
+    const char* k = getenv("EG_CONV_PERSIST_KINDS");
+    const int kinds = (k && k[0]) ? atoi(k) : CONV_PERSIST_DEFAULT_KINDS;
+    return ((kinds & kind) && total > resident) ? resident : 0;
+}
+
+bool conv_persist_forced() { return conv_persist_grid(0, 0) > 0; }
+
+template <int CIN, int NT, int S, int TH, int WM, int WN, int SCC = 0, int KIND = 0>
 int launch_conv(const ConvArgs& a, int batch, int precision, hipStream_t st) {
     dim3 grid(a.tiles, batch), block(256);
     if (precision == EG_PREC_F32) {
+        if constexpr (SCC > 0) {
+            eg_set_error("conv3x3: the fused downsample shortcut exists in the split-bf16 modes only");
+            return EG_ERR_UNSUPPORTED;
+        }
         hipLaunchKernelGGL((conv3x3_f32_kernel<CIN, NT, S, TH>), grid, block, 0, st, a);
         return eg_check_launch("conv3x3");
     }
     const size_t f32_floats = (size_t)9 * CIN * NT * 16;
     const bf8* whi = reinterpret_cast<const bf8*>(a.w + f32_floats);
     const bf8* wlo = whi + (size_t)9 * (CIN / 8) * NT * 16;
-    if (precision == EG_PREC_BF16X3) return launch_conv_bf16<CIN, NT, S, TH, WM, WN, 3>(a, whi, wlo, grid, st);
-    return launch_conv_bf16<CIN, NT, S, TH, WM, WN, 1>(a, whi, wlo, grid, st);
+    if constexpr (KIND != 0) {
+        const bool infer = !a.gap2 && !a.in_scale && !a.res_bits && !(a.res && !a.gate);
+        if (const int g = infer ? conv_persist_grid(KIND, a.tiles * batch) : 0) {
+            if (precision == EG_PREC_BF16X3) return launch_conv_bf16<CIN, NT, S, TH, WM, WN, 3, SCC, true>(a, whi, wlo, dim3(g), st);
+            return launch_conv_bf16<CIN, NT, S, TH, WM, WN, 1, SCC, true>(a, whi, wlo, dim3(g), st);
+        }
+    }
+    if (precision == EG_PREC_BF16X3) return launch_conv_bf16<CIN, NT, S, TH, WM, WN, 3, SCC>(a, whi, wlo, grid, st);
+    return launch_conv_bf16<CIN, NT, S, TH, WM, WN, 1, SCC>(a, whi, wlo, grid, st);
 }
 
 bool conv32_persistent_enabled() {
@@ -1138,10 +1281,11 @@
 }
 
 namespace {
+struct ShortcutArgs { const float* x; const float* wimg; const float* vec; int h, w, cin, stride; };
 int conv3x3_dispatch(const float* x, const float* w, const float* bias, const float* scale, const float* shift, const float* gate, const float* residual,
                      float* y, float* gap_partial, float* gap_sq, int32_t batch, int32_t h, int32_t wdt, int32_t cin, int32_t cout, int32_t stride,
                      int32_t relu, int32_t nchw_out, int32_t precision, void* stream, const float* in_scale = nullptr, const float* in_shift = nullptr,
-                     const uint32_t* res_bits = nullptr);
+                     const uint32_t* res_bits = nullptr, const ShortcutArgs* sc = nullptr);
 }
 extern "C" int eg_conv3x3_se(const float* x, const float* w, const float* bias, const float* scale, const float* shift, const float* gate,
                              const float* residual, float* y, float* gap_partial, int32_t batch, int32_t h, int32_t wdt, int32_t cin,
@@ -1174,7 +1318,8 @@
 namespace {
 int conv3x3_dispatch(const float* x, const float* w, const float* bias, const float* scale, const float* shift, const float* gate, const float* residual,
                      float* y, float* gap_partial, float* gap_sq, int32_t batch, int32_t h, int32_t wdt, int32_t cin, int32_t cout, int32_t stride,
-                     int32_t relu, int32_t nchw_out, int32_t precision, void* stream, const float* in_scale, const float* in_shift, const uint32_t* res_bits) {
+                     int32_t relu, int32_t nchw_out, int32_t precision, void* stream, const float* in_scale, const float* in_shift, const uint32_t* res_bits,
+                     const ShortcutArgs* sc) {
     EG_REQUIRE(x && w && y && batch > 0 && h > 0 && wdt > 0, EG_ERR_BAD_ARG, "eg_conv3x3: null pointer or empty shape");
     EG_REQUIRE(!res_bits || (residual && !gate && ((size_t)batch * h * wdt * cout) % 32 == 0), EG_ERR_BAD_ARG,
                "eg_conv3x3_res_masked: the bit mask needs a residual, no gate and a map of a multiple of 32 elements");
@@ -1193,7 +1338,7 @@
     a.res_bits = res_bits;
     a.in_scale = in_scale; a.in_shift = in_shift;
     a.H = h; a.W = wdt; a.Ho = (h + 2 - 3) / stride + 1; a.Wo = (wdt + 2 - 3) / stride + 1;
-    a.cout = cout; a.relu = relu; a.nchw = nchw_out;
+    a.cout = cout; a.relu = relu; a.nchw = nchw_out; a.batch = batch;
     const int th = conv_tile_rows(cin, cout, stride);
     a.tiles_x = eg_cdiv(a.Wo, 32);
     a.tiles = a.tiles_x * eg_cdiv(a.Ho, th);
@@ -1201,12 +1346,33 @@
     const int coutp = (int)eg_round_up(cout, 16);
     EgProfScope prof((int64_t)cin * 1000000 + (int64_t)cout * 1000 + stride * 100 + 1,
                      2.0 * 9 * cin * cout * (double)a.Ho * a.Wo * batch, st);
+    if (sc) {
+        EG_REQUIRE(precision != EG_PREC_F32 && stride == 1 && !nchw_out && cout == cin && (cin == 64 || cin == 128) && sc->cin * 2 == cin, EG_ERR_UNSUPPORTED,
+                   "conv3x3: the fused downsample shortcut serves 32 -> 64 and 64 -> 128 block entries in the split-bf16 modes (cin=%d cout=%d shortcut cin=%d)",
+                   cin, cout, sc->cin);
+        EG_REQUIRE(sc->x && sc->wimg && sc->vec && !gate && !residual && !bias && !relu && !gap_sq && !in_scale && sc->stride >= 1 &&
+                   (sc->h - 1) / sc->stride + 1 == h && (sc->w - 1) / sc->stride + 1 == wdt && eg_aligned16(sc->x) && eg_aligned16(sc->wimg) &&
+                   eg_aligned16(sc->vec), EG_ERR_BAD_ARG, "conv3x3: fused downsample shortcut: null / misaligned operand or a block input that does not map onto the output");
+        a.sc_x = sc->x; a.sc_vec = sc->vec; a.sc_H = sc->h; a.sc_W = sc->w; a.sc_S = sc->stride; a.sc_B = batch;
+        a.sc_whi = reinterpret_cast<const bf8*>(sc->wimg);
+        a.sc_wlo = a.sc_whi + (size_t)(sc->cin / 8) * cout;
+        a.scale = a.shift = nullptr;
+        a.relu2 = 1;
+        const int split = (cin == 64 && conv_persist_forced()) ? 1 : body_channel_split(batch, a.tiles, cin, cout, 1, precision, 0);
+        const bf8* whi = reinterpret_cast<const bf8*>(a.w + (size_t)9 * cin * cout);
+        const bf8* wlo = whi + (size_t)9 * (cin / 8) * cout;
+        if (cin == 64 && split == 2) return launch_conv_split_t<64, 2, 8, 4, 1, 3, 1>(a, batch, whi, wlo, st);
+        if (cin == 64) return launch_conv<64, 4, 1, 8, 4, 1, 1, 1>(a, batch, precision, st);
+        if (split == 2) return launch_conv_split_t<128, 4, 4, 2, 2, 3, 2>(a, batch, whi, wlo, st);
+        if (split == 4) return launch_conv_split_t<128, 2, 4, 2, 2, 3, 2>(a, batch, whi, wlo, st);
+        return launch_conv<128, 8, 1, 4, 2, 2, 2>(a, batch, precision, st);
+    }
     if (cin == 32 && coutp == 32 && cout == 32 && stride == 1 && precision != EG_PREC_F32 && !nchw_out && conv32_persistent_enabled())
         return launch_conv32_persistent(a, batch, precision, th, st);
     if (cin == 32 && coutp == 32 && stride == 1 && th == 4) return launch_conv<32, 2, 1, 4, 4, 1>(a, batch, precision, st);
     if (cin == 32 && coutp == 32 && stride == 1) return launch_conv<32, 2, 1, 8, 4, 1>(a, batch, precision, st);
-    if (cin == 32 && coutp == 64 && stride == 2) return launch_conv<32, 4, 2, 2, 2, 2>(a, batch, precision, st);
-    if (const int split = body_channel_split(batch, a.tiles, cin, cout, stride, precision, nchw_out); split > 1) {
+    if (cin == 32 && coutp == 64 && stride == 2) return launch_conv<32, 4, 2, 2, 2, 2, 0, 2>(a, batch, precision, st);
+    if (const int split = (cin == 64 && conv_persist_forced()) ? 1 : body_channel_split(batch, a.tiles, cin, cout, stride, precision, nchw_out); split > 1) {
         const size_t f32_floats = (size_t)9 * cin * cout;
         const bf8* whi = reinterpret_cast<const bf8*>(a.w + f32_floats);
         const bf8* wlo = whi + (size_t)9 * (cin / 8) * cout;
@@ -1214,15 +1380,15 @@
         if (cin == 128 && split == 2) return launch_conv_split_t<128, 4, 4, 2, 2, 3>(a, batch, whi, wlo, st);
         if (cin == 128 && split == 4) return launch_conv_split_t<128, 2, 4, 2, 2, 3>(a, batch, whi, wlo, st);
     }
-    if (cin == 64 && coutp == 64 && stride == 1) return launch_conv<64, 4, 1, 8, 4, 1>(a, batch, precision, st);
-    if (cin == 64 && coutp == 128 && stride == 2) return launch_conv<64, 8, 2, 2, 2, 2>(a, batch, precision, st);
+    if (cin == 64 && coutp == 64 && stride == 1) return launch_conv<64, 4, 1, 8, 4, 1, 0, 1>(a, batch, precision, st);
+    if (cin == 64 && coutp == 128 && stride == 2) return launch_conv<64, 8, 2, 2, 2, 2, 0, 4>(a, batch, precision, st);
     if (cin == 64 && coutp == 128 && stride == 1) return launch_conv<64, 8, 1, 4, 2, 2>(a, batch, precision, st);
     if (cin == 128 && coutp == 128 && stride == 1) return launch_conv<128, 8, 1, 4, 2, 2>(a, batch, precision, st);
     if (cin == 128 && coutp == 256 && stride == 2) return launch_conv<128, 16, 2, 2, 1, 4>(a, batch, precision, st);
     if (cin == 256 && coutp == 256 && stride == 1) return launch_conv<256, 16, 1, 2, 1, 4>(a, batch, precision, st);
     if (cin == 128 && coutp <= 64 && stride == 1) {
-        if (coutp <= 48) return launch_conv<128, 3, 1, 4, 4, 1>(a, batch, precision, st);
-        return launch_conv<128, 4, 1, 4, 4, 1>(a, batch, precision, st);
+        if (coutp <= 48) return launch_conv<128, 3, 1, 4, 4, 1, 0, 8>(a, batch, precision, st);
+        return launch_conv<128, 4, 1, 4, 4, 1, 0, 8>(a, batch, precision, st);
     }
     if (cin == 128 && coutp <= 128 && stride == 1) return launch_conv<128, 8, 1, 4, 2, 2>(a, batch, precision, st);
     eg_set_error("eg_conv3x3: unsupported channels cin=%d cout=%d stride=%d", cin, cout, stride);
@@ -1271,16 +1437,44 @@
     return eg_check_launch("se_gate");
 }
 
-extern "C" int eg_se_gate_pre(const float* t1, const float* gap_partial, int32_t tiles, const float* conv2_w, const float* scale2,
-                              const float* shift2, const float* w1, const float* b1, const float* w2, const float* b2, float* gate,
-                              int32_t batch, int32_t h, int32_t wdt, int32_t c, void* stream) {
+namespace {
+int se_gate_pre_launch(const float* t1, const float* gap_partial, int32_t tiles, const float* conv2_w, const float* scale2,
+                       const float* shift2, const float* w1, const float* b1, const float* w2, const float* b2, float* gate,
+                       int32_t batch, int32_t h, int32_t wdt, int32_t c, void* stream, const float* ds_scale, const float* ds_shift, float* sc_vec) {
     EG_REQUIRE(t1 && gap_partial && conv2_w && scale2 && shift2 && w1 && b1 && w2 && b2 && gate && batch > 0 && h > 1 && wdt > 1, EG_ERR_BAD_ARG,
                "eg_se_gate_pre: null pointer or empty shape");
     EG_REQUIRE(c % 8 == 0 && c <= 256 && 256 % c == 0 && eg_aligned16(conv2_w), EG_ERR_UNSUPPORTED, "eg_se_gate_pre: C=%d", c);
     const size_t smem = sizeof(float) * (5 * GP_T + 9 * (size_t)c + GP_T + c + (c >> 3) + 4);
+    EG_REQUIRE(!sc_vec || (ds_scale && ds_shift), EG_ERR_BAD_ARG, "eg_se_gate_pre: the shortcut vectors need the downsample BatchNorm");
     hipLaunchKernelGGL(se_gate_pre_kernel, dim3(batch), dim3(GP_T), smem, (hipStream_t)stream, t1, gap_partial, tiles, conv2_w, scale2, shift2, w1,
-                       b1, w2, b2, gate, h, wdt, c);
+                       b1, w2, b2, gate, h, wdt, c, ds_scale, ds_shift, sc_vec);
     return eg_check_launch("se_gate_pre");
+}
+}
+
+extern "C" int eg_se_gate_pre(const float* t1, const float* gap_partial, int32_t tiles, const float* conv2_w, const float* scale2,
+                              const float* shift2, const float* w1, const float* b1, const float* w2, const float* b2, float* gate,
+                              int32_t batch, int32_t h, int32_t wdt, int32_t c, void* stream) {
+    return se_gate_pre_launch(t1, gap_partial, tiles, conv2_w, scale2, shift2, w1, b1, w2, b2, gate, batch, h, wdt, c, stream, nullptr, nullptr, nullptr);
+}
+
+extern "C" int eg_se_block_fused(const float* x, const float* conv1_w, const float* scale1, const float* shift1, const float* conv2_w, const float* scale2,
+                                 const float* shift2, const float* se_w1, const float* se_b1, const float* se_w2, const float* se_b2, const float* ds_w,
+                                 const float* ds_scale, const float* ds_shift, float* t1, float* out, float* gap_partial, float* gate, float* sc_vec,
+                                 int32_t batch, int32_t h, int32_t wdt, int32_t cin, int32_t cout, int32_t stride, int32_t precision, void* stream) {
+    EG_REQUIRE(x && conv1_w && scale1 && shift1 && conv2_w && scale2 && shift2 && t1 && out && gap_partial && gate, EG_ERR_BAD_ARG, "eg_se_block_fused: null pointer");
+    EG_REQUIRE(ds_w ? (ds_scale && ds_shift && sc_vec) : (cin == cout && stride == 1), EG_ERR_BAD_ARG,
+               "eg_se_block_fused: a downsample needs its BatchNorm and the shortcut vectors; an identity shortcut needs cin == cout and stride 1");
+    EG_REQUIRE(stride == 1 || stride == 2, EG_ERR_UNSUPPORTED, "eg_se_block_fused: stride %d", stride);
+    const int ho = (h + 2 - 3) / stride + 1, wo = (wdt + 2 - 3) / stride + 1;
+    if (int rc = eg_conv3x3(x, conv1_w, nullptr, scale1, shift1, t1, gap_partial, batch, h, wdt, cin, cout, stride, 1, 0, precision, stream)) return rc;
+    const int tiles1 = eg_conv3x3_gap_tiles(h, wdt, cin, cout, stride);
+    if (int rc = se_gate_pre_launch(t1, gap_partial, tiles1, conv2_w, scale2, shift2, se_w1, se_b1, se_w2, se_b2, gate, batch, ho, wo, cout, stream,
+                                    ds_w ? ds_scale : nullptr, ds_w ? ds_shift : nullptr, ds_w ? sc_vec : nullptr)) return rc;
+    if (!ds_w) return eg_conv3x3_se(t1, conv2_w, nullptr, scale2, shift2, gate, x, out, nullptr, batch, ho, wo, cout, cout, 1, 0, 0, precision, stream);
+    const ShortcutArgs sc{x, ds_w, sc_vec, h, wdt, cin, stride};
+    return conv3x3_dispatch(t1, conv2_w, nullptr, nullptr, nullptr, nullptr, nullptr, out, nullptr, nullptr, batch, ho, wo, cout, cout, 1, 0, 0, precision, stream,
+                            nullptr, nullptr, nullptr, &sc);
 }
 
 extern "C" int eg_se_residual_relu(const float* y, const float* gate, const float* x_in, const float* ds_w,
diff --git a/emotiongestures_amd/csrc/generator.hip b/emotiongestures_amd/csrc/generator.hip
--- a/emotiongestures_amd/csrc/generator.hip
+++ b/emotiongestures_amd/csrc/generator.hip
@@ -179,6 +179,7 @@
     int64_t se_w1, se_b1, se_w2, se_b2;
     bool ds = false;
     int64_t ds_w = -1, ds_scale = -1, ds_shift = -1;
+    int64_t ds_wb = -1;
     int cin, cout, stride;
 };
 struct MhaW { LinW q, kv, qkv, o; int64_t ln_g, ln_b; };
@@ -308,7 +309,7 @@
 namespace {
 
 struct GenWs {
-    int64_t act[3], gap, gate, amap, afc1, afeat, emo_t, emo, sem_t, sem, cls_part, cls_h[3], cls_out;
+    int64_t act[3], gap, gate, scv, amap, afc1, afeat, emo_t, emo, sem_t, sem, cls_part, cls_h[3], cls_out;
     int64_t fus_in, fus_h, fusion, xa, xb, q, qkv, ao, proj, ffn_h, im_x[2], im_enc, im_h, im_a[3], im_p[2];
     int64_t prior_cat, prior_h, prior_enc, prior_rep, tm_mem, tm_pe, tm_gram, post_a, post_b, post_c, pose;
     int64_t t_emb, t_a, t_b, t_c, t_out;
@@ -331,11 +332,14 @@
             const int ho = (h + 2 - 3) / b.stride + 1, wo = (wd + 2 - 3) / b.stride + 1;
             const int64_t need = (int64_t)eg_conv3x3_gap_tiles(ho, wo, b.cout, b.cout, 1) * b.cout;
             gap_per_clip = need > gap_per_clip ? need : gap_per_clip;
+            const int64_t need1 = (int64_t)eg_conv3x3_gap_tiles(h, wd, b.cin, b.cout, b.stride) * b.cout;
+            gap_per_clip = need1 > gap_per_clip ? need1 : gap_per_clip;
             h = ho; wd = wo;
         }
         w.gap = cv.take((int64_t)B * gap_per_clip);
     }
     w.gate = cv.take((int64_t)B * 128);
+    w.scv = cv.take((int64_t)3 * B * 128);
     w.amap = cv.take(BF * g->HW3);
     w.afc1 = cv.take(BF * D); w.afeat = cv.take(BF * D);
     w.emo_t = cv.take(BF * D * 2); w.emo = cv.take(BF * D); w.sem_t = cv.take(16); w.sem = cv.take(BF * D);
@@ -461,13 +465,11 @@
             const BlockW& bw = g->blocks[bi];
             const int t1 = (xi + 1) % 3, t2 = (xi + 2) % 3;
             const int ho = (h + 2 - 3) / bw.stride + 1, wo = (wd + 2 - 3) / bw.stride + 1;
-            if (!bw.ds && g->fuse_se) {
-                EG_TRY(run_conv(arena, bw.c1, bufs[xi], bufs[t1], gap, B, h, wd, 1, 0, prec, st));
-                const int tiles1 = eg_conv3x3_gap_tiles(h, wd, bw.cin, bw.cout, 1);
-                EG_TRY(eg_se_gate_pre(bufs[t1], gap, tiles1, arena + bw.c2.w, arena + bw.c2.scale, arena + bw.c2.shift, arena + bw.se_w1,
-                                      arena + bw.se_b1, arena + bw.se_w2, arena + bw.se_b2, gate, B, ho, wo, bw.cout, st));
-                EG_TRY(eg_conv3x3_se(bufs[t1], arena + bw.c2.w, nullptr, arena + bw.c2.scale, arena + bw.c2.shift, gate, bufs[xi], bufs[t2], nullptr, B,
-                                     ho, wo, bw.cout, bw.cout, 1, 0, 0, prec, st));
+            if (g->fuse_se && (!bw.ds || prec != EG_PREC_F32)) {
+                EG_TRY(eg_se_block_fused(bufs[xi], arena + bw.c1.w, arena + bw.c1.scale, arena + bw.c1.shift, arena + bw.c2.w, arena + bw.c2.scale,
+                                         arena + bw.c2.shift, arena + bw.se_w1, arena + bw.se_b1, arena + bw.se_w2, arena + bw.se_b2,
+                                         bw.ds ? arena + bw.ds_wb : nullptr, bw.ds ? arena + bw.ds_scale : nullptr, bw.ds ? arena + bw.ds_shift : nullptr,
+                                         bufs[t1], bufs[t2], gap, gate, P(ws, w.scv), B, h, wd, bw.cin, bw.cout, bw.stride, prec, st));
                 xi = t2; h = ho; wd = wo;
                 continue;
             }
@@ -680,6 +682,7 @@
             b.ds = (b.stride != 1 || inpl != planes);
             if (b.ds) {
                 b.ds_w = L.add(p + ".downsample.0.weight", EG_PACK_CONV1X1, planes, inpl, 0, 0, (int64_t)inpl * planes);
+                b.ds_wb = L.add(p + ".downsample.0.weight", EG_PACK_CONV1X1_BF16, planes, inpl, 0, 0, (int64_t)inpl * planes);
                 add_bn(L, p + ".downsample.1", planes, planes, b.ds_scale, b.ds_shift);
             }
             g->blocks.push_back(b);
diff --git a/emotiongestures_amd/csrc/misc.hip b/emotiongestures_amd/csrc/misc.hip
--- a/emotiongestures_amd/csrc/misc.hip
+++ b/emotiongestures_amd/csrc/misc.hip
@@ -2,11 +2,10 @@
 
 namespace {
 
-struct LnSum { int nparts = 0; const float* bias2 = nullptr; const float* resid = nullptr; int ldr = 0; };
-template <int NV, bool SUMP = false>
+template <int NV>
 __global__ __launch_bounds__(256) void layernorm_kernel(const float* __restrict__ x, const float* __restrict__ g,
                                                         const float* __restrict__ b, float* __restrict__ y, int rows, int D,
-                                                        float eps, unsigned short* __restrict__ img, LnSum ps = LnSum()) {
+                                                        float eps, unsigned short* __restrict__ img) {
     const int row = blockIdx.x * 4 + (threadIdx.x >> 6), lane = threadIdx.x & 63;
     if (row >= rows) return;
     const f4* xr = reinterpret_cast<const f4*>(x + (size_t)row * D);
@@ -17,10 +16,6 @@
     for (int i = 0; i < NV; ++i) {
         const int q = lane + i * 64;
         v[i] = q < nq ? xr[q] : (f4){0.f, 0.f, 0.f, 0.f};
-        if (SUMP && q < nq) {
-            for (int p = 1; p < ps.nparts; ++p) v[i] += reinterpret_cast<const f4*>(x + ((size_t)p * rows + row) * D)[q];
-            v[i] = v[i] + reinterpret_cast<const f4*>(ps.bias2)[q] + reinterpret_cast<const f4*>(ps.resid + (size_t)row * ps.ldr)[q];
-        }
         s += (v[i][0] + v[i][1]) + (v[i][2] + v[i][3]);
     }
     const float mean = wave_sum(s) / (float)D;
diff --git a/emotiongestures_amd/modules.py b/emotiongestures_amd/modules.py
--- a/emotiongestures_amd/modules.py
+++ b/emotiongestures_amd/modules.py
@@ -263,6 +263,16 @@
         if self.downsample is not None:
             return ops.se_residual_relu(y, gate, x, self.downsample[0].weight, ds[0], ds[1], stride=self.stride)
         return ops.se_residual_relu(y, gate, x)
+
+    def forward_fused_nhwc(self, x):
+        _eval_only(self)
+        c1, c2, ds = self._packed(x.device)
+        fc = self.se.fc
+        kw = {}
+        if self.downsample is not None:
+            kw = dict(ds_weight=self.downsample[0].weight, ds_scale=ds[0], ds_shift=ds[1])
+        return ops.se_block_fused(x, c1, c2, fc[0].weight, fc[0].bias, fc[2].weight, fc[2].bias, self.conv2.weight.shape[0], stride=self.stride,
+                                  precision=self.precision, **kw)
 
     def forward(self, x):
         return self.forward_nhwc(x.permute(0, 2, 3, 1).contiguous()).permute(0, 3, 1, 2).contiguous()
diff --git a/emotiongestures_amd/ops.py b/emotiongestures_amd/ops.py
--- a/emotiongestures_amd/ops.py
+++ b/emotiongestures_amd/ops.py
@@ -113,6 +113,27 @@
     return out
 
 
+def se_block_fused(x_nhwc, c1, c2, se_w1, se_b1, se_w2, se_b2, cout, stride=1, ds_weight=None, ds_scale=None, ds_shift=None, precision="bf16x3"):
+    lib = L.load()
+    x = _need_cuda(x_nhwc, "x")
+    dev = x.device
+    B, H, W, Cin = x.shape
+    Ho, Wo = (H - 1) // stride + 1, (W - 1) // stride + 1
+    tiles = lib.eg_conv3x3_gap_tiles(H, W, Cin, cout, stride)
+    t1, out = torch.empty(B, Ho, Wo, cout, device=dev), torch.empty(B, Ho, Wo, cout, device=dev)
+    gap, gate = torch.empty(B, tiles, cout, device=dev), torch.empty(B, cout, device=dev)
+    dsw = scv = None
+    if ds_weight is not None:
+        dsw = torch.from_numpy(packing._pack_conv1x1_bf16(ds_weight.detach().cpu().float())).to(dev)
+        scv = torch.empty(3, B, cout, device=dev)
+        ds_scale, ds_shift = _need_cuda(ds_scale, "ds_scale"), _need_cuda(ds_shift, "ds_shift")
+    L.check(lib.eg_se_block_fused(_ptr(x), _ptr(c1[0]), _ptr(c1[2]), _ptr(c1[3]), _ptr(c2[0]), _ptr(c2[2]), _ptr(c2[3]), _ptr(_need_cuda(se_w1, "w1")),
+                                  _ptr(_need_cuda(se_b1, "b1")), _ptr(_need_cuda(se_w2, "w2")), _ptr(_need_cuda(se_b2, "b2")), _ptr(dsw), _ptr(ds_scale),
+                                  _ptr(ds_shift), _ptr(t1), _ptr(out), _ptr(gap), _ptr(gate), _ptr(scv), B, H, W, Cin, cout, stride,
+                                  L.precision_code(precision), _stream(dev)), "eg_se_block_fused")
+    return out
+
+
 def linear(x, weight, bias=None, res1=None, res2=None, relu=False, a_shift=0, a_seq=0, precision="f32", packed=None):
     lib = L.load()
     x = _need_cuda(x, "x")
diff --git a/emotiongestures_amd/packing.py b/emotiongestures_amd/packing.py
--- a/emotiongestures_amd/packing.py
+++ b/emotiongestures_amd/packing.py
@@ -51,6 +51,13 @@
     return _with_bf16_images(f32.numpy(), hi, lo)
 
 
+def _pack_conv1x1_bf16(w: torch.Tensor) -> np.ndarray:
+    o, i = w.shape[:2]
+    oct_ = w.reshape(o, i).t().reshape(i // 8, 8, o).permute(0, 2, 1).contiguous()
+    hi, lo = _bf16_split_bits(oct_)
+    return np.concatenate([hi.reshape(-1), lo.reshape(-1)]).view(np.float32)
+
+
 def _bn_affine(sd, prefix: str):
     scale = _t(sd, prefix + ".weight") / torch.sqrt(_t(sd, prefix + ".running_var") + BN_EPS)
     shift = _t(sd, prefix + ".bias") - _t(sd, prefix + ".running_mean") * scale
@@ -95,6 +102,8 @@
     elif kind == L.PACK_CONV1X1:
         w = _t(sd, key)
         out = w.reshape(w.shape[0], w.shape[1]).t().contiguous().reshape(-1).numpy()
+    elif kind == L.PACK_CONV1X1_BF16:
+        out = _pack_conv1x1_bf16(_t(sd, key))
     elif kind == L.PACK_STEM:
         w = _t(sd, key)
         out = w.reshape(w.shape[0], 9).t().contiguous().reshape(-1).numpy()
diff --git a/include/emogest.h b/include/emogest.h
--- a/include/emogest.h
+++ b/include/emogest.h
@@ -49,7 +49,8 @@
     EG_PACK_POS_TABLE = 10,
     EG_PACK_LINEAR_T = 11,
     EG_PACK_LINEAR_FOLD = 12,
-    EG_PACK_BIAS_FOLD = 13
+    EG_PACK_BIAS_FOLD = 13,
+    EG_PACK_CONV1X1_BF16 = 14
 } EgPackKind;
 
 typedef struct EgWeightEntry {
@@ -231,6 +232,10 @@
 int eg_se_gate_pre(const float* t1, const float* gap_partial, int32_t tiles, const float* conv2_w_packed, const float* scale2,
                    const float* shift2, const float* w1, const float* b1, const float* w2, const float* b2, float* gate,
                    int32_t batch, int32_t h, int32_t wdt, int32_t c, void* stream);
+int eg_se_block_fused(const float* x, const float* conv1_w, const float* scale1, const float* shift1, const float* conv2_w, const float* scale2,
+                      const float* shift2, const float* se_w1, const float* se_b1, const float* se_w2, const float* se_b2, const float* ds_w,
+                      const float* ds_scale, const float* ds_shift, float* t1, float* out, float* gap_partial, float* gate, float* sc_vec,
+                      int32_t batch, int32_t h, int32_t wdt, int32_t cin, int32_t cout, int32_t stride, int32_t precision, void* stream);
 int64_t eg_conv3x3_packed_floats(int32_t cin, int32_t cout_pad);
 
 int eg_stem_conv(const float* x, const float* w9xc, const float* bias, const float* scale, const float* shift,
```

Measured after the change: 26270 clips/s (median of 6 runs). 1.03x the previous value.
